# nh2/lz4-frame-conduit

Measured on AMD Instinct MI355X. Metric: GiB/s end-to-end (compress+decompress), 4 MiB blocks, 1/2/4/8 GPUs vs liblz4, higher is better.
Workload: dtype u8

## Files before the change

lz4_frame_conduit_amd/csrc/common.cuh:

```cuda
#pragma once
#include <hip/hip_runtime.h>
#include <stdint.h>

#include "records.hpp"

#define WAVE 64

namespace lz4f {

typedef const __attribute__((address_space(1))) void* gptr_t;
typedef __attribute__((address_space(3))) void* lptr_t;
typedef __attribute__((address_space(3))) uint32_t lds_u32;
typedef __attribute__((address_space(3))) uint8_t lds_u8;
typedef uint32_t u32_ua __attribute__((aligned(1)));
struct __attribute__((packed, aligned(1))) b16_ua { uint32_t a, b, c, d; };
struct __attribute__((aligned(4))) w3_a4 { uint32_t a, b, c; };

__device__ __forceinline__ uint32_t lane_id() { return threadIdx.x & (WAVE - 1); }
__device__ __forceinline__ uint32_t uni(uint32_t v) { return __builtin_amdgcn_readfirstlane(v); }
__device__ __forceinline__ uint64_t uni64(uint64_t v)
{
    uint32_t lo = __builtin_amdgcn_readfirstlane((uint32_t)v), hi = __builtin_amdgcn_readfirstlane((uint32_t)(v >> 32));
    return ((uint64_t)hi << 32) | lo;
}
// ... 41 lines not shown
        const bool body = lane < nfull, last = lane == nfull && tail;
        if (body || last) *(b16_ua*)(dst + (body ? lane * 16 : len - 16)) = b16_ua{p.a, p.b, p.c, p.d};
    }
}

struct v4u_ua { uint32_t a, b, c, d; } __attribute__((packed, aligned(1)));
struct CopyJob { const uint8_t* s; uint8_t* d; uint32_t n; };
__device__ __forceinline__ void job_load(Piece& p, const CopyJob& j, const uint8_t* safe)
{
    const uint32_t lane = lane_id(), nfull = j.n >> 4, tail = j.n & 15;
    const uint8_t* a = safe;
    if (lane < nfull) a = j.s + lane * 16; else if (lane == nfull && tail) a = j.s + j.n - 16;
    const v4u_ua t = *(const v4u_ua*)a;
    p.a = t.a; p.b = t.b; p.c = t.c; p.d = t.d;
}
__device__ __forceinline__ void job_store(const CopyJob& j, const Piece& p)
{
    const uint32_t lane = lane_id(), nfull = j.n >> 4, tail = j.n & 15;
    if (lane < nfull || (lane == nfull && tail)) {
        uint8_t* a = (lane < nfull) ? j.d + lane * 16 : j.d + j.n - 16;
        *(v4u_ua*)a = v4u_ua{p.a, p.b, p.c, p.d};
    }
}

__device__ __forceinline__ void wave_copy_match(uint8_t* dst, uint32_t offset, uint32_t len)
{
    const uint32_t lane = lane_id();
    const uint8_t* src = dst - offset;
    if (offset >= len) {
        wave_copy_disjoint(dst, src, len);
        return;
    }
    uint32_t done = 0;
    if (offset < 64) {
        uint32_t idx = lane % offset;
        const uint32_t inc = WAVE % offset;
        const uint32_t k = (1024 + offset - 1) / offset;
        const uint32_t need = (k - 1) * offset;
        while (done < len && done < need) {
            if (done + lane < len) dst[done + lane] = src[idx];
            idx += inc; if (idx >= offset) idx -= offset;
            done += WAVE;
        }
        if (done >= len) return;
        offset *= k;
        src = dst - offset;
    }
    const uint32_t R = (offset >= 1024) ? 1024u : (offset & ~15u);
    const uint32_t lanes_r = R >> 4;
    while (done < len) {
        const uint32_t left = len - done;
        if (left >= R) {
            if (lane < lanes_r) *(b16_ua*)(dst + done + lane * 16) = *(const b16_ua*)(src + done + lane * 16);
            done += R;
        } else {
            wave_copy_disjoint(dst + done, src + done, left);
            done = len;
        }
    }
}

__device__ __forceinline__ uint32_t dpp_incl_scan_add(uint32_t v)
{
    v += (uint32_t)__builtin_amdgcn_update_dpp(0, (int)v, 0x111 , 0xf, 0xf, true);
    v += (uint32_t)__builtin_amdgcn_update_dpp(0, (int)v, 0x112 , 0xf, 0xf, true);
    v += (uint32_t)__builtin_amdgcn_update_dpp(0, (int)v, 0x114 , 0xf, 0xf, true);
    v += (uint32_t)__builtin_amdgcn_update_dpp(0, (int)v, 0x118 , 0xf, 0xf, true);
    v += (uint32_t)__builtin_amdgcn_update_dpp(0, (int)v, 0x142 , 0xa, 0xf, false);
    v += (uint32_t)__builtin_amdgcn_update_dpp(0, (int)v, 0x143 , 0xc, 0xf, false);
    return v;
}
__device__ __forceinline__ uint32_t dpp_incl_scan_max(uint32_t v)
{
    uint32_t t;
    t = (uint32_t)__builtin_amdgcn_update_dpp(0, (int)v, 0x111, 0xf, 0xf, true); v = t > v ? t : v;
    t = (uint32_t)__builtin_amdgcn_update_dpp(0, (int)v, 0x112, 0xf, 0xf, true); v = t > v ? t : v;
    t = (uint32_t)__builtin_amdgcn_update_dpp(0, (int)v, 0x114, 0xf, 0xf, true); v = t > v ? t : v;
    t = (uint32_t)__builtin_amdgcn_update_dpp(0, (int)v, 0x118, 0xf, 0xf, true); v = t > v ? t : v;
    t = (uint32_t)__builtin_amdgcn_update_dpp(0, (int)v, 0x142, 0xa, 0xf, false); v = t > v ? t : v;
    t = (uint32_t)__builtin_amdgcn_update_dpp(0, (int)v, 0x143, 0xc, 0xf, false); v = t > v ? t : v;
    return v;
}

__device__ __forceinline__ uint32_t dpp_excl_scan_max(uint32_t v)
{
    const uint32_t incl = dpp_incl_scan_max(v);
    return (uint32_t)__builtin_amdgcn_update_dpp(0, (int)incl, 0x138 , 0xf, 0xf, true);
}

}
```

lz4_frame_conduit_amd/csrc/decode_indexed.cuh:

```cuda
#pragma once
#include "common.cuh"
#include "decode.cuh"
#include "decode_fused.cuh"
#include "decode_linked.cuh"
#include "encode.cuh"

namespace lz4f {

__device__ __forceinline__ uint64_t pt_load8(const uint8_t* __restrict__ in, uint32_t pos, uint64_t readable)
{
    if ((uint64_t)pos + 8 <= readable) { typedef uint64_t u64u __attribute__((aligned(1))); return *(const u64u*)(in + pos); }
    uint64_t v = 0;
    for (uint32_t i = 0; i < 8; i++) if ((uint64_t)pos + i < readable) v |= (uint64_t)in[pos + i] << (8 * i);
    return v;
}

__device__ __forceinline__ void pt_load16(const uint8_t* __restrict__ in, uint32_t pos, uint64_t readable, uint64_t& lo, uint64_t& hi)
{
    if ((uint64_t)pos + 16 <= readable) { typedef uint64_t u64u __attribute__((aligned(1))); lo = *(const u64u*)(in + pos); hi = *(const u64u*)(in + pos + 8); return; }
    lo = pt_load8(in, pos, readable); hi = pt_load8(in, pos + 8, readable);
}

__global__ void k_check_index(const void* __restrict__ ix, uint64_t ix_size, uint32_t n_max, uint32_t chunks_per_block, uint32_t chunk_size,
                              uint64_t seq_cap, uint32_t* __restrict__ flags, const ResultRec* __restrict__ res = nullptr)
{
    if (threadIdx.x != 0 || blockIdx.x != 0) return;
    const uint32_t n_blocks = res ? res->n_blocks : n_max;
    const IxHeader hd = *(const IxHeader*)ix;
    const bool ok = (!res || res->status == ST_OK) && n_blocks != 0 && n_blocks <= n_max && hd.magic == IX_MAGIC && hd.n_blocks == n_blocks && hd.chunks_per_block == chunks_per_block && hd.stride == IX_STRIDE &&
                    hd.total_entries <= (uint64_t)n_blocks * chunks_per_block * ix_max_entries_per_chunk(chunk_size) &&
                    hd.total_seqs <= (uint64_t)hd.total_entries * (IX_STRIDE + 1) && hd.total_seqs <= seq_cap &&
                    ix_entries_at(n_blocks, chunks_per_block) + (uint64_t)hd.total_entries * sizeof(IxEntry) <= ix_size;
    flags[7] = n_blocks;
    flags[8] = ok ? hd.total_entries : 0u;
    flags[9] = ok ? hd.total_seqs : 0u;
    if (!ok) atomicOr(flags, 1u);
}

__global__ __launch_bounds__(256) void k_check_blocks(const void* __restrict__ ix, const BlockOut* __restrict__ table, const ResultRec* __restrict__ res,
                                                      uint32_t n_max, uint32_t* __restrict__ flags)
{
    if (res->status != ST_OK || *flags) return;
    const uint32_t n = res->n_blocks < n_max ? res->n_blocks : n_max;
    const uint32_t b = blockIdx.x * blockDim.x + threadIdx.x;
    if (b >= n) return;
    const uint64_t n_seqs = flags[9], n_entries = flags[8];
    const IxBlock* blocks = ix_blocks(ix);
    const IxBlock bk = blocks[b];
    const bool stored = (table[b].word >> 31) != 0;
    bool wrong = stored ? (bk.nseq != 0 || bk.nentries != 0) : (bk.nseq == 0 || bk.nentries == 0);
    const uint64_t seq_end = (uint64_t)bk.seq_base + bk.nseq, ent_end = (uint64_t)bk.entry_base + bk.nentries;
    wrong |= seq_end > n_seqs || ent_end > n_entries;
    if (b == 0) wrong |= bk.seq_base != 0 || bk.entry_base != 0;
    if (b + 1 < n) { const IxBlock nb = blocks[b + 1]; wrong |= nb.seq_base != seq_end || nb.entry_base != ent_end; }
    else wrong |= seq_end != n_seqs || ent_end != n_entries;
    if (wrong) atomicOr(flags, 1u);
}

__device__ __forceinline__ bool parse_run(const uint8_t* __restrict__ in, uint32_t csize, uint64_t readable, uint32_t& pos, uint32_t op, uint32_t my_nseq,
                                          bool is_tail, SeqDesc* __restrict__ out, uint32_t linked, uint64_t out_front,
                                          uint32_t* opr = nullptr, uint32_t seq0 = 0, uint32_t omask = 0, uint32_t* op_end = nullptr)
{
    bool bad = false;
    uint32_t r0o = 0, r0n = 0, r0p = 0, r1o = 0, r1n = 0, r1p = 0, r2o = 0, r2n = 0, r2p = 0, r3o = 0, r3n = 0, r3p = 0;
    auto remember = [&](uint32_t o, uint32_t n, uint32_t pp) { r3o = r2o; r3n = r2n; r3p = r2p; r2o = r1o; r2n = r1n; r2p = r1p; r1o = r0o; r1n = r0n; r1p = r0p; r0o = o; r0n = n; r0p = pp; };
    uint64_t w, w_hi;
    SeqDesc pend{0u, 0u, 0u, 0u};
    pt_load16(in, pos, readable, w, w_hi);
    for (uint32_t i = 0; i < my_nseq && !bad; i++) {
        if (pos >= csize) { bad = true; break; }
        const uint32_t token = (uint32_t)w & 0xFF;
        uint32_t lit = token >> 4, p = pos + 1;
        if (lit == 15) {
            const uint64_t x = w >> 8;
            const uint32_t f = (uint32_t)__builtin_ctzll(~x), k = f >> 3;
            if (k < 7) { lit += 255u * k + (uint32_t)((x >> (f & 56u)) & 0xFF); p += k + 1; }
            else { for (;;) { if (p >= csize || lit > (1u << 24)) { bad = true; break; } const uint32_t v = in[p++]; lit += v; if (v != 255) break; } if (bad) break; }
        }
        if (p > csize || lit >= (1u << 24)) { bad = true; break; }
        const uint32_t in_left = csize - p;
        uint32_t mlen = 0, off = 0;
        if (lit + 8 > in_left) {
            if (lit != in_left || !is_tail || i + 1 != my_nseq) { bad = true; break; }
            pos = csize;
        } else {
            const uint32_t q = p + lit;
            uint64_t w2, w2_hi;
            pt_load16(in, q, readable, w2, w2_hi);
            __builtin_amdgcn_sched_barrier(0);
            if (i) out[i - 1] = pend;
            __builtin_amdgcn_sched_barrier(0);
            off = (uint32_t)w2 & 0xFFFF;
            if (off == 0) { bad = true; break; }
            mlen = token & 15; uint32_t pn = q + 2;
            bool reload = false;
            if (mlen == 15) {
                const uint64_t x = w2 >> 16;
                const uint32_t f = (uint32_t)__builtin_ctzll(~x), k = f >> 3;
                if (k < 6) { mlen += 255u * k + (uint32_t)((x >> (f & 56u)) & 0xFF); pn += k + 1; }
                else { reload = true; for (;;) { if (pn >= csize || mlen > (1u << 24)) { bad = true; break; } const uint32_t v = in[pn++]; mlen += v; if (v != 255) break; } if (bad) break; }
                if (pn + 4 >= csize) { bad = true; break; }
            }
            mlen += 4;
            pos = pn;
            if (reload) pt_load16(in, pos, readable, w, w_hi);
            else {
                const uint32_t sh = (pn - q) * 8u;
                w = sh >= 64 ? w2_hi : ((w2 >> sh) | (w2_hi << (64u - sh)));
            }
        }
        uint32_t f24 = off, mw = mlen;
        if (lit) remember(op, lit, p);
        if (mlen) {
            const uint32_t dm = op + lit;
            if (off > dm && (!linked || (uint64_t)(off - dm) > out_front)) { bad = true; break; }
            const uint32_t s0 = dm - off;
            uint32_t msrc = 0xFFFFFFFFu;
            if (mlen <= off && off <= dm) {
                if (s0 >= r0o && s0 + mlen <= r0o + r0n) msrc = r0p + (s0 - r0o);
// ... 1107 lines not shown
```

lz4_frame_conduit_amd/csrc/encode.cuh:

```cuda
#pragma once
#include <type_traits>
#include "common.cuh"

namespace lz4f {

constexpr uint32_t MFLIMIT = 12, LASTLIT = 5, MINMATCH = 4;
constexpr uint32_t ENC_POOL_SHORT = 0x200u;

struct ChunkInfo {
    uint32_t nrec;
    uint32_t first_lit;
    uint32_t tail_lit;
    uint32_t body_size;
    uint32_t carry_in;
    uint32_t flags;
    uint64_t out_off;
};

struct EncGeom {
    uint64_t src_size;
    uint64_t first_off;
    uint32_t write_endmark;
    uint32_t block_size;
    uint32_t chunk_size;
// ... 649 lines not shown
                        if (stop) { const uint32_t f = (uint32_t)__builtin_ctzll(stop); fw += f * 8 + (uint32_t)__builtin_amdgcn_readlane(g0, f); break; }
                        fw += WAVE * 8;
                    }
#endif
                    mp -= nb;
                    const uint32_t mlen = nb + fw;
                    myrec[nrec] = pack_rec(mp - anchor, mlen, d);
                    nrec++;
                    anchor = ip = mp + mlen;
                    step = (E1_STEP_HIT > 1 && mode == 1) ? (uint32_t)E1_STEP_HIT : 1u; two = 1;
                    atomicMax(lane == 0 ? &sh.cov : &sh.idle[lane], ip);
                    if (E1_OPENER == 2) *((lane == 0 && ip == end_lim) ? &sh.tail_d[par] : &sh.idle[lane]) = d;
                    E1DBG(a_hit += clock64() - z2;)
                    if (E1_IP2 && ip >= low + 2 && ip + 2 <= te) { const uint32_t q2 = ip - 2, hv2 = e1_mix(e1_ld32(sh.ring, q2)); *(lane == 0 ? &sh.table[e1_slot(hv2)] : (uint16_t*)&sh.idle[lane]) = (uint16_t)q2; *(lane == 0 ? &sh.tags[e1_slot(hv2)] : (uint8_t*)&sh.idle[lane]) = (uint8_t)e1_tag(hv2); }
                }
            }
            const bool mine_s = lane < grab && si + lane < nslice;
            *(mine_s ? &sh.s_end[par][si + lane] : &sh.idle[lane]) = (lane == 0 && nrec) ? anchor : 0u;
            *(mine_s ? &sh.s_n[par][si + lane] : (uint8_t*)&sh.idle[lane]) = (uint8_t)(lane == 0 ? nrec : 0u);
            if (mode == 0) atomicAdd(lane == 0 ? &sh.hits : &sh.idle[lane], nrec);
            if (opener) *(lane == 0 ? &sh.first : &sh.idle[lane]) = 1u;
        }
        E1DBG(const unsigned long long q2 = clock64();)
        __builtin_amdgcn_s_waitcnt(0);
        __syncthreads();
        mode_tile = uni(__hip_atomic_load(&sh.mode, __ATOMIC_RELAXED, __HIP_MEMORY_SCOPE_WORKGROUP));
        E1DBG(const unsigned long long q3 = clock64();)
        pend = true; p_c = c; p_par = par; p_ts = ts; p_te = te; p_bend = bend; p_ns = nslice;

        if (tid == 0) { sh.tail_d[par ^ 1u] = 0; sh.cov = nts; sh.hits = 0; sh.first = 0; sh.next = E1_ALIGN ? 0 : 1; sh.pieces[par ^ 1u] = 0; }
        if (tid < 16) sh.cur[tid] = 0;
        if (nlen) {
            if (nlen_full) {
                const uint32_t had = sh.pieces[par];
                for (uint32_t pc = had + wave; pc < E1_NPIECE; pc += E1_WAVES) e1_dma_piece(sh, src, org, nts, pc);
                if ((nts & E1_RMASK) == 0 && tid >= 64 && tid < 68) ((uint32_t*)(sh.ring + E1_RING))[tid - 64] = *(const u32_ua*)(src + (org + nts + (tid - 64) * 4u));
            } else e1_fill(sh, src, org, nts, nts + nlen, tid);
        }
        E1DBG(const unsigned long long q4 = clock64();)
        asm volatile("s_waitcnt vmcnt(0)" ::: "memory");
        E1DBG(const unsigned long long q5 = clock64();)
        __syncthreads();
        {
            const uint32_t td = uni(__hip_atomic_load(&sh.tail_d[par], __ATOMIC_RELAXED, __HIP_MEMORY_SCOPE_WORKGROUP));
            hold = (g.e1_solo & 1u) || (td != 0 && nlen >= 4 && uni(e1_ld32(sh.ring, nts)) == uni(e1_ld32(sh.ring, nts - td))) ? 1u : 0u;
        }
        E1DBG(if (blockIdx.x == 0 && lane == 0) { unsigned long long* d = (unsigned long long*)&scratch[E1_DBG_AT + 16 + wave * 8]; d[0] += q1 - q0; d[1] += q2 - q1; d[2] += q3 - q2; d[3] += q4 - q3; d[4] += q5 - q4; d[5] += clock64() - q5; d[6] += 1; unsigned long long* f = (unsigned long long*)&scratch[E1_DBG_AT + 160 + wave * 6]; f[0] += a_deq; f[1] += a_probe; f[2] += a_hit; f[3] += n_deq; f[4] += n_step; f[5] += n_hit; })
    }
    if (pend && wave == E1_WAVES - 1) merge(p_c, p_par, p_ts, p_te, p_bend, p_ns);
}


__device__ __forceinline__ uint32_t layout_block_chunks(ChunkInfo* __restrict__ ci, const uint32_t nch, const uint32_t blen)
{
    const uint32_t lane = lane_id();
    uint32_t carry_run = 0, total = 0;
    for (uint32_t c0 = 0; c0 < nch; c0 += WAVE) {
        const uint32_t c = c0 + lane;
        const bool act = c < nch;
        const uint4 x = act ? *(const uint4*)&ci[c] : uint4{0u, 0u, 0u, 0u};
        const bool has = act && x.x != 0;
        const uint64_t m = __ballot(has);
        uint32_t sum_tail, sum_size;
        const uint32_t pt = wave_excl_scan(act ? x.z : 0u, sum_tail);
        const uint64_t below = m & ((1ull << lane) - 1ull);
        const uint32_t p = below ? 63u - (uint32_t)__builtin_clzll(below) : 0u;
        const uint32_t pt_p = __shfl(pt, (int)p);
        const uint32_t carry = below ? pt - pt_p : carry_run + pt;
        const uint32_t size = has ? x.w + carry + len_ext_bytes(x.y + carry) - len_ext_bytes(x.y) : 0u;
        const uint32_t off = wave_excl_scan(size, sum_size);
        if (act) {
            *(uint2*)&ci[c].carry_in = uint2{carry, (c + 1 == nch) ? 2u : 0u};
            ci[c].out_off = total + off;
        }
        if (m) { const uint32_t last = 63u - (uint32_t)__builtin_clzll(m); carry_run = sum_tail - (uint32_t)__shfl(pt, (int)last); }
        else carry_run += sum_tail;
        total += sum_size;
    }
    total += 1 + len_ext_bytes(carry_run) + carry_run;
    const bool raw = total >= blen;
    if (raw) for (uint32_t c = lane; c < nch; c += WAVE) ci[c].flags = ((c + 1 == nch) ? 2u : 0u) | 1u;
    return raw ? (blen | 0x80000000u) : total;
}
__device__ __forceinline__ void layout_block(const EncGeom& g, ChunkInfo* __restrict__ info, BlockOut* __restrict__ table, uint32_t* __restrict__ blk_bytes, uint32_t b)
{
    const uint64_t bstart = g.first_off + (uint64_t)b * g.block_size;
    const uint32_t blen = (uint32_t)((bstart + g.block_size < g.src_size) ? g.block_size : g.src_size - bstart);
    const uint32_t word = layout_block_chunks(info + (uint64_t)b * g.chunks_per_block, (blen + g.chunk_size - 1) / g.chunk_size, blen);
    if (lane_id() == 0) {
        table[b].word = word;
        table[b].dst_off = bstart - g.first_off;
        table[b].dst_size = blen;
        blk_bytes[b] = 4 + (word & 0x7FFFFFFFu) + 4 * g.block_checksum;
    }
}
template <int WAVES_PER_WG>
__global__ __launch_bounds__(64 * WAVES_PER_WG) void k_layout_blocks(EncGeom g, ChunkInfo* __restrict__ info, BlockOut* __restrict__ table,
                                                                     uint32_t* __restrict__ blk_bytes)
{
    const uint32_t b = uni(blockIdx.x * WAVES_PER_WG + (threadIdx.x >> 6));
    if (b >= g.n_blocks) return;
    layout_block(g, info, table, blk_bytes, b);
}

__device__ __forceinline__ void layout_scan(const EncGeom& g, BlockOut* __restrict__ table, const uint32_t* __restrict__ blk_bytes,
                                            uint8_t* __restrict__ dst, uint64_t dst_cap, ResultRec* __restrict__ res, const uint64_t* __restrict__ recs,
                                            uint64_t* s_part, uint64_t& s_carry)
{
    const uint32_t t = threadIdx.x;
    if (t == 0) s_carry = g.header_size;
    __syncthreads();
    for (uint32_t base = 0; base < g.n_blocks; base += 1024) {
        const uint32_t b = base + t;
        const uint64_t v = (b < g.n_blocks) ? blk_bytes[b] : 0;
        s_part[t] = v;
        __syncthreads();
        for (uint32_t off = 1; off < 1024; off <<= 1) {
            uint64_t add = (t >= off) ? s_part[t - off] : 0;
            __syncthreads();
            s_part[t] += add;
            __syncthreads();
        }
        if (b < g.n_blocks) table[b].src_off = s_carry + s_part[t] - v + 4;
        __syncthreads();
        if (t == 1023) s_carry += s_part[1023];
        __syncthreads();
    }
    const uint64_t frame_size = s_carry + (g.write_endmark == 2 ? 8 : g.write_endmark ? 4 : 0);
    const bool fits = frame_size <= dst_cap;
    if (fits) {
        if (t < g.header_size) dst[t] = g.header[t];
        if (t < 4 && g.write_endmark) dst[s_carry + t] = 0;
    }
    if (t == 0 && res) {
        res->size = fits ? frame_size : 0; res->consumed = g.src_size - g.first_off;
        res->status = fits ? ST_OK : ST_DSTSMALL; res->n_blocks = g.n_blocks; res->first_bad_block = 0xFFFFFFFFu; res->flags = g.header[4] | ((g.n_chunks && rec_ctl(recs)[1]) ? ENC_POOL_SHORT : 0u);
    }
    if (t == 0 && g.n_chunks) { rec_ctl(recs)[0] = 0ull; rec_ctl(recs)[1] = 0ull; }
}
__global__ __launch_bounds__(1024) void k_layout_scan(EncGeom g, BlockOut* __restrict__ table, const uint32_t* __restrict__ blk_bytes,
                                                      uint8_t* __restrict__ dst, uint64_t dst_cap, ResultRec* __restrict__ res, const uint64_t* __restrict__ recs)
{
    __shared__ uint64_t s_part[1024];
    __shared__ uint64_t s_carry;
    layout_scan(g, table, blk_bytes, dst, dst_cap, res, recs, s_part, s_carry);
}

__device__ __forceinline__ void layout_chunk(const EncGeom& g, ChunkInfo* __restrict__ info, const BlockOut* __restrict__ table,
                                             uint8_t* __restrict__ dst, const ResultRec* res, uint32_t chunk)
{
    if (res->status != ST_OK) { info[chunk].flags |= 4u; return; }
    const uint32_t b = chunk / g.chunks_per_block, c = chunk % g.chunks_per_block;
    const BlockOut e = table[b];
    const uint32_t nch = (e.dst_size + g.chunk_size - 1) / g.chunk_size;
    if (c == 0) { const uint32_t w = e.word; uint8_t* q = dst + e.src_off - 4; q[0] = (uint8_t)w; q[1] = (uint8_t)(w >> 8); q[2] = (uint8_t)(w >> 16); q[3] = (uint8_t)(w >> 24); }
    if (c >= nch) return;
    info[chunk].out_off = (e.word >> 31) ? e.src_off + (uint64_t)c * g.chunk_size : e.src_off + info[chunk].out_off;
}
__global__ __launch_bounds__(256) void k_layout_chunks(EncGeom g, ChunkInfo* __restrict__ info, const BlockOut* __restrict__ table,
                                                       uint8_t* __restrict__ dst, const ResultRec* __restrict__ res)
{
    const uint32_t chunk = blockIdx.x * 256 + threadIdx.x;
    if (chunk >= g.n_chunks) return;
    layout_chunk(g, info, table, dst, res, chunk);
}
constexpr uint32_t LAYOUT_SMALL_BLOCKS = 64, LAYOUT_SMALL_CHUNKS = 4096;
__global__ __launch_bounds__(1024) void k_layout_small(EncGeom g, ChunkInfo* info, BlockOut* table, uint32_t* blk_bytes, uint8_t* __restrict__ dst, uint64_t dst_cap,
                                                       ResultRec* res, const uint64_t* __restrict__ recs)
{
    __shared__ uint64_t s_part[1024];
    __shared__ uint64_t s_carry;
    for (uint32_t b = uni(threadIdx.x >> 6); b < g.n_blocks; b += 16) layout_block(g, info, table, blk_bytes, b);
    __threadfence_block(); __syncthreads();
    layout_scan(g, table, blk_bytes, dst, dst_cap, res, recs, s_part, s_carry);
    __threadfence_block(); __syncthreads();
    for (uint32_t chunk = threadIdx.x; chunk < g.n_chunks; chunk += 1024) layout_chunk(g, info, table, dst, res, chunk);
}

constexpr uint32_t IX_MAGIC = 0x3258494Cu;
constexpr uint32_t IX_SRC_BIAS = 1u << 22;
constexpr uint32_t IX_STRIDE = 16;
struct IxHeader { uint32_t magic, n_blocks, chunks_per_block, total_seqs, total_entries, stride, pad0, pad1; };
struct IxBlock  { uint32_t seq_base, nseq, entry_base, nentries; };
struct IxChunk  { uint32_t ent_off, seq_off; };
struct IxEntry  { uint32_t in_off, out_pos, seq_off, nseq_blk; };
__host__ __device__ inline uint32_t ix_max_entries_per_chunk(uint32_t chunk_size) { return (chunk_size / 4 + 1 + IX_STRIDE - 1) / IX_STRIDE + 1; }
__host__ __device__ inline size_t ix_typical_entries(uint64_t src_size, uint32_t n_chunks) { return (size_t)(src_size / (64u * IX_STRIDE)) + n_chunks + 64; }
__host__ __device__ inline size_t ix_entries_at(uint32_t n_blocks, uint32_t chunks_per_block)
{
    return sizeof(IxHeader) + (size_t)n_blocks * sizeof(IxBlock) + (size_t)n_blocks * chunks_per_block * sizeof(IxChunk);
}
__device__ __forceinline__ IxBlock* ix_blocks(void* ix) { return (IxBlock*)((uint8_t*)ix + sizeof(IxHeader)); }
__device__ __forceinline__ const IxBlock* ix_blocks(const void* ix) { return (const IxBlock*)((const uint8_t*)ix + sizeof(IxHeader)); }
__device__ __forceinline__ IxChunk* ix_chunks(void* ix, uint32_t n_blocks) { return (IxChunk*)((uint8_t*)ix + sizeof(IxHeader) + (size_t)n_blocks * sizeof(IxBlock)); }
__device__ __forceinline__ IxEntry* ix_entries_w(void* ix, uint32_t n_blocks, uint32_t chunks_per_block) { return (IxEntry*)((uint8_t*)ix + ix_entries_at(n_blocks, chunks_per_block)); }
__device__ __forceinline__ const IxEntry* ix_entries(const void* ix, uint32_t n_blocks)
{
    return (const IxEntry*)((const uint8_t*)ix + ix_entries_at(n_blocks, ((const IxHeader*)ix)->chunks_per_block));
}

template <int WAVES_PER_WG>
__global__ __launch_bounds__(64 * WAVES_PER_WG) void k_index_blocks(EncGeom g, const ChunkInfo* __restrict__ info, const BlockOut* __restrict__ table,
                                                                    const ResultRec* __restrict__ res, void* __restrict__ ix, uint64_t ix_capacity)
{
    const uint32_t lane = lane_id();
    const uint32_t b = uni(blockIdx.x * WAVES_PER_WG + (threadIdx.x >> 6));
    if (b >= g.n_blocks || ix_capacity < ix_entries_at(g.n_blocks, g.chunks_per_block)) return;
    IxBlock* blocks = ix_blocks(ix);
    IxChunk* ck = ix_chunks(ix, g.n_blocks) + (uint64_t)b * g.chunks_per_block;
    const bool usable = res->status == ST_OK;
    const BlockOut e = table[b];
    const ChunkInfo* ci = info + (uint64_t)b * g.chunks_per_block;
    const uint32_t nch = (e.dst_size + g.chunk_size - 1) / g.chunk_size;
    uint32_t nseq = 0, nent = 0, last = 0xFFFFFFFFu;
    for (uint32_t c0 = 0; c0 < g.chunks_per_block; c0 += WAVE) {
        const uint32_t c = c0 + lane;
        const uint32_t nr = (c < nch && usable && !(e.word >> 31)) ? ci[c].nrec : 0u;
        uint32_t ts, te;
        const uint32_t ps = wave_excl_scan(nr, ts), pe = wave_excl_scan((nr + IX_STRIDE - 1) / IX_STRIDE, te);
        if (c < g.chunks_per_block) ck[c] = IxChunk{nent + pe, nseq + ps};
        const uint64_t m = __ballot(nr != 0);
        if (m) last = c0 + 63u - (uint32_t)__builtin_clzll(m);
        nseq += ts; nent += te;
    }
    if (lane == 0) {
        if (last != 0xFFFFFFFFu) { ck[last].ent_off |= 0x80000000u; nseq += 1; }
        blocks[b].nseq = nseq; blocks[b].nentries = nent;
    }
}

__global__ __launch_bounds__(1024) void k_build_index(EncGeom g, const ChunkInfo* __restrict__ info, const BlockOut* __restrict__ table,
                                                      const ResultRec* __restrict__ res, void* __restrict__ ix, uint64_t ix_capacity,
                                                      uint32_t blocks_done = 0)
{
    __shared__ uint32_t s_a[1024], s_b[1024];
    __shared__ uint32_t s_carry_a, s_carry_b;
    const uint32_t t = threadIdx.x;
    IxHeader* hd = (IxHeader*)ix;
    IxBlock* blocks = ix_blocks(ix);
    IxChunk* chunks = ix_chunks(ix, g.n_blocks);
    const size_t fixed = ix_entries_at(g.n_blocks, g.chunks_per_block);
    if (ix_capacity < fixed) { if (t == 0 && ix_capacity >= sizeof(IxHeader)) hd->magic = 0; return; }
    const bool usable = res->status == ST_OK;
    for (uint32_t b = t; b < g.n_blocks && !blocks_done; b += 1024) {
        const BlockOut e = table[b];
        const ChunkInfo* ci = info + (uint64_t)b * g.chunks_per_block;
        IxChunk* ck = chunks + (uint64_t)b * g.chunks_per_block;
        const uint32_t nch = (e.dst_size + g.chunk_size - 1) / g.chunk_size;
        uint32_t nseq = 0, nent = 0, last = 0xFFFFFFFFu;
        for (uint32_t c0 = 0; c0 < g.chunks_per_block; c0 += 8) {
            uint32_t nr[8];
#pragma unroll
            for (uint32_t k = 0; k < 8; k++) nr[k] = (c0 + k < nch) ? ci[c0 + k].nrec : 0;
#pragma unroll
            for (uint32_t k = 0; k < 8; k++) {
                const uint32_t c = c0 + k;
                if (c >= g.chunks_per_block) break;
                ck[c] = IxChunk{nent, nseq};
                if (usable && !(e.word >> 31) && nr[k]) { nseq += nr[k]; nent += (nr[k] + IX_STRIDE - 1) / IX_STRIDE; last = c; }
            }
        }
        if (last != 0xFFFFFFFFu) { ck[last].ent_off |= 0x80000000u; nseq += 1; }
        blocks[b].nseq = nseq; blocks[b].nentries = nent;
    }
    __syncthreads();
    if (t == 0) { s_carry_a = 0; s_carry_b = 0; }
    __syncthreads();
    for (uint32_t base = 0; base < g.n_blocks; base += 1024) {
        const uint32_t b = base + t;
        const uint32_t va = (b < g.n_blocks) ? blocks[b].nseq : 0, vb = (b < g.n_blocks) ? blocks[b].nentries : 0;
        s_a[t] = va; s_b[t] = vb;
        __syncthreads();
        for (uint32_t off = 1; off < 1024; off <<= 1) {
            const uint32_t aa = (t >= off) ? s_a[t - off] : 0, ab = (t >= off) ? s_b[t - off] : 0;
            __syncthreads();
            s_a[t] += aa; s_b[t] += ab;
            __syncthreads();
        }
        if (b < g.n_blocks) { blocks[b].seq_base = s_carry_a + s_a[t] - va; blocks[b].entry_base = s_carry_b + s_b[t] - vb; }
        __syncthreads();
        if (t == 1023) { s_carry_a += s_a[1023]; s_carry_b += s_b[1023]; }
        __syncthreads();
    }
    if (t == 0) {
        const bool fits = (uint64_t)s_carry_b * sizeof(IxEntry) <= ix_capacity - fixed;
        *hd = IxHeader{usable && fits ? IX_MAGIC : 0u, g.n_blocks, g.chunks_per_block, s_carry_a, s_carry_b, IX_STRIDE, g.linked ? 1u : 0u, 0u};
    }
}

__device__ __forceinline__ void emit_len_ext(uint8_t* p, uint32_t v )
{
    const uint32_t n255 = v / 255, lane = lane_id();
    for (uint32_t i = lane; i < n255; i += WAVE) p[i] = 255;
    if (lane == 0) p[n255] = (uint8_t)(v - n255 * 255);
}

#ifndef E2_V2
#define E2_V2 1
#endif
template <bool split>
__device__ __forceinline__ void emit_chunk(const uint8_t* __restrict__ src, const EncPlace& pl, const ChunkInfo& ci, const uint64_t* __restrict__ rec,
                                           uint8_t* __restrict__ dst, IxEntry* ent, const uint32_t ent_seq0, const uint32_t ent_last, const uint64_t pay0,
                                           const uint32_t blk, uint4* T0, uint4* T1, const uint32_t sub, const uint32_t nsub)
{
    const uint32_t lane = lane_id();
    const uint64_t bstart = pl.bstart, cs_abs = pl.cs_abs, ce_abs = pl.ce_abs;
    if (ci.flags & 4u) return;
    if (ci.flags & 1u) {
        uint8_t* o = dst + ci.out_off;
        const uint64_t n = ce_abs - cs_abs;
        if (sub) return;
        for (uint64_t off = 0; off < n; off += 1u << 20) {
            const uint32_t m = (uint32_t)((n - off < (1u << 20)) ? n - off : (1u << 20));
            wave_copy_disjoint(o + off, src + cs_abs + off, m);
        }
        return;
    }
    uint64_t lp_off = cs_abs - ci.carry_in;
    uint64_t o_off = ci.out_off;
    auto scan = [&](uint32_t v, uint32_t& total) -> uint32_t {
        uint32_t incl = v;
#pragma unroll
        for (int sft = 1; sft < 64; sft <<= 1) { const uint32_t t = __shfl_up(incl, sft); if ((int)lane >= sft) incl += t; }
        total = __builtin_amdgcn_readlane(incl, 63);
        return incl - v;
    };
    auto find = [&](uint32_t u) -> uint32_t {
        uint32_t j = 0;
#pragma unroll
        for (uint32_t step = 32; step; step >>= 1) { const uint32_t c = j + step; if (T0[c].x <= u) j = c; }
        return j;
    };
    auto put_ext = [&](uint8_t* q, uint32_t v ) {
        const uint32_t n255 = v / 255;
        for (uint32_t i = 0; i < n255; i++) q[i] = 255;
        q[n255] = (uint8_t)(v - n255 * 255);
    };
    if ((uint64_t)ci.nrec * 192 <= ce_abs - cs_abs) {
        uint8_t* o = dst + o_off;
        const uint8_t* lp = src + lp_off;
#if E2_V2
        for (uint32_t r0 = 0; r0 < ci.nrec; r0 += WAVE) {
            const uint32_t rl = r0 + lane;
            const uint64_t xr = rl < ci.nrec ? rec[rl] : 0ull;
            uint32_t vlit = (uint32_t)(xr & 0xFFFFFFu);
            const uint32_t vmlen = (uint32_t)((xr >> 24) & 0xFFFFFFu), voff = (uint32_t)(xr >> 48);
            if (rl == 0) vlit += ci.carry_in;
            const uint32_t vmcode = rl < ci.nrec ? vmlen - MINMATCH : 0u;
            const uint32_t vhb = 1 + len_ext_bytes(vlit), vtb = 2 + len_ext_bytes(vmcode);
            const uint32_t vtoken = ((vlit < 15 ? vlit : 15) << 4) | (vmcode < 15 ? vmcode : 15);
            const uint32_t vlrest = vlit >= 15 ? (vlit - 15) % 255 : 0u, vmrest = vmcode >= 15 ? (vmcode - 15) % 255 : 0u;
            const bool vbig = vhb > WAVE || vtb > WAVE;
            const uint32_t vp1 = (vbig ? 0u : vhb | (vtb << 8)) | (vtoken << 16) | (vlrest << 24), vp2 = voff | (vmrest << 16), vadv = vlit + vmlen;
            const uint32_t nb = ci.nrec - r0 < WAVE ? ci.nrec - r0 : WAVE;
            if constexpr (split) {
                const bool vact = rl < ci.nrec;
                uint32_t tot_sz, tot_adv;
                const uint32_t vso = scan(vact ? vhb + vlit + vtb : 0u, tot_sz), vsa = scan(vact ? vadv : 0u, tot_adv);
                for (uint32_t k = sub; k < nb; k += nsub) {
                    const uint32_t r = r0 + k;
                    const uint32_t lit = (uint32_t)__builtin_amdgcn_readlane((int)vlit, (int)k), so = (uint32_t)__builtin_amdgcn_readlane((int)vso, (int)k);
                    const uint32_t sa = (uint32_t)__builtin_amdgcn_readlane((int)vsa, (int)k);
                    const uint32_t p1 = (uint32_t)__builtin_amdgcn_readlane((int)vp1, (int)k), p2 = (uint32_t)__builtin_amdgcn_readlane((int)vp2, (int)k);
                    const uint32_t hb = p1 & 0xFFu, tb = (p1 >> 8) & 0xFFu, token = (p1 >> 16) & 0xFFu, off = p2 & 0xFFFFu;
                    uint8_t* q = o + so;
                    const uint8_t* ls = lp + sa;
                    if (ent && (r % IX_STRIDE) == 0 && lane == 0) {
                        uint32_t ns = ci.nrec - r < IX_STRIDE ? ci.nrec - r : IX_STRIDE;
                        if (ent_last && r + IX_STRIDE >= ci.nrec) ns += 1;
                        ent[r / IX_STRIDE] = IxEntry{(uint32_t)((uint64_t)(q - dst) - pay0), (uint32_t)((uint64_t)(ls - src) - bstart), ent_seq0 + r, ns | (blk << 8)};
// ... 228 lines not shown
```

lz4_frame_conduit_amd/csrc/engine.hip:

```cpp
#include <hip/hip_runtime.h>
#include <stdarg.h>
#include <stdio.h>
#include <stdlib.h>
#include <string.h>

#include <algorithm>
#include <mutex>
#include <vector>

#include "engine.hpp"
#include "frame_dev.cuh"
#include "decode_batch.cuh"
#include "encode_batch.cuh"
#include "measure_batch.cuh"

using namespace lz4f;

static_assert(sizeof(ChunkInfo) == 32, "chunk info layout");
static_assert(sizeof(BatchFrame) == 80 && sizeof(BatchBlk) == 40, "batch workspace layout");
static_assert(sizeof(BatchCore) == 64 && sizeof(MeasBlk) == 24, "batch measure workspace layout");
static_assert(sizeof(BcFrame) == 72 && sizeof(BcBlk) == 32 && sizeof(BcChunk) == 64, "batch encode workspace layout");

namespace lz4f {

// ... 62 lines not shown
    dense_mode = (unsigned)num("LZ4F_MI355X_DENSE_MODE", 0, 2, 0);
    group_kib = (unsigned)num("LZ4F_MI355X_GROUP_KIB", 64, 4096, 0);
    if (group_kib & (group_kib - 1)) group_kib = 0;
    feed_round = (unsigned)num("LZ4F_MI355X_FEED_ROUND", 17, 4096, 0);
    chain_gate = num("LZ4F_MI355X_CHAIN_GATE", 1, (1 << 20) - 1, 0);
    decode_mode = 0; if (const char* v = getenv("LZ4F_MI355X_DECODE")) decode_mode = v[0];
    e1_run = (unsigned)num("LZ4F_MI355X_E1_RUN", 1, 4096, 0);
    e1_solo = 0; if (const char* v = getenv("LZ4F_MI355X_E1_SOLO")) e1_solo = (unsigned)atoi(v);
    if (on("LZ4F_MI355X_DETERMINISTIC")) e1_solo |= 1u;
    wait_ticks = 0; if (const char* v = getenv("LZ4F_MI355X_WAIT_TICKS")) { unsigned long long a = 0; if (sscanf(v, "%llu", &a) == 1) wait_ticks = a; }
    dblk_lds = (unsigned)num("LZ4F_MI355X_DBLK_LDS", 1, 150, 0) << 10;
    recs_per_tile = (unsigned)num("LZ4F_MI355X_RECS_PER_TILE", 1, 16385, 0);
    hc_attempts = (unsigned)num("LZ4F_MI355X_HC_ATTEMPTS", 1, 65536, 0);
    hc_lazy = (unsigned)num("LZ4F_MI355X_HC_LAZY", 1, 2, 0);
    seed = 2; if (const char* v = getenv("LZ4F_MI355X_SEED")) { unsigned a = 0; if (sscanf(v, "%u", &a) == 1 && a >= 1 && a <= 64) seed = a; }
}
namespace lz4f {
size_t new_engine(lz4f_mi355x_engine** out, int device, void* stream, bool borrow)
{
    int n = 0;
    hipError_t e = hipGetDeviceCount(&n);
    if (e != hipSuccess || n <= 0) {
        set_last_error("no usable HIP device (hipGetDeviceCount: %s, count %d): liblz4f_mi355x has no CPU fallback", hipGetErrorString(e), n);
        return make_err(LZ4F_ERROR_GENERIC);
    }
    if (device < 0 || device >= n) { set_last_error("device %d out of range (%d devices)", device, n); return make_err(LZ4F_ERROR_GENERIC); }
    HIP_TRY(hipSetDevice(device));
    lz4f_mi355x_engine* en = new lz4f_mi355x_engine();
    en->device = device;
    en->sw.read();
    if (borrow) { en->stream = stream; en->own_stream = false; }
    else {
        hipStream_t s;
        hipError_t e2 = hipStreamCreateWithFlags(&s, hipStreamNonBlocking);
        if (e2 != hipSuccess) { delete en; set_last_error("hipStreamCreate failed: %s", hipGetErrorString(e2)); return make_err(LZ4F_ERROR_GENERIC); }
        en->stream = s; en->own_stream = true;
    }
    *out = en;
    return 0;
}

namespace {
struct EnginePool {
    std::mutex mu;
    std::vector<lz4f_mi355x_engine*> idle;
    ~EnginePool() { drain(); }
    void drain()
    {
        std::vector<lz4f_mi355x_engine*> v;
        { std::lock_guard<std::mutex> g(mu); v.swap(idle); }
        for (auto* e : v) delete e;
    }
};
EnginePool& pool() { static EnginePool p; return p; }
}

size_t acquire_engine(lz4f_mi355x_engine** out, int device)
{
    if (device < 0) device = selected_device();
    {
        EnginePool& p = pool();
        std::lock_guard<std::mutex> g(p.mu);
        for (size_t i = 0; i < p.idle.size(); i++)
            if (p.idle[i]->device == device) { *out = p.idle[i]; p.idle.erase(p.idle.begin() + i); return 0; }
    }
    return new_engine(out, device, nullptr, false);
}
void release_engine(lz4f_mi355x_engine* e)
{
    if (!e) return;
    EnginePool& p = pool();
    std::lock_guard<std::mutex> g(p.mu);
    p.idle.push_back(e);
}
void release_idle_engines() { pool().drain(); }

}

lz4f_mi355x_engine::~lz4f_mi355x_engine()
{
    (void)hipSetDevice(device);
    (void)hipStreamSynchronize((hipStream_t)stream);
    desc.release(); seqcnt.release(); spx.release(); selfix.release(); selfcnt.release(); postab.release(); pdbuf.release(); tight.release();
    info.release(); recs.release(); e1_scratch.release(); walkbuf.release(); density.release(); ixtmp.release(); table.release(); blk_bytes.release(); res.release(); bad.release();
    d_in.release(); d_out.release(); bframes.release(); btable.release(); mframes.release(); mtable.release(); cframes.release(); cblocks.release(); cchunks.release();
    h_in.release(); h_out.release(); h_small.release();
    for (int i = 0; i < 24; i++) if (ev[i]) (void)hipEventDestroy((hipEvent_t)ev[i]);
    if (aux_stream) { (void)hipStreamSynchronize((hipStream_t)aux_stream); (void)hipStreamDestroy((hipStream_t)aux_stream); }
    if (ev_fork) (void)hipEventDestroy((hipEvent_t)ev_fork);
    if (ev_join) (void)hipEventDestroy((hipEvent_t)ev_join);
    if (own_stream && stream) (void)hipStreamDestroy((hipStream_t)stream);
}

void lz4f_mi355x_engine::tick(int slot, bool end, void* on_stream)
{
    if (!timing) return;
    const int i = slot * 2 + (end ? 1 : 0);
    if (!ev[i]) { hipEvent_t e; if (hipEventCreate(&e) != hipSuccess) return; ev[i] = e; }
    (void)hipEventRecord((hipEvent_t)ev[i], (hipStream_t)(on_stream ? on_stream : stream));
    if (end) ev_used[slot] = true;
}
bool lz4f_mi355x_engine::aux_ready()
{
    if (aux_stream && ev_fork && ev_join) return true;
    hipStream_t s; hipEvent_t a, b;
    if (!aux_stream) { if (hipStreamCreateWithFlags(&s, hipStreamNonBlocking) != hipSuccess) { (void)hipGetLastError(); return false; } aux_stream = s; }
    if (!ev_fork) { if (hipEventCreateWithFlags(&a, hipEventDisableTiming) != hipSuccess) { (void)hipGetLastError(); return false; } ev_fork = a; }
    if (!ev_join) { if (hipEventCreateWithFlags(&b, hipEventDisableTiming) != hipSuccess) { (void)hipGetLastError(); return false; } ev_join = b; }
    return true;
}

size_t lz4f_mi355x_engine::sync()
{
    HIP_TRY(hipSetDevice(device));
    HIP_TRY(hipStreamSynchronize((hipStream_t)stream));
    if (aux_pending && aux_stream) { HIP_TRY(hipStreamSynchronize((hipStream_t)aux_stream)); aux_pending = false; }
    return 0;
}

static unsigned long long* g_prof = nullptr;
static unsigned long long* prof_buf()
{
    if (!g_prof) { if (hipMalloc(&g_prof, 1024) != hipSuccess) return nullptr; (void)hipMemset(g_prof, 0, 1024); (void)hipMemset(g_prof + 70, 0xFF, 8); (void)hipMemset(g_prof + 75, 0xFF, 8); }
    return g_prof;
}
extern "C" __attribute__((visibility("default"))) int lz4f_mi355x_debug_prof(unsigned long long* out128)
{
    if (!prof_buf()) return 1;
    (void)hipDeviceSynchronize();
    const int rc = hipMemcpy(out128, g_prof, 1024, hipMemcpyDeviceToHost) == hipSuccess ? 0 : 2;
#ifdef DB_PROF
    { unsigned long long z[32] = {0}; (void)hipMemcpyFromSymbol(out128 + 96, HIP_SYMBOL(lz4f::g_dbprof), sizeof(z)); (void)hipMemcpyToSymbol(HIP_SYMBOL(lz4f::g_dbprof), z, sizeof(z)); }
#endif
    (void)hipMemset(g_prof, 0, 1024); (void)hipMemset(g_prof + 70, 0xFF, 8); (void)hipMemset(g_prof + 75, 0xFF, 8);
    return rc;
}

static uint32_t device_cus(int device)
{
    static int cus[64];
    const unsigned d = (unsigned)device % 64;
    if (!cus[d]) { int v = 0; if (hipDeviceGetAttribute(&v, hipDeviceAttributeMultiprocessorCount, device) != hipSuccess || v < 1) v = 256; cus[d] = v; }
    return (uint32_t)cus[d];
}


struct EncShape { uint32_t chunk, chunks_per_block; uint64_t n_blocks; };
static EncShape enc_shape(uint64_t payload, uint32_t block_size)
{
    const uint32_t chunk = pick_chunk_size(block_size);
    return EncShape{chunk, block_size / chunk, (payload + block_size - 1) / block_size};
}
static size_t index_capacity(uint64_t payload, const EncShape& s)
{
    return ix_entries_at((uint32_t)s.n_blocks, s.chunks_per_block) + ix_typical_entries(payload, (uint32_t)(s.n_blocks * s.chunks_per_block)) * sizeof(IxEntry);
}

static uint64_t rec_pool_records(uint32_t n_chunks, uint32_t max_rec_per_chunk, unsigned per_tile)
{
    const uint64_t worst = (uint64_t)(n_chunks + 1) * max_rec_per_chunk;
    uint64_t want = (uint64_t)(n_chunks + 1) * (per_tile ? per_tile : 12288u);
    if (want < 64ull * max_rec_per_chunk) want = 64ull * max_rec_per_chunk;
    if (want > worst) want = worst;
    if (want > 0xFFFFFFF0ull) want = 0xFFFFFFF0ull;
    return want;
}

struct lz4f_mi355x_engine::EncodePlan {
    bool too_large;
    EncGeom g;
    enum Finder { E1_SHARED, E1_SOLO, HASH_CHAIN } finder;
    uint32_t e1_wgs;
    bool layout_small, e2_split;
    bool xxh_lane4;
    bool inband;
    size_t index_cap;
    size_t info_bytes, recs_bytes, blk_bytes, table_bytes, res_bytes, e1_scratch_bytes, ixtmp_bytes;
};

lz4f_mi355x_engine::EncodePlan lz4f_mi355x_engine::encode_plan(const CompressJob& j, const Switches& sw, uint32_t cus, bool inband, size_t index_cap)
{
    EncodePlan p; memset(&p, 0, sizeof(p));
    EncGeom& g = p.g;
    const uint64_t payload = j.src_size - j.first_off;
    const EncShape s = enc_shape(payload, j.block_size);
    if (s.n_blocks > 0x7FFFFFFFull / s.chunks_per_block) { p.too_large = true; return p; }
    g.src_size = j.src_size; g.first_off = j.first_off; g.write_endmark = j.endmark ? (j.content_checksum ? 2 : 1) : 0;
    g.block_size = j.block_size; g.chunk_size = s.chunk; g.chunks_per_block = s.chunks_per_block;
    g.n_blocks = (uint32_t)s.n_blocks; g.n_chunks = g.n_blocks * g.chunks_per_block;
    g.linked = j.linked; g.block_checksum = j.block_checksum;
    g.header_size = j.header_size; memcpy(g.header, j.header, j.header_size);
    g.max_rec_per_chunk = g.chunk_size / 4 + 1;
    g.seed_stride = sw.seed;
    const bool hc = j.level >= 3;
    p.finder = hc ? EncodePlan::HASH_CHAIN : ((sw.e1_solo & 1u) && !(sw.e1_solo & 4u)) ? EncodePlan::E1_SOLO : EncodePlan::E1_SHARED;
    if (hc) {
        const HcLevel hl = hc_level(j.level);
        g.hc_attempts = sw.hc_attempts ? sw.hc_attempts : hl.attempts;
        g.hc_lazy = sw.hc_lazy ? sw.hc_lazy : hl.lazy;
    }
    g.rec_pool = rec_pool_records(g.n_chunks, g.max_rec_per_chunk, ((sw.e1_solo & 1u) || hc) ? 16385u : sw.recs_per_tile);
    if (g.n_chunks) {
        uint32_t run = g.n_chunks / cus; run = run < 1 ? 1 : run > 64 ? 64 : run;
        if ((g.n_chunks + run - 1) / run > 1024) run = (g.n_chunks + 1023) / 1024;
        if (sw.e1_run) run = sw.e1_run;
        g.tiles_per_wg = run;
        g.e1_solo = sw.e1_solo;
        p.e1_wgs = (g.n_chunks + run - 1) / run;
        p.e1_scratch_bytes = (size_t)p.e1_wgs * 2 * E1_NSLICE * E1_REC_PER_SLICE * 8 + 2048;
    }
    p.layout_small = g.n_blocks <= LAYOUT_SMALL_BLOCKS && g.n_chunks <= LAYOUT_SMALL_CHUNKS; p.e2_split = g.n_chunks <= 512;
    p.xxh_lane4 = g.n_blocks < XXH_LANE4_BELOW;
    p.inband = inband;
    p.index_cap = inband ? index_capacity(payload, s) + 64 : index_cap;
    p.ixtmp_bytes = inband ? p.index_cap + 64 : 0;
    p.info_bytes = (size_t)(g.n_chunks + 1) * sizeof(ChunkInfo); p.recs_bytes = (size_t)(rec_pool_at(g.n_chunks) + g.rec_pool) * 8;
    p.blk_bytes = (size_t)(g.n_blocks + 1) * 4; p.table_bytes = (size_t)(g.n_blocks + 1) * sizeof(BlockOut);
    p.res_bytes = sizeof(ResultRec) + sizeof(TrailerPlan) + 64;
    return p;
}

#ifdef E1_DEBUG
static void e1_debug_dump(hipStream_t st, const uint8_t* counters)
{
    unsigned long long d[256]; if (hipStreamSynchronize(st) == hipSuccess && hipMemcpy(d, counters, 2048, hipMemcpyDeviceToHost) == hipSuccess) {
                for (int w = 0; w < 16; w += 5) { unsigned long long* x = d + 16 + w * 8; if (x[6]) fprintf(stderr, "E1 wave %d: per tile cycles: merge %llu parse %llu waitB1 %llu dma-issue %llu dma-wait %llu waitB2 %llu (%llu tiles)\n", w, x[0]/x[6], x[1]/x[6], x[2]/x[6], x[3]/x[6], x[4]/x[6], x[5]/x[6], x[6]); unsigned long long* f = d + 160 + w * 6; fprintf(stderr, "   parse: dequeue %llu cycles x %llu, probe step %llu cycles x %llu, hit %llu cycles x %llu (per tile)\n", f[3] ? f[0]/f[3] : 0, f[3]/x[6], f[4] ? f[1]/f[4] : 0, f[4]/x[6], f[5] ? f[2]/f[5] : 0, f[5]/x[6]); }
                fprintf(stderr, "E1 dense passes (workgroup 0): %llu, matches taken %llu, positions advanced %llu; one-match steps because: hit in B %llu, mode not dense %llu, step != 1 %llu, first match long %llu\n", d[13], d[14], d[15], d[4], d[5], d[6], d[7]);
                fprintf(stderr, "E1 debug: bounds hit: dequeue %llu, probe %llu, backward %llu, forward %llu; probe ip/last %llx step/slice %llx; back room/nb %llx; fwd mp/fw %llx end_lim/d %llx\n", d[0], d[1], d[2], d[3], d[8], d[9], d[10], d[11], d[12]); }
}
#endif

size_t lz4f_mi355x_engine::enc_workspaces(const EncodePlan& p, bool own_table)
{
    if (ixtmp.ensure(p.ixtmp_bytes) || res.ensure(p.res_bytes) || info.ensure(p.info_bytes) || recs.ensure(p.recs_bytes) || blk_bytes.ensure(p.blk_bytes) ||
        (own_table && table.ensure(p.table_bytes)) || e1_scratch.ensure(p.e1_scratch_bytes))
        return make_err(LZ4F_ERROR_allocation_failed);
    return 0;
}

size_t lz4f_mi355x_engine::enc_find(const CompressJob& j, const EncodePlan& p)
{
    hipStream_t st = (hipStream_t)stream; const EncGeom& g = p.g;
#ifdef E1_DEBUG
    uint8_t* const counters = (uint8_t*)e1_scratch.p + p.e1_scratch_bytes - 2048;
    (void)hipMemsetAsync(counters, 0, 2048, st);
#endif
    if (recs_ctl_clean != recs.p) { HIP_TRY(hipMemsetAsync(recs.p, 0, 64, st)); }
    recs_ctl_clean = nullptr;
    if (p.finder == EncodePlan::HASH_CHAIN)
        hipLaunchKernelGGL(k_find_matches_hc, dim3(g.n_chunks), dim3(64 * HC_WAVES), 0, st, j.d_src, g, (ChunkInfo*)info.p, (uint64_t*)recs.p);
    else if (p.finder == EncodePlan::E1_SOLO)
        hipLaunchKernelGGL((k_find_matches_solo<1>), dim3(g.n_chunks), dim3(64), 0, st, j.d_src, g, (ChunkInfo*)info.p, (uint64_t*)recs.p);
    else
        hipLaunchKernelGGL(k_find_matches, dim3(p.e1_wgs), dim3(64 * E1_WAVES), 0, st, j.d_src, g, (ChunkInfo*)info.p, (uint64_t*)recs.p, (uint64_t*)e1_scratch.p);
    if (sw.e1_sync) (void)hipStreamSynchronize(st);
#ifdef E1_DEBUG
    e1_debug_dump(st, counters);
#endif
    return 0;
}

void lz4f_mi355x_engine::enc_layout(const EncodePlan& p, uint8_t* d_dst, uint64_t dst_cap, ResultRec* rec, BlockOut* tbl, void* d_index)
{
    constexpr int W = 4;
    hipStream_t st = (hipStream_t)stream; const EncGeom& g = p.g;
    if (p.layout_small)
        hipLaunchKernelGGL(k_layout_small, dim3(1), dim3(1024), 0, st, g, (ChunkInfo*)info.p, tbl, (uint32_t*)blk_bytes.p, d_dst, dst_cap, rec, (const uint64_t*)recs.p);
    else {
        if (g.n_blocks) hipLaunchKernelGGL((k_layout_blocks<W>), dim3((g.n_blocks + W - 1) / W), dim3(64 * W), 0, st, g, (ChunkInfo*)info.p, tbl, (uint32_t*)blk_bytes.p);
        hipLaunchKernelGGL(k_layout_scan, dim3(1), dim3(1024), 0, st, g, tbl, (const uint32_t*)blk_bytes.p, d_dst, dst_cap, rec, (const uint64_t*)recs.p);
        if (g.n_chunks) hipLaunchKernelGGL(k_layout_chunks, dim3((g.n_chunks + 255) / 256), dim3(256), 0, st, g, (ChunkInfo*)info.p, (const BlockOut*)tbl, d_dst, (const ResultRec*)rec);
    }
    if (g.n_chunks) recs_ctl_clean = recs.p;
    if (d_index) {
        if (g.n_blocks) hipLaunchKernelGGL((k_index_blocks<W>), dim3((g.n_blocks + W - 1) / W), dim3(64 * W), 0, st, g, (const ChunkInfo*)info.p, (const BlockOut*)tbl, (const ResultRec*)rec, d_index, (uint64_t)p.index_cap);
        hipLaunchKernelGGL(k_build_index, dim3(1), dim3(1024), 0, st, g, (const ChunkInfo*)info.p, (const BlockOut*)tbl, (const ResultRec*)rec, d_index, (uint64_t)p.index_cap, 1u);
    }
}

void lz4f_mi355x_engine::enc_emit(const CompressJob& j, const EncodePlan& p, uint8_t* d_dst, const ResultRec* rec, BlockOut* tbl, void* d_index)
{
    constexpr int W = 4;
    hipStream_t st = (hipStream_t)stream; const EncGeom& g = p.g;
    tick(2, false);
    if (p.e2_split)
        hipLaunchKernelGGL((k_emit_gather<W, true>), dim3(g.n_chunks), dim3(64 * W), 0, st, j.d_src, g, (const ChunkInfo*)info.p,
                           (const uint64_t*)recs.p, d_dst, (const BlockOut*)tbl, d_index);
    else
        hipLaunchKernelGGL((k_emit_gather<W, false>), dim3((g.n_chunks + W - 1) / W), dim3(64 * W), 0, st, j.d_src, g, (const ChunkInfo*)info.p,
                           (const uint64_t*)recs.p, d_dst, (const BlockOut*)tbl, d_index);
    tick(2, true);
    if (!j.block_checksum) return;
    tick(3, false);
    if (p.xxh_lane4)
        hipLaunchKernelGGL((k_xxh32_blocks4<1>), dim3(g.n_blocks), dim3(64), XXH_SPREAD_LDS, st, d_dst, tbl, rec, g.n_blocks, 0u, (uint32_t*)nullptr);
    else
        hipLaunchKernelGGL((k_xxh32_blocks<W>), dim3((g.n_blocks + W - 1) / W), dim3(64 * W), 0, st, d_dst, tbl, rec, g.n_blocks, 0u, (uint32_t*)nullptr);
    tick(3, true);
}

void lz4f_mi355x_engine::enc_tail(const CompressJob& j, const EncodePlan& p, uint8_t* d_dst, uint64_t dst_cap, ResultRec* rec, const BlockOut* tbl, const void* d_index)
{
    hipStream_t st = (hipStream_t)stream; const EncGeom& g = p.g;
    if (j.endmark && j.content_checksum)
        hipLaunchKernelGGL(k_xxh32_content, dim3(1), dim3(64), 0, st, j.d_src + j.first_off, (uint64_t)(j.src_size - j.first_off), d_dst, rec, 0u);
    if (p.inband && g.n_blocks) {
        TrailerPlan* plan = (TrailerPlan*)((uint8_t*)res.p + sizeof(ResultRec) + 32);
        hipLaunchKernelGGL(k_trailer_plan, dim3(1), dim3(64), 0, st, d_dst, dst_cap, rec, g.n_blocks, d_index,
                           (uint64_t)ix_entries_at(g.n_blocks, g.chunks_per_block), plan);
        hipLaunchKernelGGL(k_trailer_copy, dim3(256), dim3(256), 0, st, d_dst, (const TrailerPlan*)plan, tbl, g.n_blocks, d_index);
    }
}

lz4f_mi355x_engine::CompressJob lz4f_mi355x_engine::make_compress_job(const uint8_t* d_src, uint64_t src_size, uint64_t first_off, uint32_t block_size,
                                                                      bool linked, bool block_checksum, int level, const LZ4F_preferences_t* frame)
{
    CompressJob j; memset(&j, 0, sizeof(j));
    j.d_src = d_src; j.src_size = src_size; j.first_off = first_off; j.block_size = block_size;
    j.linked = linked; j.block_checksum = block_checksum; j.level = level;
    if (frame) { j.endmark = true; j.content_checksum = frame->frameInfo.contentChecksumFlag != 0; j.header_size = (uint32_t)write_frame_header(j.header, *frame); }
    return j;
}

size_t lz4f_mi355x_engine::launch_compress(const CompressJob& j, uint8_t* d_dst, uint64_t dst_cap,
                                           lz4f_mi355x_result* d_res, lz4f_mi355x_block* d_table, void* d_index, size_t index_cap)
{
    const bool inband = d_index == nullptr && index_cap == LZ4F_MI355X_INBAND;
    HIP_TRY(hipSetDevice(device));
    const EncodePlan p = encode_plan(j, sw, device_cus(device), inband, index_cap);
    if (inband && ((uintptr_t)d_dst & 15) != 0) { set_last_error("in-band index: the frame buffer must be 16-byte aligned"); return make_err(LZ4F_ERROR_GENERIC); }
    if (p.too_large) { set_last_error("input too large for one call"); return make_err(LZ4F_ERROR_srcSize_tooLarge); }
    if (size_t e = enc_workspaces(p, !d_table)) return e;
    if (inband) d_index = ixtmp.p;
    BlockOut* tbl = (BlockOut*)(d_table ? d_table : table.p);
    ResultRec* r = (ResultRec*)(d_res ? d_res : res.p);
    for (int i = 0; i < 4; i++) ev_used[i] = false;
    ev_used[10] = false;
    tick(10, false);
    if (p.g.n_chunks) {
        tick(0, false);
        if (size_t e = enc_find(j, p)) return e;
        tick(0, true);
    }
    tick(1, false);
    enc_layout(p, d_dst, dst_cap, r, tbl, d_index);
    tick(1, true);
    if (p.g.n_chunks) enc_emit(j, p, d_dst, r, tbl, d_index);
    enc_tail(j, p, d_dst, dst_cap, r, tbl, d_index);
    tick(10, true);
    HIP_TRY(hipGetLastError());
    return 0;
}

lz4f_mi355x_engine::DecodePlan lz4f_mi355x_engine::decode_plan(const DecompressJob& j, const Switches& sw, uint32_t cus)
{
    DecodePlan p;
    p.given = j.d_table || j.table_in_place || j.table_direct;
    p.n_max = p.given ? j.n_blocks : j.max_blocks;
    p.begin_small = p.given && p.n_max <= 256;
    const bool hinted = j.hint_list && j.hint_n <= p.n_max;
    if (p.given) p.walk = DecodePlan::WALK_NONE;
    else if (hinted) p.walk = DecodePlan::WALK_TRAILER;
    else if (j.block_size <= (256u << 10) && j.frame_cap >= (1u << 20) && !sw.serial_walk) p.walk = DecodePlan::WALK_PARALLEL;
    else if (j.block_size > (256u << 10) && j.frame_cap >= (size_t)192 * j.block_size && !sw.serial_walk) p.walk = DecodePlan::WALK_SEEDED;
    else p.walk = DecodePlan::WALK_SERIAL;
    p.mode = sw.decode_mode ? sw.decode_mode : (j.linked || j.block_size >= (256u << 10)) ? 'f' : '1';
    p.ix_by_trailer = j.d_index && j.ix_seqs && hinted;
    p.self_index = !sw.no_selfindex && (j.linked ? j.hist0 <= 65536 && p.n_max >= 2 : j.block_size >= (256u << 10) && j.block_size <= (4u << 20) && !sw.no_spx);
    p.n_ix = hinted ? j.hint_n : p.n_max;
    p.windowed = j.linked && j.dst_cap < 0xFFF00000ull && !sw.no_window && !(p.n_max == 1 && p.given);
    p.small = !j.linked && j.block_size <= (1u << 20);
    p.relay = j.block_size > 65536u && sw.dense_mode != 2 && (sw.dense_mode == 1 || p.n_max <= 3u * cus);
    const uint32_t group_bytes = sw.group_kib ? sw.group_kib << 10 : ((uint64_t)p.n_ix * j.block_size <= (2ull << 30) ? (512u << 10) : (1u << 20));
    p.group = (j.linked && j.block_size < group_bytes && !sw.no_groups) ? group_bytes / j.block_size : 1u;
    p.wait_ticks = sw.wait_ticks ? sw.wait_ticks : 50000000ull + 20ull * p.n_ix * j.block_size;
    return p;
}
lz4f_mi355x_engine::IxRoute lz4f_mi355x_engine::ix_route(const DecompressJob& j, const Switches& sw, uint32_t n_ix, uint32_t ix_seqs)
{
    IxRoute r;
    const uint64_t span = (uint64_t)n_ix * j.block_size;
    r.doubling = ((uint64_t)ix_seqs * 48 > span || sw.trace_always) && span <= IXP_MAX_SPAN && !sw.no_doubling;
    r.selffed = !j.linked && !sw.no_selffeed && !sw.no_resolve && !sw.trace_always && !r.doubling;
    const bool trace_can = !sw.no_trace && !sw.no_resolve && (j.block_size & 63u) == 0;
    r.gate = !trace_can ? 0u : sw.trace_always ? 2u : (j.linked || r.doubling) ? 1u : 0u;
    return r;
}
static bool prof_read(hipStream_t st, void* to, const void* from, size_t n) { return hipStreamSynchronize(st) == hipSuccess && hipMemcpy(to, from, n, hipMemcpyDeviceToHost) == hipSuccess; }

size_t lz4f_mi355x_engine::dec_table(const DecompressJob& j, const DecodePlan& p, ResultRec* res, BlockOut** tbl_out, uint32_t* path)
{
    hipStream_t st = (hipStream_t)stream; const uint32_t n_max = p.n_max;
    BlockOut* tbl = (BlockOut*)j.table_direct;
    if (!tbl) { if (table.ensure((size_t)(n_max + 1) * sizeof(BlockOut))) return make_err(LZ4F_ERROR_allocation_failed); tbl = (BlockOut*)table.p; }
    if (p.given) {
        if (!j.table_in_place && !j.table_direct)
            HIP_TRY(hipMemcpyAsync(tbl, j.d_table, (size_t)n_max * sizeof(BlockOut), hipMemcpyDeviceToDevice, st));
        if (p.begin_small)
            hipLaunchKernelGGL(k_begin_table_small, dim3(1), dim3(256), 0, st, (const BlockOut*)tbl, n_max, (uint64_t)j.frame_cap, (uint64_t)j.dst_cap,
                               j.block_size, j.block_checksum ? 1u : 0u, j.linked ? 1u : 0u, res, (uint32_t*)bad.p);
        else {
            hipLaunchKernelGGL(k_init_result, dim3(1), dim3(64), 0, st, res, n_max, 0u);
            if (n_max) hipLaunchKernelGGL(k_check_table, dim3(std::min<uint32_t>((n_max + 255) / 256, 1024u)), dim3(256), 0, st, (const BlockOut*)tbl, n_max, (uint64_t)j.frame_cap, (uint64_t)j.dst_cap,
                                          j.block_size, j.block_checksum ? 1u : 0u, j.linked ? 1u : 0u, res);
        }
        *path |= LZ4F_MI355X_PATH_TABLE_GIVEN;
    } else {
        tick(4, false);
        const size_t list_cap = (size_t)n_max + 1024;
        uint32_t lgrid = std::min<uint32_t>((uint32_t)((list_cap + 255) / 256), 4096u);
        WalkState* ws = nullptr; const uint64_t* list = nullptr;
        if (p.walk == DecodePlan::WALK_TRAILER) {
            if (walkbuf.ensure(256)) return make_err(LZ4F_ERROR_allocation_failed);
            ws = (WalkState*)walkbuf.p;
            hipLaunchKernelGGL(k_walk_head, dim3(1), dim3(64), 0, st, j.d_frame, j.frame_cap, ws, j.hint_n);
            list = j.hint_list;
            lgrid = std::min<uint32_t>((j.hint_n + 255) / 256, 4096u);
            *path |= LZ4F_MI355X_PATH_TRAILER;
        } else if (p.walk == DecodePlan::WALK_PARALLEL) {
            const uint32_t n_chunks = (uint32_t)((j.frame_cap + WK_CHUNK - 1) / WK_CHUNK);
            const size_t at_chunks = 256, at_list = at_chunks + (size_t)n_chunks * sizeof(WalkChunk), at_list2 = at_list + list_cap * 8, at_mark = at_list2 + list_cap * 8;
            if (walkbuf.ensure(at_mark + list_cap * 4)) return make_err(LZ4F_ERROR_allocation_failed);
            ws = (WalkState*)walkbuf.p;
            WalkChunk* ch = (WalkChunk*)((uint8_t*)walkbuf.p + at_chunks);
            uint64_t* list1 = (uint64_t*)((uint8_t*)walkbuf.p + at_list);
            uint64_t* list2 = (uint64_t*)((uint8_t*)walkbuf.p + at_list2);
            uint32_t* mark = (uint32_t*)((uint8_t*)walkbuf.p + at_mark);
            HIP_TRY(hipMemsetAsync(mark, 0, list_cap * 4, st));
            hipLaunchKernelGGL(k_walk_head, dim3(1), dim3(64), 0, st, j.d_frame, j.frame_cap, ws);
            hipLaunchKernelGGL(k_walk_cand, dim3(n_chunks), dim3(256), 0, st, j.d_frame, j.frame_cap, (const WalkState*)ws, ch);
            hipLaunchKernelGGL(k_walk_order, dim3(1), dim3(1024), 0, st, ch, n_chunks, ws, list1, (uint32_t)list_cap);
            hipLaunchKernelGGL(k_walk_mark, dim3(lgrid), dim3(256), 0, st, j.d_frame, j.frame_cap, (const WalkState*)ws, (const uint64_t*)list1, mark);
            hipLaunchKernelGGL(k_walk_filter, dim3(1), dim3(1024), 0, st, ws, (const uint64_t*)list1, (const uint32_t*)mark, list2);
            list = list2;
            *path |= LZ4F_MI355X_PATH_PARALLEL_WALK;
        } else if (p.walk == DecodePlan::WALK_SEEDED) {
            const size_t at_seeds = 256, at_list = at_seeds + (WK_SEEDS + 1) * 8;
            if (walkbuf.ensure(at_list + list_cap * 8)) return make_err(LZ4F_ERROR_allocation_failed);
            ws = (WalkState*)walkbuf.p;
            unsigned long long* seeds = (unsigned long long*)((uint8_t*)walkbuf.p + at_seeds);
            HIP_TRY(hipMemsetAsync(seeds, 0xFF, (WK_SEEDS + 1) * 8, st));
            uint64_t* list1 = (uint64_t*)((uint8_t*)walkbuf.p + at_list);
            hipLaunchKernelGGL(k_walk_head, dim3(1), dim3(64), 0, st, j.d_frame, j.frame_cap, ws);
            hipLaunchKernelGGL(k_walk_seeds, dim3(WK_SEEDS * wk_seed_pieces(j.block_size)), dim3(256), 0, st, j.d_frame, j.frame_cap, (const WalkState*)ws, seeds);
            hipLaunchKernelGGL(k_walk_chains, dim3(1), dim3(WK_SEEDS), 0, st, j.d_frame, j.frame_cap, ws, (const unsigned long long*)seeds, list1, (uint32_t)std::min<size_t>(list_cap, 0xFFFFFFFFu));
            list = list1;
            *path |= LZ4F_MI355X_PATH_PARALLEL_WALK;
        }
        if (list) {
            hipLaunchKernelGGL(k_walk_link, dim3(lgrid), dim3(256), 0, st, j.d_frame, j.frame_cap, j.dst_cap, ws, list, tbl, n_max);
            hipLaunchKernelGGL(k_walk_verdict, dim3(1), dim3(64), 0, st, j.d_frame, j.frame_cap, j.dst_cap, ws, list, n_max, res);
            WalkState h;
            if (sw.prof && p.walk == DecodePlan::WALK_PARALLEL && prof_read(st, &h, ws, sizeof(h))) fprintf(stderr, "parallel walk: done %u overflow %u candidates %u first_end %u first_break %u (header ok %u, hsize %u, block %u)\n", h.done, h.overflow, h.total, h.first_end, h.first_break, h.head_ok, h.hsize, h.bs);
            if (sw.prof && p.walk == DecodePlan::WALK_SEEDED && prof_read(st, &h, ws, sizeof(h))) fprintf(stderr, "seeded walk: done %u overflow %u entries %u first_end %u first_break %u\n", h.done, h.overflow, h.total, h.first_end, h.first_break);
        }
        hipLaunchKernelGGL(k_walk_frame, dim3(1), dim3(64), 0, st, j.d_frame, j.frame_cap, j.dst_cap, tbl, n_max, res, list ? (const uint32_t*)&ws->done : nullptr);
        tick(4, true);
    }
    if (!p.begin_small) {
        HIP_TRY(hipMemsetAsync(bad.p, 0xFF, 8, st));
        HIP_TRY(hipMemsetAsync((uint8_t*)bad.p + 8, 0, 24, st));
    }
    *tbl_out = tbl;
    return 0;
}

size_t lz4f_mi355x_engine::dec_checksums(const DecompressJob& j, const DecodePlan& p, ResultRec* res, BlockOut* tbl)
{
    constexpr int W = 4;
    hipStream_t st = (hipStream_t)stream; const uint32_t n_max = p.n_max;
    const bool beside = !sw.no_overlap && aux_ready();
    hipStream_t xs = beside ? (hipStream_t)aux_stream : st;
    if (beside) { HIP_TRY(hipEventRecord((hipEvent_t)ev_fork, st)); HIP_TRY(hipStreamWaitEvent(xs, (hipEvent_t)ev_fork, 0)); }
    tick(5, false, xs);
    if (n_max < XXH_LANE4_BELOW)
        hipLaunchKernelGGL((k_xxh32_blocks4<1>), dim3(n_max), dim3(64), beside ? (12u << 10) : XXH_SPREAD_LDS, xs, (uint8_t*)j.d_frame, tbl, res, n_max, 1u, (uint32_t*)bad.p);
    else
        hipLaunchKernelGGL((k_xxh32_blocks<W>), dim3((n_max + W - 1) / W), dim3(64 * W), 0, xs, (uint8_t*)j.d_frame, tbl, res, n_max, 1u, (uint32_t*)bad.p);
    tick(5, true, xs);
    if (beside) { HIP_TRY(hipEventRecord((hipEvent_t)ev_join, xs)); aux_pending = true; }
    return 0;
}

size_t lz4f_mi355x_engine::dec_index(const DecompressJob& j, const DecodePlan& p, ResultRec* res, BlockOut* tbl, IndexSrc* ix, uint32_t* path)
{
    if (p.mode != 'f' || sw.no_index) return 0;
    hipStream_t st = (hipStream_t)stream;
    IndexSrc x{p.ix_by_trailer ? IndexSrc::TRAILER : IndexSrc::GIVEN, j.d_index, j.index_size, j.ix_seqs, j.ix_entries};
    if (j.d_index && j.index_size >= sizeof(IxHeader) && !p.ix_by_trailer && (j.linked || !j.ix_seqs)) {
        IxHeader hd; memset(&hd, 0, sizeof(hd));
        HIP_TRY(hipMemcpyAsync(&hd, j.d_index, sizeof(hd), hipMemcpyDeviceToHost, st));
        HIP_TRY(hipStreamSynchronize(st));
        if (hd.magic == IX_MAGIC && hd.stride == IX_STRIDE) { x.seqs = hd.total_seqs; x.entries = hd.total_entries; x.from = IndexSrc::HEADER; }
        else if (j.linked) x = IndexSrc();
    }
    if (!x.d && p.self_index)
        if (size_t e = dec_self_index(j, p, res, tbl, !j.linked, &x)) return e;
    const bool self = x.from == IndexSrc::SELF_LINKED || x.from == IndexSrc::SPX;
    if (self) *path |= LZ4F_MI355X_PATH_SELF_INDEX;
    if (!x.d || x.size < sizeof(IxHeader) || (j.linked && !self && !((p.given || p.ix_by_trailer) && j.hist0 <= 65536))) return 0;
    if ((uint64_t)x.seqs > (uint64_t)x.entries * (IX_STRIDE + 1) || x.entries > (x.size - sizeof(IxHeader)) / sizeof(IxEntry)) x.seqs = 0;
    *ix = x;
    return 0;
}

size_t lz4f_mi355x_engine::dec_self_index(const DecompressJob& j, const DecodePlan& p, ResultRec* res, BlockOut* tbl, bool spx_walk, IndexSrc* ix)
{
    hipStream_t st = (hipStream_t)stream; const uint32_t n_max = p.n_max, cpb = j.block_size / pick_chunk_size(j.block_size);
    const size_t fixed = ix_entries_at(n_max, cpb), spx_at = (size_t)n_max * (SPX_MAXPT + 1) * sizeof(SpxPoint);
    if (selfcnt.ensure((size_t)n_max * 8 + 64) || seqcnt.ensure(256 + (size_t)n_max * (8 + 8 * IXL_PUB)) || selfix.ensure(fixed + 64) || density.ensure(64) ||
        (spx_walk && spx.ensure((size_t)n_max * ((SPX_MAXPT + 1) * sizeof(SpxPoint) + 4) + 64)))
        return make_err(LZ4F_ERROR_allocation_failed);
    uint32_t* cnt = (uint32_t*)selfcnt.p; uint32_t* osz = cnt + n_max;
    HIP_TRY(hipMemsetAsync(seqcnt.p, 0, spx_walk ? 256 : 64, st));
    hipLaunchKernelGGL(k_density_probe, dim3(1), dim3(64), 0, st, j.d_frame, (uint64_t)j.frame_cap, (const BlockOut*)tbl, res, n_max, (uint32_t*)density.p);
    if (spx_walk)
        hipLaunchKernelGGL(k_spx_index, dim3(n_max), dim3(SPX_MAXSEG), 0, st, j.d_frame, (uint64_t)j.frame_cap, (const BlockOut*)tbl, res, n_max, cnt, osz,
                           (SpxPoint*)spx.p, (uint32_t*)((uint8_t*)spx.p + spx_at), (uint32_t*)seqcnt.p, sw.no_density_probe ? (const uint32_t*)nullptr : (const uint32_t*)density.p + 1);
    else {
        hipLaunchKernelGGL((k_selfindex_walk_wave<0, 4>), dim3((n_max + 3) / 4), dim3(256), 0, st, j.d_frame, (uint64_t)j.frame_cap, (const BlockOut*)tbl,
                           res, n_max, cnt, osz, (void*)nullptr, (uint32_t*)seqcnt.p, (const uint32_t*)density.p);
        hipLaunchKernelGGL(k_selfindex_walk<0>, dim3((n_max + 255) / 256), dim3(256), 0, st, j.d_frame, (uint64_t)j.frame_cap, (const BlockOut*)tbl,
                           res, n_max, cnt, osz, (void*)nullptr, (uint32_t*)seqcnt.p, (const uint32_t*)density.p + 1);
    }
    uint32_t tot[10];
    for (int pass = 0; pass < 2; pass++) {
        hipLaunchKernelGGL(k_selfindex_scan, dim3(1), dim3(1024), 0, st, tbl, res, n_max, (const uint32_t*)cnt, (const uint32_t*)osz,
                           selfix.p, cpb, (uint64_t)j.dst_cap, j.block_size, (uint32_t*)seqcnt.p, spx_walk ? 1u : 0u);
        if (pass == 1) break;
        HIP_TRY(hipMemcpyAsync(tot, seqcnt.p, sizeof(tot), hipMemcpyDeviceToHost, st));
        HIP_TRY(hipStreamSynchronize(st));
        if (spx_walk && sw.prof) fprintf(stderr, "spx: flags %u, %u sequences in %u blocks, %u stretches walked by the stitching thread\n", tot[0], tot[9], n_max, tot[2]);
#ifdef SPX_PROF
        if (spx_walk) { uint32_t y[8]; if (hipMemcpy(y, (uint32_t*)seqcnt.p + 48, 32, hipMemcpyDeviceToHost) == hipSuccess) fprintf(stderr, "spx lanes: hit the hop cap %u, without a start %u, started at their segment's first byte %u, ran into something %u; most sequences in one lane %u\n", y[0], y[1], y[2], y[3], y[4]); }
        if (spx_walk) { uint32_t z[8]; if (hipMemcpy(z, (uint32_t*)seqcnt.p + 40, 32, hipMemcpyDeviceToHost) == hipSuccess) fprintf(stderr, "spx cycles: guess max %u avg %u, walk max %u avg %u, stitch max %u avg %u, workgroup max %u (waves %u)\n", z[0], (unsigned)(((unsigned long long)z[4] << 8) / (2 * n_max)), z[1], (unsigned)(((unsigned long long)z[5] << 8) / (2 * n_max)), z[2], (unsigned)(((unsigned long long)z[6] << 8) / n_max), z[3], 2 * n_max); }
#endif
        if (tot[0] != 0 || tot[9] == 0) break;
        const void* before = selfix.p;
        if (selfix.ensure(fixed + (size_t)tot[8] * sizeof(IxEntry) + 64)) return make_err(LZ4F_ERROR_allocation_failed);
        if (selfix.p == before) break;
    }
    if (tot[0] != 0 || tot[9] == 0) return 0;
    if (!spx_walk) {
        hipLaunchKernelGGL((k_selfindex_walk_wave<1, 4>), dim3((n_max + 3) / 4), dim3(256), 0, st, j.d_frame, (uint64_t)j.frame_cap, (const BlockOut*)tbl,
                           res, n_max, cnt, osz, selfix.p, (uint32_t*)seqcnt.p, (const uint32_t*)density.p);
        hipLaunchKernelGGL(k_selfindex_walk<1>, dim3((n_max + 255) / 256), dim3(256), 0, st, j.d_frame, (uint64_t)j.frame_cap, (const BlockOut*)tbl,
                           res, n_max, cnt, osz, selfix.p, (uint32_t*)seqcnt.p, (const uint32_t*)density.p + 1);
    }
    *ix = IndexSrc{spx_walk ? IndexSrc::SPX : IndexSrc::SELF_LINKED, selfix.p, fixed + (size_t)tot[8] * sizeof(IxEntry), tot[9], tot[8]};
    return 0;
}

size_t lz4f_mi355x_engine::dec_indexed(const DecompressJob& j, const DecodePlan& p, ResultRec* res, BlockOut* tbl, const IndexSrc& ix, const uint32_t** ix_flags, uint32_t* path)
{
    if (!ix.d) return 0;
    hipStream_t st = (hipStream_t)stream; void* d_index = ix.d;
    const uint32_t chunk = pick_chunk_size(j.block_size), cpb = j.block_size / chunk, n_ix = p.n_ix;
    if ((size_t)ix.seqs + 4096 > ix_seq_cap) ix_seq_cap = (size_t)ix.seqs + ix.seqs / 4 + 4096;
    if (!ix.seqs) return 0;
    const size_t dsrc_at = (ix_seq_cap + 64) * sizeof(SeqDesc);
    if (desc.ensure(dsrc_at + (ix_seq_cap + 64) * 4) || seqcnt.ensure(256 + (size_t)p.n_max * (8 + 8 * IXL_PUB))) return make_err(LZ4F_ERROR_allocation_failed);
    HIP_TRY(hipMemsetAsync(seqcnt.p, 0, 256 + (j.linked ? (size_t)p.n_max * 8 : 0), st));
    unsigned long long* iprof = (unsigned long long*)(sw.prof ? prof_buf() : nullptr);
    tick(8, false);
    hipLaunchKernelGGL(k_check_index, dim3(1), dim3(64), 0, st, (const void*)d_index, (uint64_t)ix.size, n_ix, cpb, chunk,
                       (uint64_t)ix_seq_cap, (uint32_t*)seqcnt.p, (const ResultRec*)res);
    hipLaunchKernelGGL(k_check_blocks, dim3((n_ix + 255) / 256), dim3(256), 0, st, (const void*)d_index, (const BlockOut*)tbl, (const ResultRec*)res, n_ix,
                       (uint32_t*)seqcnt.p);
    const IxRoute r = ix_route(j, sw, n_ix, ix.seqs);
    *ix_flags = (const uint32_t*)seqcnt.p;
    *path |= LZ4F_MI355X_PATH_INDEXED;
    if (r.selffed) {
        tick(8, true); tick(9, false);
        auto selffed = [&](auto src) {
            using S = decltype(src);
            if (j.block_size <= (1u << 20))
                hipLaunchKernelGGL((k_copy_selffed<FzCfgS4, S>), dim3(n_ix), dim3(64 * 4), 0, st, j.d_frame, (uint64_t)j.frame_cap, j.d_dst, tbl, (const ResultRec*)res, n_ix,
                                   (const void*)d_index, (SeqDesc*)desc.p, (uint32_t*)seqcnt.p, iprof, src, sw.feed_round, j.block_size);
            else
                hipLaunchKernelGGL((k_copy_selffed<FzCfgS8, S>), dim3(n_ix), dim3(64 * 8), 0, st, j.d_frame, (uint64_t)j.frame_cap, j.d_dst, tbl, (const ResultRec*)res, n_ix,
                                   (const void*)d_index, (SeqDesc*)desc.p, (uint32_t*)seqcnt.p, iprof, src, sw.feed_round, j.block_size);
        };
        if (ix.from == IndexSrc::SPX) selffed(FzSrcSpx{(const SpxPoint*)spx.p, (const uint32_t*)((const uint8_t*)spx.p + (size_t)p.n_max * (SPX_MAXPT + 1) * sizeof(SpxPoint))});
        else selffed(FzSrcIx{(const void*)d_index, n_ix});
        tick(9, true);
        return 0;
    }
    uint32_t* done = (uint32_t*)seqcnt.p + 64;
    const uint32_t lk = j.linked ? 1u | (uint32_t)sw.chain_gate << 1 : 0u;
    const uint32_t n_lanes = ix.entries > n_ix ? ix.entries : n_ix;
    if (ix.from == IndexSrc::SPX)
        hipLaunchKernelGGL(k_spx_parse, dim3(n_ix), dim3(128), 0, st, j.d_frame, (uint64_t)j.frame_cap, (const BlockOut*)tbl, (const ResultRec*)res, n_ix,
                           d_index, (const SpxPoint*)spx.p, (const uint32_t*)((const uint8_t*)spx.p + (size_t)p.n_max * (SPX_MAXPT + 1) * sizeof(SpxPoint)),
                           (SeqDesc*)desc.p, (uint32_t*)seqcnt.p);
    else
        hipLaunchKernelGGL(k_parse_indexed, dim3((n_lanes + 255) / 256), dim3(256), 0, st, j.d_frame, (uint64_t)j.frame_cap,
                           (const BlockOut*)tbl, d_index, n_ix, (SeqDesc*)desc.p, (uint32_t*)seqcnt.p, lk, (uint64_t)j.hist0);
    const uint64_t trace_span = (uint64_t)n_ix * j.block_size;
    const uint32_t res_gy = j.block_size >= (1u << 19) ? j.block_size >> 18 : 1u;
    uint32_t gate = r.gate;
    if (gate && postab.ensure((size_t)(trace_span >> 6) * 4 + 512 + ((size_t)(trace_span >> IXT_REGION_LOG) + 4) * 4)) gate = 0;
    if (gate && r.doubling)
        hipLaunchKernelGGL(k_dense_gate, dim3(1), dim3(64), 0, st, (uint32_t*)seqcnt.p, gate, (const BlockOut*)tbl, (const ResultRec*)res, n_ix, 1u, 1u);
    uint32_t* dsrc = sw.no_resolve ? nullptr : (uint32_t*)((uint8_t*)desc.p + dsrc_at);
    if (dsrc)
        hipLaunchKernelGGL(k_resolve_direct, dim3(n_ix, res_gy), dim3(256), 0, st, d_index, (const BlockOut*)tbl, (const ResultRec*)res, n_ix, (const SeqDesc*)desc.p,
                           dsrc, (uint32_t*)seqcnt.p, (iprof ? 1u : 0u) | (gate ? 2u : 0u), lk);
    if (iprof) {
        uint32_t c[8]; if (prof_read(st, c, seqcnt.p, 32)) fprintf(stderr, "indexed: flags %u, matches direct after parse %u, resolved %u, left to the chain %u\n", c[0], c[4], c[5], c[6]);
        uint32_t x[6] = {0, 0, 0, 0, 0, 0}; if (hipMemcpy(x, (uint32_t*)seqcnt.p + 10, 24, hipMemcpyDeviceToHost) == hipSuccess) fprintf(stderr, "indexed (linked): %u matches stay on the chain, %u of them reach into the block in front (%u blocks); not resolved because: beyond one block %u, source straddles two runs %u, run-length source %u, hop limit %u\n", x[0], x[1], n_ix, x[2], x[3], x[4], x[5]);
    }
    hipLaunchKernelGGL(k_dense_gate, dim3(1), dim3(64), 0, st, (uint32_t*)seqcnt.p, gate, (const BlockOut*)tbl, (const ResultRec*)res, n_ix, 0u, res_gy);
    if (gate) {
        hipLaunchKernelGGL(k_build_postab, dim3(n_ix, res_gy), dim3(256), 0, st, d_index, (const BlockOut*)tbl, (const ResultRec*)res, n_ix,
                           (const SeqDesc*)desc.p, (uint32_t*)postab.p, (uint32_t*)seqcnt.p);
        const uint64_t n_thr = (trace_span + IXT_TB - 1) / IXT_TB;
        const uint32_t pd_grid = (uint32_t)((trace_span / 4 + 255) / 256), pd_ngrp = pd_grid * 4u;
        const size_t pd_grp_at = (((size_t)trace_span * 4 + 255) & ~(size_t)255) + (((IXP_ROUNDS + 1) * IXP_STRIPES * 4 + 255) & ~(size_t)255);
        if (r.doubling && !pdbuf.ensure(pd_grp_at + 2 * (size_t)pd_ngrp + 256)) {
            *path |= LZ4F_MI355X_PATH_DOUBLING;
            uint32_t* remaining = (uint32_t*)((uint8_t*)pdbuf.p + (((size_t)trace_span * 4 + 255) & ~(size_t)255));
            if (hipMemsetAsync(remaining, 0, (IXP_ROUNDS + 1) * IXP_STRIPES * 4, st) != hipSuccess) return make_err(LZ4F_ERROR_GENERIC);
            hipLaunchKernelGGL(k_pd_init, dim3((uint32_t)((n_thr + 255) / 256)), dim3(256), 0, st, j.d_frame, (uint64_t)j.frame_cap, j.d_dst, (const BlockOut*)tbl,
                               (const ResultRec*)res, n_ix, d_index, (const SeqDesc*)desc.p, (const uint32_t*)dsrc, (const uint32_t*)postab.p, (uint32_t*)seqcnt.p,
                               lk & 1u, (uint32_t)j.block_size, (uint64_t)j.hist0, (uint32_t*)pdbuf.p, remaining);
            for (uint32_t rd = 1; rd <= IXP_ROUNDS; rd++)
                hipLaunchKernelGGL(k_pd_round, dim3(pd_grid), dim3(256), 0, st, j.d_dst, (uint32_t*)pdbuf.p, (const BlockOut*)tbl,
                                   (const ResultRec*)res, n_ix, rd, remaining, (uint32_t*)seqcnt.p, (uint8_t*)pdbuf.p + pd_grp_at, pd_ngrp);
            hipLaunchKernelGGL(k_pd_verdict, dim3(1), dim3(64), 0, st, (uint32_t*)seqcnt.p, (const uint32_t*)remaining);
            if (iprof) { static uint32_t t[(IXP_ROUNDS + 1) * IXP_STRIPES]; if (prof_read(st, t, remaining, sizeof(t))) { fprintf(stderr, "doubling: bytes open after each round:"); for (uint32_t rd = 0; rd <= IXP_ROUNDS; rd++) { uint64_t sum = 0; for (uint32_t q = 0; q < IXP_STRIPES; q++) sum += t[rd * IXP_STRIPES + q]; fprintf(stderr, " %llu", (unsigned long long)sum); } fprintf(stderr, "\n"); } }
        } else {
            *path |= LZ4F_MI355X_PATH_TRACE_HOPS;
            uint32_t* region_cnt = (uint32_t*)((uint8_t*)postab.p + (((size_t)(trace_span >> 6) * 4 + 255) & ~(size_t)255));
            if (hipMemsetAsync(region_cnt, 0, ((size_t)(trace_span >> IXT_REGION_LOG) + 2) * 4, st) != hipSuccess) return make_err(LZ4F_ERROR_GENERIC);
            const uint32_t tc_wg = (uint32_t)((n_thr + 255) / 256);
            hipLaunchKernelGGL(k_trace_copy, dim3(std::min<uint32_t>(tc_wg, 8192u)), dim3(256), 0, st, j.d_frame, (uint64_t)j.frame_cap, j.d_dst, (const BlockOut*)tbl,
                               (const ResultRec*)res, n_ix, d_index, (const SeqDesc*)desc.p, (const uint32_t*)dsrc, (const uint32_t*)postab.p, (uint32_t*)seqcnt.p,
                               lk & 1u, (uint32_t)j.block_size, (uint64_t)j.hist0, region_cnt, iprof ? 1u : 0u, tc_wg);
            uint32_t t[8] = {0, 0, 0, 0, 0, 0, 0, 0};
            if (iprof && prof_read(st, t, (uint32_t*)seqcnt.p + 24, 32) && t[0]) fprintf(stderr, "traced: %llu turns for %u pieces (%u read from the output), deepest thread %u turns\n", (unsigned long long)t[2] | ((unsigned long long)t[3] << 32), t[4], t[5], t[6]);
        }
    }
    tick(8, true); tick(9, false);
    auto copy = [&](auto cfg) {
        using C = decltype(cfg);
        hipLaunchKernelGGL(k_copy_indexed<C>, dim3((n_ix + p.group - 1) / p.group), dim3(64 * C::WAVES), 0, st, j.d_frame, j.d_dst, tbl, (const ResultRec*)res, n_ix,
                           d_index, (const SeqDesc*)desc.p, (const uint32_t*)dsrc, (uint32_t*)seqcnt.p, iprof, lk, done, p.group, (uint64_t)j.hist0, p.wait_ticks);
    };
    if (j.block_size <= (1u << 20)) copy(FzCfg<4>()); else copy(FzCfg<8>());
    tick(9, true);
    uint32_t y[4] = {0, 0, 0, 0};
    if (iprof && j.linked && prof_read(st, y, (uint32_t*)seqcnt.p + 20, 16)) fprintf(stderr, "indexed (linked): blocks that found the block in front at state 3: %u (of those, had to wait for all of it: %u); blocks with set-aside matches %u (block in front already done: %u)\n", y[0], y[1], y[2], y[3]);
    hipLaunchKernelGGL(k_check_tails, dim3((n_ix + 255) / 256), dim3(256), 0, st, tbl, (const ResultRec*)res, n_ix, d_index,
                       (const SeqDesc*)desc.p, (uint64_t)ix_seq_cap, j.block_size, (const uint32_t*)seqcnt.p);
    return 0;
}

size_t lz4f_mi355x_engine::dec_generic(const DecompressJob& j, const DecodePlan& p, ResultRec* res, BlockOut* tbl, const uint32_t* only_if, uint32_t* path)
{
    constexpr int W = 4;
    hipStream_t st = (hipStream_t)stream; const uint32_t n_max = p.n_max;
    if (p.mode == 'f') {
        unsigned long long* prof = (unsigned long long*)(sw.prof ? prof_buf() : nullptr);
        const bool indexed = only_if != nullptr;
        if (p.windowed) {
            *path |= LZ4F_MI355X_PATH_WINDOW;
            if (!indexed && seqcnt.ensure(256)) return make_err(LZ4F_ERROR_allocation_failed);
            uint32_t* fb = (uint32_t*)seqcnt.p + (indexed ? 16 : 0);
            hipLaunchKernelGGL(k_decode_linked, dim3(1), dim3(64 * LK_WAVES), 0, st, j.d_frame, j.d_dst, j.dst_cap, tbl,
                               (const ResultRec*)res, n_max, j.block_size, j.hist0, fb, only_if);
            only_if = fb;
            uint32_t dbg[3] = {0, 0, 0};
            if (sw.prof && prof_read(st, dbg, fb, 12)) fprintf(stderr, "k_decode_linked: fallback %u why %u block %u\n", dbg[0], dbg[1], dbg[2]);
        }
        *path |= LZ4F_MI355X_PATH_FUSED;
        if (!indexed && !j.linked && !sw.no_density_probe) {
            if (density.ensure(64)) return make_err(LZ4F_ERROR_allocation_failed);
            hipLaunchKernelGGL(k_density_probe, dim3(1), dim3(64), 0, st, j.d_frame, (uint64_t)j.frame_cap, (const BlockOut*)tbl, (const ResultRec*)res, n_max, (uint32_t*)density.p);
            if (p.relay) {
                *path |= LZ4F_MI355X_PATH_WORKGROUP_PER_BLOCK;
                hipLaunchKernelGGL((k_decode_blocks_relay<RELAY_W, RELAY_S>), dim3(n_max), dim3(64 * (RELAY_W + RELAY_S + 3)), 0, st, j.d_frame, j.d_dst, tbl, (const ResultRec*)res, n_max, (uint64_t)j.frame_cap,
                                   (const uint32_t*)density.p);
            } else
                hipLaunchKernelGGL((k_decode_blocks<W>), dim3((n_max + W - 1) / W), dim3(64 * W), 0, st, j.d_frame, j.d_dst, j.dst_cap, tbl, (const ResultRec*)res,
                                   n_max, 0u, j.block_size, j.hist0, (uint64_t)j.frame_cap, (const uint32_t*)density.p);
            only_if = (const uint32_t*)density.p + 1;
            *path |= LZ4F_MI355X_PATH_WAVE_PER_BLOCK;
        }
        auto fused = [&](auto cfg) {
            using C = decltype(cfg);
            hipLaunchKernelGGL(k_decode_blocks_fused<C>, dim3(j.linked ? 1u : n_max), dim3(64 * C::WAVES), 0, st, j.d_frame, j.d_dst, j.dst_cap, tbl,
                               (const ResultRec*)res, n_max, j.linked ? 1u : 0u, j.block_size, j.hist0, prof, only_if);
        };
        if (p.small) fused(FzCfg<4>()); else fused(FzCfg<8>());
    } else {
        *path |= LZ4F_MI355X_PATH_WAVE_PER_BLOCK;
        hipLaunchKernelGGL((k_decode_blocks<W>), dim3(j.linked ? 1u : (n_max + W - 1) / W), dim3(64 * W), sw.dblk_lds, st, j.d_frame, j.d_dst, j.dst_cap, tbl, (const ResultRec*)res,
                           n_max, j.linked ? 1u : 0u, j.block_size, j.hist0, (uint64_t)j.frame_cap);
    }
    return 0;
}

size_t lz4f_mi355x_engine::dec_finish(const DecompressJob& j, const DecodePlan& p, ResultRec* res, BlockOut* tbl, const uint32_t* ix_flags, uint32_t path)
{
    hipStream_t st = (hipStream_t)stream; const uint32_t n_max = p.n_max;
    tick(7, false);
    if (n_max && !p.given && j.block_size && j.dst_cap % j.block_size != 0) {
        if (tight.ensure((size_t)65536 + j.block_size + 64)) return make_err(LZ4F_ERROR_allocation_failed);
        hipLaunchKernelGGL(k_redo_tight_block, dim3(1), dim3(64), 0, st, j.d_frame, (uint64_t)j.frame_cap, j.d_dst, (uint64_t)j.dst_cap, tbl,
                           (const ResultRec*)res, n_max, j.linked ? 1u : 0u, j.block_size, (uint64_t)j.hist0, (uint8_t*)tight.p);
    }
    const bool check_here = n_max <= 64;
    if (n_max && !check_here) hipLaunchKernelGGL(k_finish_check, dim3((n_max + 255) / 256), dim3(256), 0, st, (const BlockOut*)tbl, (const ResultRec*)res, n_max, j.linked ? 1u : 0u, j.block_size, (uint32_t*)bad.p);
    hipLaunchKernelGGL(k_finish_decode, dim3(1), dim3(64), 0, st, j.d_dst, tbl, res, n_max, j.linked ? 1u : 0u, j.block_size,
                       (const uint32_t*)bad.p, j.block_checksum ? 1u : 0u, path, ix_flags, check_here ? 1u : 0u, (uint64_t)j.dst_cap);
    if (j.content_checksum && !p.given && !sw.no_content_check)
        hipLaunchKernelGGL(k_xxh32_content, dim3(1), dim3(64), 0, st, (const uint8_t*)j.d_dst, 0ull, (uint8_t*)j.d_frame, res, 1u);
    tick(7, true);
    return 0;
}

size_t lz4f_mi355x_engine::launch_decompress(const DecompressJob& j, lz4f_mi355x_result* d_res)
{
    HIP_TRY(hipSetDevice(device));
    hipStream_t st = (hipStream_t)stream;
    if (!d_res) { if (res.ensure(sizeof(ResultRec))) return make_err(LZ4F_ERROR_allocation_failed); d_res = (lz4f_mi355x_result*)res.p; }
    if (bad.ensure(64)) return make_err(LZ4F_ERROR_allocation_failed);
    ResultRec* r = (ResultRec*)d_res;
    const DecodePlan p = decode_plan(j, sw, device_cus(device));
    uint32_t path = 0;
    for (int i = 4; i < 10; i++) ev_used[i] = false;
    ev_used[11] = false;
    if (aux_pending) { HIP_TRY(hipStreamWaitEvent(st, (hipEvent_t)ev_join, 0)); aux_pending = false; }
    struct AuxJoin {
        lz4f_mi355x_engine* e; hipStream_t st;
        ~AuxJoin() { if (e->aux_pending && hipStreamWaitEvent(st, (hipEvent_t)e->ev_join, 0) == hipSuccess) e->aux_pending = false; }
    } aux_join{this, st};
    tick(11, false);
    BlockOut* tbl;
    if (size_t e = dec_table(j, p, r, &tbl, &path)) return e;
    const uint32_t* ix_flags = nullptr;
    if (p.n_max) {
        if (j.block_checksum) { if (size_t e = dec_checksums(j, p, r, tbl)) return e; }
        tick(6, false);
        IndexSrc ix;
        if (size_t e = dec_index(j, p, r, tbl, &ix, &path)) return e;
        if (size_t e = dec_indexed(j, p, r, tbl, ix, &ix_flags, &path)) return e;
        if (size_t e = dec_generic(j, p, r, tbl, ix_flags, &path)) return e;
        tick(6, true);
    }
    if (aux_pending) { HIP_TRY(hipStreamWaitEvent(st, (hipEvent_t)ev_join, 0)); aux_pending = false; }
    if (size_t e = dec_finish(j, p, r, tbl, ix_flags, path)) return e;
    tick(11, true);
    HIP_TRY(hipGetLastError());
    return 0;
}


constexpr uint32_t BATCH_GRID = 8192;

static size_t batch_begin(lz4f_mi355x_engine* e, const char* call, bool pointers_ok)
{
    if (!pointers_ok) { set_last_error("%s: null pointer", call); return make_err(LZ4F_ERROR_GENERIC); }
    if (hipSetDevice(e->device) != hipSuccess) { set_last_error("hipSetDevice failed"); return make_err(LZ4F_ERROR_GENERIC); }
    if (e->aux_pending) { HIP_TRY(hipStreamWaitEvent((hipStream_t)e->stream, (hipEvent_t)e->ev_join, 0)); e->aux_pending = false; }
    return 0;
}
static size_t batch_end(const char* call)
{
    if (hipGetLastError() != hipSuccess) { set_last_error("%s: launch failed", call); return make_err(LZ4F_ERROR_GENERIC); }
    return 0;
}
static uint64_t batch_table_cap(uint32_t n_frames, uint64_t shared)
{
    return std::min<uint64_t>((uint64_t)n_frames + shared + 1, 0xFFFFFFF0ull);
}
static dim3 batch_grid(uint64_t items, uint32_t per_wg, uint32_t most = BATCH_GRID)
{
    return dim3((uint32_t)std::min<uint64_t>((items + per_wg - 1) / per_wg, most));
}
struct Carve {
    DevBuf& buf;
    size_t end = 0;
    size_t take(size_t bytes, size_t align = 1) { const size_t at = (end + align - 1) & ~(align - 1); end = at + bytes; return at; }
    int ensure() { return buf.ensure(end); }
    template <typename T> T* at(size_t off) const { return (T*)((uint8_t*)buf.p + off); }
};

extern "C" {

const char* lz4f_mi355x_last_error(void) { return lz4f::last_error(); }

int lz4f_mi355x_device_count(void)
{
    int n = 0;
    if (hipGetDeviceCount(&n) != hipSuccess) return 0;
    return n;
}

size_t lz4f_mi355x_set_device(int device)
{
    int n = lz4f_mi355x_device_count();
    if (device < 0 || device >= n) { set_last_error("device %d out of range (%d devices)", device, n); return make_err(LZ4F_ERROR_GENERIC); }
    lz4f::t_device = device;
    return 0;
}

size_t lz4f_mi355x_engine_create(lz4f_mi355x_engine** out, int device, void* hipStream, int borrowStream)
{
    if (!out) return make_err(LZ4F_ERROR_GENERIC);
    return new_engine(out, device, hipStream, borrowStream != 0);
}
size_t lz4f_mi355x_engine_free(lz4f_mi355x_engine* e) { delete e; return 0; }
void lz4f_mi355x_release_engines(void) { lz4f::release_idle_engines(); }
void* lz4f_mi355x_host_alloc(size_t size)
{
    void* p = nullptr;
    if (hipSetDevice(lz4f::selected_device()) != hipSuccess || hipHostMalloc(&p, size ? size : 1, hipHostMallocPortable) != hipSuccess) { (void)hipGetLastError(); set_last_error("hipHostMalloc(%zu) failed", size); return nullptr; }
    return p;
}
void lz4f_mi355x_host_free(void* p) { if (p) (void)hipHostFree(p); }
void* lz4f_mi355x_engine_stream(lz4f_mi355x_engine* e) { return e ? e->stream : nullptr; }

size_t lz4f_mi355x_engine_set_deterministic(lz4f_mi355x_engine* e, int enable)
{
    if (!e) return make_err(LZ4F_ERROR_GENERIC);
    if (enable) e->sw.e1_solo |= 1u; else e->sw.e1_solo &= ~1u;
    return 0;
}
size_t lz4f_mi355x_engine_set_timing(lz4f_mi355x_engine* e, int enable)
// ... 272 lines not shown
```

lz4_frame_conduit_amd/csrc/engine.hpp:

```cpp
#pragma once
#include <stddef.h>
#include <stdint.h>
#include <functional>
#include <string>
#include <vector>

#include "../../include/lz4f_mi355x.h"
#include "records.hpp"

namespace lz4f {

inline size_t make_err(int code) { return (size_t)-(ptrdiff_t)code; }
inline bool   is_err(size_t v) { return v > make_err(LZ4F_ERROR_maxCode); }
const char*   err_name(size_t v);
void          set_last_error(const char* fmt, ...);
const char*   last_error();

struct Xxh32State {
    uint32_t total_len, large, v[4], memsize;
    uint8_t  mem[16];
    void reset(uint32_t seed = 0);
    void update(const void* data, size_t len);
    uint32_t digest() const;
};
uint32_t xxh32_host(const void* data, size_t len, uint32_t seed = 0);

size_t block_size_of(unsigned blockSizeID);
size_t write_frame_header(uint8_t* dst, const LZ4F_preferences_t& p);
size_t compress_bound_internal(size_t srcSize, const LZ4F_preferences_t* prefs, size_t alreadyBuffered);
struct ParsedHeader { LZ4F_frameInfo_t info; size_t header_size; size_t max_block; };
size_t parse_frame_header(const uint8_t* src, size_t n, ParsedHeader* out);

struct DevBuf {
    void* p = nullptr; size_t cap = 0;
    int ensure(size_t n);
    void release();
};
struct PinBuf {
    void* p = nullptr; size_t cap = 0;
    int ensure(size_t n);
    void release();
};

#define HIP_TRY(expr)                                                                                   \
    do {                                                                                                \
        hipError_t e_ = (expr);                                                                         \
        if (e_ != hipSuccess) {                                                                         \
            lz4f::set_last_error("%s failed: %s (%s:%d)", #expr, hipGetErrorString(e_), __FILE__, __LINE__);  \
            return lz4f::make_err(LZ4F_ERROR_GENERIC);                                                  \
        }                                                                                               \
    } while (0)

}

struct lz4f_mi355x_engine {
    int   device = 0;
    void* stream = nullptr;
    bool  own_stream = false;
    lz4f::DevBuf info, recs, table, blk_bytes, res, bad;
    lz4f::DevBuf ixtmp;
    lz4f::DevBuf walkbuf;
    lz4f::DevBuf density;
    lz4f::DevBuf e1_scratch;
    lz4f::DevBuf spx;
    lz4f::DevBuf selfix, selfcnt;
    lz4f::DevBuf pdbuf;
    lz4f::DevBuf tight;
    lz4f::DevBuf postab;
    lz4f::DevBuf desc, seqcnt;
    lz4f::DevBuf d_in, d_out;
    lz4f::DevBuf bframes, btable;
    lz4f::DevBuf mframes, mtable;
    lz4f::DevBuf cframes, cblocks, cchunks;
    lz4f::PinBuf h_in, h_out, h_small;
    struct Switches {
        bool no_index, no_selfindex, no_resolve, no_trace, no_doubling, trace_always, no_groups, no_window, serial_walk, no_trailer, no_content_check, no_density_probe, no_spx, no_overlap, prof, e1_sync, no_selffeed;
        unsigned dense_mode;
        unsigned group_kib;
        unsigned feed_round;
        int chain_gate; char decode_mode; unsigned e1_run, e1_solo, seed, dblk_lds, recs_per_tile, hc_attempts, hc_lazy; unsigned long long wait_ticks;
        void read();
    } sw;
    void*  recs_ctl_clean = nullptr;
    size_t ix_seq_cap = 0;
    bool  timing = false;
    void* ev[24] = {nullptr};
    bool  ev_used[12] = {false};
    void  tick(int slot, bool end, void* on_stream = nullptr);
    void* aux_stream = nullptr; void* ev_fork = nullptr; void* ev_join = nullptr;
    bool  aux_ready();
    bool  aux_pending = false;

    struct CompressJob {
        const uint8_t* d_src; uint64_t src_size; uint64_t first_off;
        uint32_t block_size; bool linked; bool block_checksum; bool endmark;
        bool content_checksum;
        uint8_t header[20]; uint32_t header_size;
        int level;
    };
    static CompressJob make_compress_job(const uint8_t* d_src, uint64_t src_size, uint64_t first_off, uint32_t block_size, bool linked, bool block_checksum,
                                         int level, const LZ4F_preferences_t* frame = nullptr);
    size_t launch_compress(const CompressJob& j, uint8_t* d_dst, uint64_t dst_cap, lz4f_mi355x_result* d_res, lz4f_mi355x_block* d_table,
                           void* d_index = nullptr, size_t index_cap = 0);
    struct DecompressJob {
        const uint8_t* d_frame; uint64_t frame_cap; uint8_t* d_dst; uint64_t dst_cap; uint64_t hist0;
        void* d_index; size_t index_size;
        uint32_t block_size; bool linked; bool block_checksum;
        bool content_checksum;
        const lz4f_mi355x_block* d_table; uint32_t n_blocks;
        bool table_in_place;
        lz4f_mi355x_block* table_direct;
        uint32_t max_blocks;
        const uint64_t* hint_list; uint32_t hint_n;
        uint32_t ix_seqs, ix_entries;
    };
    size_t launch_decompress(const DecompressJob& j, lz4f_mi355x_result* d_res);
    size_t sync();

    size_t compress_blocks_host(const uint8_t* src, size_t n, const uint8_t* hist, size_t hist_len,
                                uint32_t block_size, bool linked, bool block_checksum, uint8_t* dst, size_t dst_cap, size_t* written, int level = 0);
    size_t slab_compress(const uint8_t* src, size_t n, const uint8_t* hist, size_t hist_len, uint32_t block_size, bool linked, bool block_checksum,
                         bool src_pinned, size_t* size, int level = 0);
    size_t slab_fetch(uint8_t* dst, size_t size, size_t d_off, bool dst_pinned);
    size_t compress_block_pinned(const uint8_t* pin_src, size_t hist_len, size_t n, uint32_t block_size, bool linked, bool block_checksum,
                                 uint8_t* pin_dst, size_t dst_cap, size_t* size, int level = 0);
    size_t slab_decode(const uint8_t* frame_part, size_t part_len, const std::vector<lz4f_mi355x_block>& entries, const lz4f::ParsedHeader& ph,
                       const uint8_t* hist, size_t hist_len, bool src_pinned, size_t* got, uint8_t* fetch_to = nullptr, size_t fetch_room = 0);
    size_t decompress_block_host(const uint8_t* payload, uint32_t csize, bool bck, const uint8_t* hist, size_t hist_len,
                                 uint8_t* dst, uint32_t dst_cap, bool linked, uint32_t block_size, uint32_t* decoded);

    ~lz4f_mi355x_engine();

private:
    struct EncodePlan;
    static EncodePlan encode_plan(const CompressJob& j, const Switches& sw, uint32_t cus, bool inband, size_t index_cap);
    size_t enc_workspaces(const EncodePlan& p, bool own_table);
    size_t enc_find(const CompressJob& j, const EncodePlan& p);
    void   enc_layout(const EncodePlan& p, uint8_t* d_dst, uint64_t dst_cap, lz4f::ResultRec* rec, lz4f::BlockOut* tbl, void* d_index);
    void   enc_emit(const CompressJob& j, const EncodePlan& p, uint8_t* d_dst, const lz4f::ResultRec* rec, lz4f::BlockOut* tbl, void* d_index);
    void   enc_tail(const CompressJob& j, const EncodePlan& p, uint8_t* d_dst, uint64_t dst_cap, lz4f::ResultRec* rec, const lz4f::BlockOut* tbl, const void* d_index);

    struct DecodePlan {
        bool given, begin_small;
        uint32_t n_max, n_ix;
        enum Walk { WALK_NONE, WALK_TRAILER, WALK_PARALLEL, WALK_SEEDED, WALK_SERIAL } walk;
        char mode;
        bool ix_by_trailer;
        bool self_index;
        bool windowed, small, relay;
        uint32_t group;
        uint64_t wait_ticks;
    };
    struct IndexSrc {
        enum From { GIVEN, TRAILER, HEADER, SELF_LINKED, SPX } from = GIVEN;
        void* d = nullptr; size_t size = 0;
        uint32_t seqs = 0, entries = 0;
    };
    struct IxRoute { bool selffed, doubling; uint32_t gate; };
    static DecodePlan decode_plan(const DecompressJob& j, const Switches& sw, uint32_t cus);
    static IxRoute ix_route(const DecompressJob& j, const Switches& sw, uint32_t n_ix, uint32_t ix_seqs);
    size_t dec_table(const DecompressJob& j, const DecodePlan& p, lz4f::ResultRec* res, lz4f::BlockOut** tbl, uint32_t* path);
    size_t dec_checksums(const DecompressJob& j, const DecodePlan& p, lz4f::ResultRec* res, lz4f::BlockOut* tbl);
    size_t dec_index(const DecompressJob& j, const DecodePlan& p, lz4f::ResultRec* res, lz4f::BlockOut* tbl, IndexSrc* ix, uint32_t* path);
    size_t dec_self_index(const DecompressJob& j, const DecodePlan& p, lz4f::ResultRec* res, lz4f::BlockOut* tbl, bool spx_walk, IndexSrc* ix);
    size_t dec_indexed(const DecompressJob& j, const DecodePlan& p, lz4f::ResultRec* res, lz4f::BlockOut* tbl, const IndexSrc& ix, const uint32_t** ix_flags, uint32_t* path);
    size_t dec_generic(const DecompressJob& j, const DecodePlan& p, lz4f::ResultRec* res, lz4f::BlockOut* tbl, const uint32_t* only_if, uint32_t* path);
    size_t dec_finish(const DecompressJob& j, const DecodePlan& p, lz4f::ResultRec* res, lz4f::BlockOut* tbl, const uint32_t* ix_flags, uint32_t path);
};

namespace lz4f {
size_t acquire_engine(lz4f_mi355x_engine** out, int device = -1);
void   release_engine(lz4f_mi355x_engine* e);
void   release_idle_engines();
struct EngineLease {
    lz4f_mi355x_engine* e = nullptr;
    size_t get(int device = -1) { return acquire_engine(&e, device); }
    ~EngineLease() { release_engine(e); }
    lz4f_mi355x_engine* operator->() const { return e; }
};
size_t new_engine(lz4f_mi355x_engine** out, int device, void* stream, bool borrow);
int    selected_device();
bool   is_pinned_host(const void* p);
int    bulk_devices();
void   set_bulk_devices(int n);
int    logical_devices();
size_t pipe_compress_blocks(const uint8_t* src, size_t n, uint32_t block_size, bool linked, bool bck, uint8_t* dst, size_t cap, size_t* written,
                            size_t hist_before = 0, int level = 0);
struct FrameCarry { Xxh32State cck; uint64_t out_total = 0; std::vector<uint8_t> hist; FrameCarry() { cck.reset(0); } };
size_t pipe_decompress_frame(const uint8_t* frame, size_t n, const ParsedHeader& ph, uint8_t* flat, size_t flat_cap,
                             const std::function<void(const uint8_t*, size_t)>* sink, size_t* decoded, size_t* consumed, FrameCarry* carry = nullptr);
uint32_t pick_chunk_size(uint32_t block_size);
struct BlockList {
    std::vector<uint64_t> at;
    bool add_blocks(const uint8_t* blocks, size_t n, uint64_t frame_off, bool block_checksum);
};
size_t host_trailer_size(uint64_t frame_size, uint64_t n_blocks);
void   host_write_trailer(uint8_t* dst, uint64_t frame_size, const uint64_t* at, uint32_t n_blocks);
}
```

lz4_frame_conduit_amd/csrc/frame_dev.cuh:

```cuda
#pragma once
#include "common.cuh"
#include "decode.cuh"
#include "decode_relay.cuh"
#include "decode_fused.cuh"
#include "decode_linked.cuh"
#include "encode.cuh"
#include "encode_solo.cuh"
#include "encode_hc.cuh"
#include "decode_indexed.cuh"
#include "decode_spx.cuh"

namespace lz4f {

__device__ __forceinline__ uint32_t xxh32_finish(uint32_t h, const uint8_t* p, uint32_t rem)
{
    while (rem >= 4) { h = rotl32(h + ld32(p) * XP3, 17) * XP4; p += 4; rem -= 4; }
    while (rem > 0) { h = rotl32(h + (*p) * XP5, 11) * XP1; p++; rem--; }
    h ^= h >> 15; h *= XP2; h ^= h >> 13; h *= XP3; h ^= h >> 16;
    return h;
}

__device__ __forceinline__ uint32_t wave_xxh32(const uint8_t* __restrict__ p, uint32_t len)
{
    const uint32_t lane = lane_id();
// ... 70 lines not shown
    const uint32_t lane = lane_id();
    const uint64_t nstripes = len >> 4;
    uint32_t h = XP5;
    if (len >= 16) {
        const uint32_t c = lane & 3u;
        uint32_t v = c == 0 ? XP1 + XP2 : c == 1 ? XP2 : c == 2 ? 0u : 0u - XP1;
        auto fetch = [&](uint64_t s0) -> b16_ua {
            const uint64_t s = s0 + lane < nstripes ? s0 + lane : nstripes - 1;
            return *(const b16_ua*)(p + s * 16);
        };
        auto store = [&](const b16_ua& w, uint32_t half) {
            *(uint4*)((uint8_t*)park + half * 1024u + lane * 16u) = uint4{w.a * XP2, w.b * XP2, w.c * XP2, w.d * XP2};
        };
        b16_ua r0 = fetch(0);            asm volatile("" ::: "memory");
        b16_ua r1 = fetch(WAVE);         asm volatile("" ::: "memory");
        b16_ua r2 = fetch(2 * WAVE);     asm volatile("" ::: "memory");
        b16_ua r3 = fetch(3 * WAVE);     asm volatile("" ::: "memory");
        uint32_t half = 0;
        auto step = [&](const b16_ua& r, uint64_t s0) {
            store(r, half);
            const uint32_t n = (nstripes - s0 < WAVE) ? (uint32_t)(nstripes - s0) : WAVE;
            const uint32_t* q = (const uint32_t*)((const uint8_t*)park + half * 1024u) + c;
            if (n == WAVE) {
#pragma unroll
                for (int i = 0; i < WAVE; i++) { v = rotl32(v + q[i * 4], 13) * XP1; asm("" : "+v"(v)); }
            } else {
                for (uint32_t i = 0; i < n; i++) { v = rotl32(v + q[i * 4], 13) * XP1; asm("" : "+v"(v)); }
            }
            half ^= 1u;
        };
        for (uint64_t s0 = 0; s0 < nstripes; s0 += 4 * WAVE) {
            step(r0, s0); r0 = fetch(s0 + 4 * WAVE);
            if (s0 + WAVE < nstripes) step(r1, s0 + WAVE);
            r1 = fetch(s0 + 5 * WAVE);
            if (s0 + 2 * WAVE < nstripes) step(r2, s0 + 2 * WAVE);
            r2 = fetch(s0 + 6 * WAVE);
            if (s0 + 3 * WAVE < nstripes) step(r3, s0 + 3 * WAVE);
            r3 = fetch(s0 + 7 * WAVE);
        }
        h = rotl32((uint32_t)__builtin_amdgcn_readlane(v, 0), 1) + rotl32((uint32_t)__builtin_amdgcn_readlane(v, 1), 7) +
            rotl32((uint32_t)__builtin_amdgcn_readlane(v, 2), 12) + rotl32((uint32_t)__builtin_amdgcn_readlane(v, 3), 18);
    }
    h += (uint32_t)len;
    const uint64_t done = nstripes << 4;
    return xxh32_finish(h, p + done, (uint32_t)(len - done));
}

constexpr uint32_t XXH_SPREAD_LDS = 36u << 10;
constexpr uint32_t XXH_LANE4_BELOW = 16384;
template <int WAVES_PER_WG>
__global__ __launch_bounds__(64 * WAVES_PER_WG) void k_xxh32_blocks4(uint8_t* frame, BlockOut* __restrict__ table, const ResultRec* __restrict__ res,
                                                                     uint32_t n_max, uint32_t mode, uint32_t* __restrict__ bad)
{
    __shared__ __attribute__((aligned(16))) uint32_t park[WAVES_PER_WG][XXH_PARK / 4];
    const uint32_t wv = uni(threadIdx.x >> 6);
    const uint32_t b = uni(blockIdx.x * WAVES_PER_WG + wv);
    const uint32_t n = res ? res->n_blocks : n_max;
    if (b >= n || b >= n_max) return;
    if (res && res->status != ST_OK) return;
    const uint64_t off = table[b].src_off;
    const uint32_t len = table[b].word & 0x7FFFFFFFu;
    const uint32_t h = lane4_xxh32(frame + off, len, park[wv]);
    if (lane_id() == 0) {
        uint8_t* c = frame + off + len;
        if (mode == 0) st32le(c, h);
        else if (rd32le(c) != h) atomicMin(bad, b);
    }
}

__global__ __launch_bounds__(64) void k_xxh32_content(const uint8_t* __restrict__ data, uint64_t data_len, uint8_t* frame, ResultRec* __restrict__ res, uint32_t mode)
{
    __shared__ __attribute__((aligned(16))) uint32_t park[XXH_PARK / 4];
    if (res->status != ST_OK) return;
    if (mode == 1 && !flg_cck(res->flags)) return;
    const uint64_t len = mode == 0 ? data_len : res->size;
    const uint32_t h = lane4_xxh32(data, len, park);
    if (threadIdx.x == 0) {
        uint8_t* c = frame + (mode == 0 ? res->size : res->consumed) - 4;
        if (mode == 0) st32le(c, h);
        else if (rd32le(c) != h) res->status = ST_CONTENTCK;
    }
}

__global__ __launch_bounds__(64) void k_walk_frame(const uint8_t* __restrict__ frame, uint64_t frame_cap, uint64_t dst_cap,
                             BlockOut* __restrict__ table, uint32_t table_cap, ResultRec* __restrict__ res, const uint32_t* __restrict__ walked = nullptr)
{
    if (threadIdx.x >= WAVE || blockIdx.x != 0) return;
    if (walked && *walked) return;
    const uint32_t lane = lane_id();
    ResultRec r; r.size = 0; r.consumed = 0; r.status = ST_OK; r.n_blocks = 0; r.first_bad_block = 0xFFFFFFFFu; r.flags = 0;
    __shared__ uint32_t ra_sink[WAVE];
    const uint32_t sink0 = uni((uint32_t)(uintptr_t)(lptr_t)ra_sink);
    auto fail = [&](uint32_t st) { asm volatile("s_waitcnt vmcnt(0)" ::: "memory"); r.status = st; *res = r; };
    if (frame_cap < 7) return fail(ST_INCOMPLETE);
    if (is_skippable(rd32le(frame))) {
        if (const uint32_t st = skippable_span(frame, frame_cap, r.consumed)) { r.consumed = 0; return fail(st); }
        r.flags = FLAG_SKIPPABLE; *res = r; return;
    }
    FrameHead h;
    if (const uint32_t st = frame_head_parse(frame, frame_cap, h)) return fail(st);
    const uint32_t flg = h.flg, bs = h.bs, bck = h.bck;
    r.flags = flg;
    uint64_t pos = h.hsize, out = 0;
    uint32_t n = 0;
    if (!frame_word_fits(frame_cap - pos)) return fail(ST_INCOMPLETE);
    uint32_t w = *(const u32_ua*)(frame + pos);
    for (;;) {
        pos += 4;
        if (is_endmark(w)) break;
        uint32_t csz; uint64_t step;
        if (const uint32_t st = frame_block_word(w, bs, bck, frame_cap - pos, csz, step)) return fail(st);
        if (n >= table_cap) return fail(ST_DSTSMALL);
        if (out >= dst_cap) return fail(ST_DSTSMALL);
        table[n].src_off = pos; table[n].dst_off = out; table[n].word = w;
        table[n].dst_size = (uint32_t)((dst_cap - out < bs) ? dst_cap - out : bs);
        out += bs;
        pos += step;
        n++;
        if (!frame_word_fits(frame_cap - pos)) return fail(ST_INCOMPLETE);
        const uint64_t guess = pos + 4 + step + (uint64_t)lane * 128u;
        const bool inside = guess >= 4096u + 4u && guess - 4096u + 4u <= frame_cap;
        const uint8_t* pw = frame + pos;
        const uint8_t* pa = inside ? frame + ((guess - 4096u) & ~(uint64_t)3) : pw;
        uint32_t keep;
        asm volatile("global_load_dword %0, %2, off\n\ts_mov_b32 %1, m0\n\ts_mov_b32 m0, %4\n\ts_nop 0\n\tglobal_load_lds_dword %3, off\n\ts_mov_b32 m0, %1\n\ts_waitcnt vmcnt(1)"
                     : "=&v"(w), "=&s"(keep) : "v"(pw), "v"(pa), "s"(sink0) : "memory");
    }
    asm volatile("s_waitcnt vmcnt(0)" ::: "memory");
    uint32_t tail;
    if (const uint32_t st = frame_end(flg, frame_cap - pos, tail)) return fail(st);
    pos += tail;
    r.n_blocks = n; r.consumed = pos; r.size = h.content;
    *res = r;
}

constexpr uint32_t WK_CHUNK = 65536, WK_SLOTS = 30, WK_HOPS = 3;
struct WalkState {
    uint32_t done;
    uint32_t overflow;
    uint32_t total;
    uint32_t first_end;
    uint32_t first_break;
    uint32_t hsize, bs, bck, flg;
    uint32_t head_ok;
    uint64_t content;
};
struct WalkChunk { uint32_t n; uint32_t off[WK_SLOTS]; uint32_t pad; };

__global__ void k_walk_head(const uint8_t* __restrict__ frame, uint64_t frame_cap, WalkState* __restrict__ ws, uint32_t preset_total = 0)
{
    if (threadIdx.x != 0 || blockIdx.x != 0) return;
    FrameHead h = {};
    const uint32_t st = frame_head_parse(frame, frame_cap, h);
    ws->done = 0; ws->overflow = 0; ws->total = preset_total; ws->first_end = 0xFFFFFFFFu; ws->first_break = 0xFFFFFFFFu;
    ws->hsize = h.hsize; ws->bs = h.bs; ws->bck = h.bck; ws->flg = h.flg; ws->content = h.content;
    ws->head_ok = st == ST_OK ? 1u : 0u;
}

__device__ __forceinline__ bool walk_step(const uint8_t* __restrict__ frame, uint64_t frame_cap, uint32_t bs, uint32_t bck, uint64_t pos, uint64_t& next, bool& end)
{
    if (pos > frame_cap || !frame_word_fits(frame_cap - pos)) return false;
    const uint32_t w = *(const u32_ua*)(frame + pos);
    end = is_endmark(w);
    uint32_t csz; uint64_t step;
    if (frame_block_word(w, bs, bck, frame_cap - pos - 4, csz, step)) return false;
    next = pos + 4 + step;
    return end || frame_word_fits(frame_cap - next);
}

__global__ __launch_bounds__(256) void k_walk_cand(const uint8_t* __restrict__ frame, uint64_t frame_cap, const WalkState* __restrict__ ws,
                                                   WalkChunk* __restrict__ chunks)
{
    __shared__ uint32_t s_n;
    __shared__ uint32_t s_off[WK_SLOTS];
    if (!ws->head_ok) return;
    const uint32_t bs = ws->bs, bck = ws->bck, hsize = ws->hsize;
    const uint64_t c0 = (uint64_t)blockIdx.x * WK_CHUNK;
    if (threadIdx.x == 0) s_n = 0;
    __syncthreads();
    const uint32_t hi_mask = ~((bs << 1) - 1u) & 0x7FFFFFFFu;
    auto load20 = [&](uint64_t p0, uint32_t (&w)[5]) {
        w[0] = w[1] = w[2] = w[3] = w[4] = 0;
        if (p0 + 4 > frame_cap) return;
        if (p0 + 20 <= frame_cap) { const b16_ua t = *(const b16_ua*)(frame + p0); w[0] = t.a; w[1] = t.b; w[2] = t.c; w[3] = t.d; w[4] = *(const u32_ua*)(frame + p0 + 16); }
        else { for (uint32_t k = 0; k < 20 && p0 + k < frame_cap; k++) w[k >> 2] |= (uint32_t)frame[p0 + k] << (8 * (k & 3)); }
    };
    auto scan16 = [&](uint32_t o, const uint32_t (&w)[5]) {
        const uint64_t p0 = c0 + o;
        if (p0 + 4 > frame_cap) return;
        auto zb = [](uint32_t x) { const uint32_t y = x & 0x7F7F7F7Fu; return (y - 0x01010101u) & 0x80808080u; };
        if (((zb(w[0]) & 0x80000000u) | zb(w[1]) | zb(w[2]) | zb(w[3]) | (zb(w[4]) & 0x00808080u)) == 0u) return;
        uint32_t plausible = 0;
#pragma unroll
        for (uint32_t i = 0; i < 16; i++) {
            const uint32_t sh = (i & 3) * 8;
            const uint32_t v = sh ? (w[i >> 2] >> sh) | (w[(i >> 2) + 1] << (32 - sh)) : w[i >> 2];
            plausible |= ((v & hi_mask) == 0 && v != 0) ? 1u << i : 0u;
        }
#pragma unroll 1
        while (plausible) {
            const uint32_t i = (uint32_t)__builtin_ctz(plausible);
            plausible &= plausible - 1;
            const uint64_t p = p0 + i;
            if (p < hsize || p + 4 > frame_cap) continue;
            uint64_t q = p, nx = 0; bool end = false, good = true;
#pragma unroll 1
            for (uint32_t h = 0; h < WK_HOPS && good && !end; h++) { good = walk_step(frame, frame_cap, bs, bck, q, nx, end); if (h == 0 && end) good = false; q = nx; }
            if (!good) continue;
            const uint32_t at = atomicAdd(&s_n, 1u);
            if (at < WK_SLOTS) s_off[at] = o + i;
        }
    };
    constexpr uint32_t STRIDE = 256 * 16;
    for (uint32_t o = threadIdx.x * 16; o < WK_CHUNK; o += 4 * STRIDE) {
        uint32_t wa[5], wb[5], wc[5], wd[5];
        load20(c0 + o, wa); load20(c0 + o + STRIDE, wb); load20(c0 + o + 2 * STRIDE, wc); load20(c0 + o + 3 * STRIDE, wd);
        scan16(o, wa); scan16(o + STRIDE, wb); scan16(o + 2 * STRIDE, wc); scan16(o + 3 * STRIDE, wd);
// ... 94 lines not shown
    const uint32_t n = s_n < WK_SEED_LIST ? s_n : WK_SEED_LIST;
    for (uint32_t j = t; j < n; j += 256) {
        const uint32_t o = s_list[j];
        uint64_t c = pp + o, nx = 0; bool end = false, good = true;
#pragma unroll 1
        for (uint32_t h = 0; h < WK_SEED_HOPS && good && !end; h++) { good = walk_step(frame, frame_cap, bs, bck, c, nx, end); if (h == 0 && end) good = false; c = nx; }
        if (good) atomicMin(&s_best, o);
    }
    __syncthreads();
    if (t == 0 && s_best != 0xFFFFFFFFu) atomicMin(&seeds[s], (unsigned long long)(pp + s_best));
}
__global__ __launch_bounds__(WK_SEEDS) void k_walk_chains(const uint8_t* __restrict__ frame, uint64_t frame_cap, WalkState* __restrict__ ws,
                                                          const unsigned long long* __restrict__ seeds, uint64_t* __restrict__ list, uint32_t list_cap)
{
    __shared__ uint64_t s_seed[WK_SEEDS + 1];
    __shared__ uint32_t s_cnt[WK_SEEDS];
    __shared__ uint64_t s_pos[WK_LANE_CAP][WK_SEEDS];
    if (!ws->head_ok) return;
    const uint32_t bs = ws->bs, bck = ws->bck, t = threadIdx.x;
    s_seed[t] = seeds[t];
    if (t == 0) s_seed[WK_SEEDS] = WK_NOSEED;
    __syncthreads();
    uint64_t start = s_seed[t];
    for (uint32_t k = 0; k < t; k++) if (s_seed[k] != WK_NOSEED && s_seed[k] >= start) start = WK_NOSEED;
    uint64_t stop = WK_NOSEED;
    for (uint32_t k = t + 1; k < WK_SEEDS; k++) if (s_seed[k] != WK_NOSEED && s_seed[k] > start) { stop = s_seed[k]; break; }
    uint64_t p = start; uint32_t c = 0; bool over = false;
    while (p != WK_NOSEED && p < stop) {
        uint64_t nx = 0; bool end = false;
        if (!walk_step(frame, frame_cap, bs, bck, p, nx, end) || end) break;
        if (c >= WK_LANE_CAP) { over = true; break; }
        s_pos[c][t] = p;
        c++; p = nx;
    }
    s_cnt[t] = over ? 0xFFFFFFFFu : c;
    __syncthreads();
    uint32_t base = 0, tot = 0; bool any_over = false;
    for (uint32_t k = 0; k < WK_SEEDS; k++) { if (s_cnt[k] == 0xFFFFFFFFu) { any_over = true; break; } if (k == t) base = tot; tot += s_cnt[k]; }
    if (any_over || tot > list_cap) { if (t == 0) ws->overflow = 1; return; }
    for (uint32_t i = 0; i < c; i++) list[base + i] = s_pos[i][t];
    if (t == 0) ws->total = tot;
}

__global__ __launch_bounds__(256) void k_walk_mark(const uint8_t* __restrict__ frame, uint64_t frame_cap, const WalkState* __restrict__ ws,
                                                   const uint64_t* __restrict__ list, uint32_t* __restrict__ mark)
{
    if (!ws->head_ok || ws->overflow) return;
    const uint32_t total = ws->total, bs = ws->bs, bck = ws->bck;
    for (uint32_t i = blockIdx.x * 256 + threadIdx.x; i < total; i += gridDim.x * 256) {
        uint64_t nx = 0; bool end = false;
        if (!walk_step(frame, frame_cap, bs, bck, list[i], nx, end) || end) continue;
        uint32_t lo = i + 1, hi = total;
        while (lo < hi) { const uint32_t mid = (lo + hi) >> 1; if (list[mid] < nx) lo = mid + 1; else hi = mid; }
        if (lo < total && list[lo] == nx) mark[lo] = 1;
    }
}
__global__ __launch_bounds__(1024) void k_walk_filter(WalkState* __restrict__ ws, const uint64_t* __restrict__ list, const uint32_t* __restrict__ mark, uint64_t* __restrict__ list2)
{
    __shared__ uint32_t s_part[1024];
    __shared__ uint32_t s_carry;
    if (!ws->head_ok || ws->overflow) return;
    const uint32_t t = threadIdx.x, total = ws->total;
    if (t == 0) s_carry = 0;
    __syncthreads();
    for (uint32_t base = 0; base < total; base += 1024) {
        const uint32_t i = base + t;
        const uint32_t k = (i < total && (i == 0 || mark[i])) ? 1u : 0u;
        s_part[t] = k;
        __syncthreads();
        for (uint32_t off = 1; off < 1024; off <<= 1) {
            const uint32_t a = t >= off ? s_part[t - off] : 0u;
            __syncthreads();
            s_part[t] += a;
            __syncthreads();
        }
        if (k) list2[s_carry + s_part[t] - 1] = list[i];
        __syncthreads();
        if (t == 1023) s_carry += s_part[1023];
        __syncthreads();
    }
    if (t == 0) ws->total = s_carry;
}

__global__ __launch_bounds__(256) void k_walk_link(const uint8_t* __restrict__ frame, uint64_t frame_cap, uint64_t dst_cap, WalkState* __restrict__ ws,
                                                   const uint64_t* __restrict__ list, BlockOut* __restrict__ table, uint32_t table_cap)
{
    if (!ws->head_ok || ws->overflow) return;
    const uint32_t total = ws->total;
    const uint32_t bs = ws->bs, bck = ws->bck;
    for (uint32_t i = blockIdx.x * 256 + threadIdx.x; i < total; i += gridDim.x * 256) {
        const uint64_t p = list[i];
        uint64_t nx = 0; bool end = false;
        bool ok = walk_step(frame, frame_cap, bs, bck, p, nx, end) && !end;
        bool last = false;
        if (ok) {
            uint64_t n2 = 0; bool e2 = false;
            const bool ok2 = walk_step(frame, frame_cap, bs, bck, nx, n2, e2);
            last = ok2 && e2;
            ok = last || (i + 1 < total && list[i + 1] == nx);
        }
        if (!ok) atomicMin(&ws->first_break, i);
        else if (last) atomicMin(&ws->first_end, i);
        if (ok && i < table_cap) {
            const uint64_t out = (uint64_t)i * bs;
            const uint32_t w = *(const u32_ua*)(frame + p);
            table[i].src_off = p + 4; table[i].dst_off = out; table[i].word = w;
            table[i].dst_size = out >= dst_cap ? 0u : (uint32_t)((dst_cap - out < bs) ? dst_cap - out : bs);
        }
    }
}

__global__ void k_walk_verdict(const uint8_t* __restrict__ frame, uint64_t frame_cap, uint64_t dst_cap, WalkState* __restrict__ ws,
                               const uint64_t* __restrict__ list, uint32_t table_cap, ResultRec* __restrict__ res)
{
    if (threadIdx.x != 0 || blockIdx.x != 0) return;
    if (!ws->head_ok || ws->overflow) return;
    const uint32_t hsize = ws->hsize, bs = ws->bs, bck = ws->bck, flg = ws->flg;
    uint32_t n = 0; uint64_t pos = hsize;
    if (ws->total == 0 || list[0] != hsize) {
        if (frame_cap - pos < 4 || *(const u32_ua*)(frame + pos) != 0) return;
        pos += 4;
    } else {
        const uint32_t e = ws->first_end;
        if (e == 0xFFFFFFFFu || ws->first_break <= e || e >= table_cap) return;
        if ((uint64_t)e * bs >= dst_cap) return;
        n = e + 1;
        const uint64_t p = list[e];
        pos = p + 4 + word_size(*(const u32_ua*)(frame + p)) + 4 * bck + 4;
    }
    uint32_t tail;
    if (frame_end(flg, frame_cap - pos, tail)) return;
    pos += tail;
    ResultRec r; r.size = ws->content; r.consumed = pos; r.status = ST_OK; r.n_blocks = n; r.first_bad_block = 0xFFFFFFFFu; r.flags = flg;
    *res = r;
    ws->done = 1;
}

struct TrailerPlan { uint64_t at, list_at, ix_at, ix_bytes, total; uint32_t n_list, ok; };

__global__ void k_trailer_plan(uint8_t* __restrict__ dst, uint64_t dst_cap, ResultRec* __restrict__ res, uint32_t n_blocks, const void* __restrict__ ix,
                               uint64_t ix_fixed, TrailerPlan* __restrict__ plan)
{
    if (threadIdx.x != 0 || blockIdx.x != 0) return;
    TrailerPlan p; memset(&p, 0, sizeof(p));
    if (res->status == ST_OK && n_blocks) {
        const uint64_t F = res->size;
        const IxHeader* hd = (const IxHeader*)ix;
        const bool with_ix = ix && hd->magic == IX_MAGIC;
        p.at = F;
        p.list_at = (F + 8 + 15) & ~(uint64_t)15;
        p.n_list = (n_blocks + 1) & ~1u;
        p.ix_at = p.list_at + (uint64_t)p.n_list * 8;
        p.ix_bytes = with_ix ? (ix_fixed + (uint64_t)hd->total_entries * sizeof(IxEntry) + 15) & ~(uint64_t)15 : 0;
        p.total = p.ix_at + p.ix_bytes + sizeof(TrailerFoot) - F;
        p.ok = (F + p.total <= dst_cap && p.total - 8 < 0xFFFFFFFFull) ? 1u : 0u;
        if (p.ok) {
            uint8_t* t = dst + F;
            const uint32_t sz = (uint32_t)(p.total - 8);
            st32le(t, TR_MAGIC); st32le(t + 4, sz);
            for (uint64_t q = F + 8; q < p.list_at; q++) dst[q] = 0;
            TrailerFoot f{with_ix ? hd->total_seqs : 0u, with_ix ? hd->total_entries : 0u, 0u, 0u, TR_FOOT, n_blocks, p.total};
            memcpy(dst + p.ix_at + p.ix_bytes, &f, sizeof(f));
            res->size = F + p.total;
        } else res->status = ST_DSTSMALL;
    }
    *plan = p;
}
__global__ __launch_bounds__(256) void k_trailer_copy(uint8_t* __restrict__ dst, const TrailerPlan* __restrict__ plan, const BlockOut* __restrict__ table,
                                                      uint32_t n_blocks, const void* __restrict__ ix)
{
    const TrailerPlan p = *plan;
    if (!p.ok) return;
    const uint64_t t = (uint64_t)blockIdx.x * 256 + threadIdx.x, step = (uint64_t)gridDim.x * 256;
    uint64_t* list = (uint64_t*)(dst + p.list_at);
    for (uint64_t i = t; i < p.n_list; i += step) list[i] = i < n_blocks ? table[i].src_off - 4 : 0;
    const uint4* s = (const uint4*)ix; uint4* d = (uint4*)(dst + p.ix_at);
    for (uint64_t i = t; i < p.ix_bytes / 16; i += step) d[i] = s[i];
}

__global__ void k_init_result(ResultRec* res, uint32_t n_blocks, uint32_t flags)
{
    if (threadIdx.x == 0 && blockIdx.x == 0) {
        res->size = 0; res->consumed = 0; res->status = ST_OK; res->n_blocks = n_blocks; res->first_bad_block = 0xFFFFFFFFu; res->flags = flags;
    }
}
__device__ __forceinline__ void check_table_entries(const BlockOut* __restrict__ table, uint32_t n, uint64_t frame_cap, uint64_t dst_cap, uint32_t block_size,
                                                    uint32_t bck, uint32_t linked, ResultRec* res)
{
    for (uint32_t i = blockIdx.x * 256 + threadIdx.x; i < n; i += gridDim.x * 256) {
        const BlockOut e = table[i];
        const uint64_t csz = e.word & 0x7FFFFFFFu;
        bool bad = csz > block_size || e.src_off > frame_cap || frame_cap - e.src_off < csz + 4ull * bck;
        bad = bad || e.dst_off > dst_cap || e.dst_size > block_size || (!linked && dst_cap - e.dst_off < e.dst_size);
        if (!bad && i + 1 < n) {
            const BlockOut x = table[i + 1];
            bad = x.src_off < e.src_off + csz + 4ull * bck + 4ull;
            if (!linked) bad = bad || x.dst_off < e.dst_off + e.dst_size;
        }
        if (bad) { atomicMin(&res->first_bad_block, i); atomicMax(&res->status, (uint32_t)ST_GENERIC); }
    }
}
__global__ __launch_bounds__(256) void k_check_table(const BlockOut* __restrict__ table, uint32_t n, uint64_t frame_cap, uint64_t dst_cap, uint32_t block_size,
                                                     uint32_t bck, uint32_t linked, ResultRec* __restrict__ res)
{
    check_table_entries(table, n, frame_cap, dst_cap, block_size, bck, linked, res);
}
__global__ __launch_bounds__(256) void k_begin_table_small(const BlockOut* __restrict__ table, uint32_t n, uint64_t frame_cap, uint64_t dst_cap, uint32_t block_size,
                                                           uint32_t bck, uint32_t linked, ResultRec* res, uint32_t* __restrict__ w)
{
    if (threadIdx.x == 0) { res->size = 0; res->consumed = 0; res->status = ST_OK; res->n_blocks = n; res->first_bad_block = 0xFFFFFFFFu; res->flags = 0u; }
    if (threadIdx.x < 8) w[threadIdx.x] = threadIdx.x < 2 ? 0xFFFFFFFFu : 0u;
    __threadfence_block(); __syncthreads();
    check_table_entries(table, n, frame_cap, dst_cap, block_size, bck, linked, res);
}
__global__ void k_set_block(BlockOut* t, BlockOut e) { if (threadIdx.x == 0 && blockIdx.x == 0) *t = e; }

__global__ __launch_bounds__(64) void k_density_probe(const uint8_t* __restrict__ frame, uint64_t frame_cap, const BlockOut* __restrict__ table,
                                                      const ResultRec* __restrict__ res, uint32_t n_max, uint32_t* __restrict__ flags)
{
    const uint32_t lane = lane_id();
    uint32_t seqs = 0, bytes = 0;
    const uint32_t n = res->n_blocks < n_max ? res->n_blocks : n_max;
    if (res->status == ST_OK && n) {
        const uint32_t b = (uint32_t)(((uint64_t)lane * n) >> 6);
        const BlockOut e = table[b];
        const uint32_t csz = e.word & 0x7FFFFFFFu;
        if (!(e.word >> 31) && csz >= 64 && e.src_off + csz <= frame_cap && (lane == 0 || b != (uint32_t)(((uint64_t)(lane - 1) * n) >> 6))) {
            const uint8_t* in = frame + e.src_off;
            const uint32_t want = n >= 64u ? 512u : n >= 4u ? 512u * (64u / n) : 8192u;
            const uint32_t lim = csz < want ? csz - 16u : want - 16u;
            uint32_t pos = 0, first_end = 0;
            while (pos < lim && seqs < 2048u) {
                const uint32_t t = in[pos++];
                uint32_t lit = t >> 4;
                if (lit == 15) { uint32_t x; do { x = pos < lim ? in[pos] : 0u; pos++; lit += x; } while (x == 255u && pos < lim); }
                pos += lit + 2;
                if ((t & 15u) == 15u) { uint32_t x; do { x = pos < lim ? in[pos] : 0u; pos++; } while (x == 255u && pos < lim); }
                seqs++;
                if (seqs == 1) first_end = pos;
            }
            if (seqs > 1) { seqs -= 1; bytes = (pos < want + 512u ? pos : want + 512u) - (first_end < pos ? first_end : pos); } else { seqs = 0; bytes = 0; }
        }
    }
    uint32_t st = seqs, bt = bytes;
#pragma unroll
    for (int sft = 1; sft < 64; sft <<= 1) { st += __shfl_xor(st, sft); bt += __shfl_xor(bt, sft); }
    if (lane == 0) { const bool dense = st != 0 && bt < 24u * st; flags[0] = dense ? 1u : 0u; flags[1] = dense ? 0u : 1u; flags[2] = st ? bt / st : 0u; }
}

template <int WAVES_PER_WG>
__global__ __launch_bounds__(64 * WAVES_PER_WG, 8) void k_decode_blocks(const uint8_t* __restrict__ frame, uint8_t* dst, uint64_t dst_cap,
                                                                     BlockOut* __restrict__ table, const ResultRec* __restrict__ res,
                                                                     uint32_t n_max, uint32_t linked, uint32_t block_size, uint64_t hist0,
                                                                     uint64_t frame_cap, const uint32_t* __restrict__ only_if = nullptr)
{
    __shared__ uint32_t expand[WAVES_PER_WG][64];
    const uint32_t w = uni(blockIdx.x * WAVES_PER_WG + (threadIdx.x >> 6));
    if (res->status != ST_OK) return;
    if (only_if && *only_if == 0) return;
    const uint32_t n = res->n_blocks < n_max ? res->n_blocks : n_max;
    const uint32_t lane = lane_id();
    if (!linked) {
        if (w >= n) return;
        const BlockOut e = table[w];
        const uint32_t csz = e.word & 0x7FFFFFFFu;
        int32_t got;
        if (e.word >> 31) {
            if (csz > e.dst_size) got = -2;
            else { wave_copy_disjoint(dst + e.dst_off, frame + e.src_off, csz); got = (int32_t)csz; }
        } else {
            got = wave_decode_block_win<true>(frame + e.src_off, csz, frame_cap - e.src_off, dst + e.dst_off, e.dst_size, expand[uni(threadIdx.x >> 6)]);
        }
        if (lane == 0) table[w].dst_size = (uint32_t)got;
        return;
    }
    if (w != 0) return;
    uint64_t out = 0;
    for (uint32_t b = 0; b < n; b++) {
        const BlockOut e = table[b];
        const uint32_t csz = e.word & 0x7FFFFFFFu;
        const uint32_t room = (uint32_t)((dst_cap - out < block_size) ? dst_cap - out : block_size);
        int32_t got;
        if (e.word >> 31) {
            if (csz > room) got = -2;
            else { wave_copy_disjoint(dst + out, frame + e.src_off, csz); got = (int32_t)csz; }
        } else {
            got = wave_decode_block(frame + e.src_off, csz, dst + out, room, out + hist0);
        }
        if (lane == 0) { table[b].dst_off = out; table[b].dst_size = (uint32_t)got; }
        if (got < 0) {
            for (uint32_t k = b + 1 + lane; k < n; k += WAVE) table[k].dst_size = 0;
            break;
        }
        out += (uint32_t)got;
    }
}

__global__ __launch_bounds__(64) void k_redo_tight_block(const uint8_t* __restrict__ frame, uint64_t frame_cap, uint8_t* dst, uint64_t dst_cap,
                                                         BlockOut* __restrict__ table, const ResultRec* __restrict__ res, uint32_t n_max,
                                                         uint32_t linked, uint32_t block_size, uint64_t hist0, uint8_t* __restrict__ scratch)
{
    if (res->status != ST_OK) return;
    const uint32_t n = res->n_blocks < n_max ? res->n_blocks : n_max;
    if (n == 0) return;
    const uint32_t b = n - 1, lane = lane_id();
    const BlockOut e = table[b];
    if ((int32_t)e.dst_size >= 0 || (e.word >> 31) || e.dst_off > dst_cap || dst_cap - e.dst_off >= block_size) return;
    if (linked && b > 0 && (int32_t)table[b - 1].dst_size < 0) return;
    const uint32_t csz = e.word & 0x7FFFFFFFu;
    if (csz == 0 || csz > block_size || e.src_off + csz > frame_cap) return;
    const uint32_t h = linked ? (uint32_t)(e.dst_off + hist0 < 65536u ? e.dst_off + hist0 : 65536u) : 0u;
    uint8_t* const out = scratch + 65536u;
    for (uint32_t i = lane; i < h; i += WAVE) out[(int64_t)i - h] = dst[(int64_t)e.dst_off + i - h];
    __threadfence(); __syncthreads();
    const int32_t got = wave_decode_block(frame + e.src_off, csz, out, block_size, h);
    __threadfence(); __syncthreads();
    const uint64_t room = dst_cap - e.dst_off;
    if (got >= 0 && (uint64_t)got <= room) wave_copy_disjoint(dst + e.dst_off, out, (uint32_t)got);
    if (lane == 0) table[b].dst_size = got < 0 ? (uint32_t)-3 : (uint64_t)got <= room ? (uint32_t)got : (uint32_t)-2;
}

__global__ __launch_bounds__(256) void k_finish_check(const BlockOut* __restrict__ table, const ResultRec* __restrict__ res, uint32_t n_max,
                                                      uint32_t linked, uint32_t block_size, uint32_t* __restrict__ w)
{
    if (res->status != ST_OK) return;
    const uint32_t n = res->n_blocks < n_max ? res->n_blocks : n_max;
    const uint32_t b = blockIdx.x * 256u + threadIdx.x, lane = lane_id();
    const bool in = b < n;
    const uint32_t sz = in ? table[b].dst_size : 0u;
    const uint64_t at = in ? table[b].dst_off : 0ull;
    const bool bad = in && (int32_t)sz < 0;
    if (bad) atomicMin(&w[1], b);
    const bool moves = in && !linked && (at != (uint64_t)b * block_size || (b + 1 < n && sz != block_size));
    const uint64_t mv = __ballot(moves);
    uint32_t sum = bad ? 0u : sz;
#pragma unroll
    for (int sft = 1; sft < 64; sft <<= 1) sum += __shfl_xor(sum, sft);
    if (lane == 0) {
        if (mv) atomicOr(&w[2], 1u);
        if (sum) atomicAdd((unsigned long long*)(w + 4), (unsigned long long)sum);
    }
}

__global__ __launch_bounds__(64) void k_finish_decode(uint8_t* dst, BlockOut* __restrict__ table, ResultRec* res, uint32_t n_max,
                                                      uint32_t linked, uint32_t block_size, const uint32_t* __restrict__ bad_ck, uint32_t with_ck,
                                                      uint32_t plan = 0, const uint32_t* __restrict__ ix_flags = nullptr, uint32_t check_here = 0,
                                                      uint64_t dst_cap = ~0ull)
{
    if (lane_id() == 0) res->flags = (res->flags & 0xFFFu) | (plan << 12) | ((ix_flags && *ix_flags) ? (LZ4F_MI355X_PATH_INDEX_DROPPED << 12) : 0u);
    if (res->status != ST_OK) return;
    const uint32_t n = res->n_blocks < n_max ? res->n_blocks : n_max;
    uint32_t n_scan = n;
    const uint32_t lane = lane_id();
    uint32_t w1 = 0xFFFFFFFFu, w2 = 0u; uint64_t w45 = 0;
    if (check_here) {
        const bool in = lane < n;
        const uint32_t sz = in ? table[lane].dst_size : 0u;
        const uint64_t at = in ? table[lane].dst_off : 0ull;
        const bool bad = in && (int32_t)sz < 0;
        const uint64_t bm = __ballot(bad);
        if (bm) w1 = (uint32_t)__builtin_ctzll(bm);
        w2 = __ballot(in && !linked && (at != (uint64_t)lane * block_size || (lane + 1 < n && sz != block_size))) ? 1u : 0u;
        uint64_t sum = bad ? 0u : sz;
#pragma unroll
        for (int sft = 1; sft < 64; sft <<= 1) sum += __shfl_xor(sum, sft);
        w45 = sum;
    } else { w1 = bad_ck[1]; w2 = bad_ck[2]; w45 = *(const uint64_t*)(bad_ck + 4); }
    const uint32_t first_bad = w1 < n ? w1 : 0xFFFFFFFFu;
    const uint32_t bad_kind = first_bad != 0xFFFFFFFFu ? table[first_bad].dst_size : 0u;
    const uint32_t ck = with_ck ? bad_ck[0] : 0xFFFFFFFFu;
    if (ck != 0xFFFFFFFFu && ck <= first_bad) {
        if (lane == 0) { res->status = ST_BLOCKCK; res->first_bad_block = ck; }
        return;
    }
    if (first_bad != 0xFFFFFFFFu) {
        if (lane == 0) { res->status = block_fail_status((int32_t)bad_kind, table[first_bad].dst_off, dst_cap, block_size); res->first_bad_block = first_bad; }
        return;
    }
    uint64_t out = w45;
    bool in_place = w2 == 0;
    if (!in_place) { out = 0; in_place = true; }
    else n_scan = 0;
    for (uint32_t b0 = 0; b0 < n_scan; b0 += WAVE) {
        const uint32_t b = b0 + lane;
        const uint32_t sz = b < n ? table[b].dst_size : 0u;
        const uint64_t at = b < n ? table[b].dst_off : 0ull;
        uint64_t incl = sz;
        for (uint32_t d = 1; d < WAVE; d <<= 1) { const uint64_t t = __shfl_up(incl, d); if (lane >= d) incl += t; }
        if (!linked && __ballot(b < n && at != out + incl - sz)) { in_place = false; break; }
        out += __shfl(incl, WAVE - 1);
    }
    if (!in_place) {
        out = 0;
        for (uint32_t b = 0; b < n; b++) {
            const uint64_t at = table[b].dst_off; const uint32_t sz = table[b].dst_size;
            if (at != out) {
                for (uint32_t o = 0; o < sz; o += 1024) {
                    const uint32_t m = (sz - o < 1024) ? sz - o : 1024;
                    uint8_t v = 0; b16_ua v16;
                    const uint32_t i = lane * 16;
                    const bool full = i + 16 <= m;
                    if (full) v16 = *(const b16_ua*)(dst + at + o + i);
                    if (full) *(b16_ua*)(dst + out + o + i) = v16;
                    for (uint32_t j = (m & ~15u) + lane; j < m; j += WAVE) { v = dst[at + o + j]; dst[out + o + j] = v; }
                }
                if (lane == 0) table[b].dst_off = out;
            }
            out += sz;
        }
    }
    if (lane == 0) {
        const uint64_t declared = res->size;
        res->size = out;
        if (const uint32_t st = frame_size_status(res->flags, declared, out)) res->status = st;
    }
}

}
```

Measured before the change: 749.8.

## Fuse layout, index, trailer and finish kernels using last-workgroup ticket

Merges the per-block layout and index kernels with their scans into one kernel. A last-arriving workgroup, chosen by an atomic ticket with agent-scope fences, performs the serial scan. The trailer plan and copy kernels become one, and finish_check is fused with finish_decode the same way. The 1024-wide LDS Hillis-Steele scans are replaced by wave-level scans plus a 16-entry reduction. This cuts kernel launches and barriers per frame, at the cost of ticket and fence synchronization and the risk of subtle memory-ordering bugs.

```diff
diff --git a/lz4_frame_conduit_amd/csrc/common.cuh b/lz4_frame_conduit_amd/csrc/common.cuh
--- a/lz4_frame_conduit_amd/csrc/common.cuh
+++ b/lz4_frame_conduit_amd/csrc/common.cuh
@@ -147,6 +147,27 @@
     return v;
 }
 
+__device__ __forceinline__ bool wg_arrives_last(uint32_t* ticket, uint32_t n_wgs, uint32_t* s_last)
+{
+    asm volatile("s_waitcnt vmcnt(0)" ::: "memory");
+    __syncthreads();
+    if (threadIdx.x == 0) {
+        __builtin_amdgcn_fence(__ATOMIC_RELEASE, "agent");
+        asm volatile("s_waitcnt vmcnt(0)" ::: "memory");
+        const uint32_t t = __hip_atomic_fetch_add(ticket, 1u, __ATOMIC_RELAXED, __HIP_MEMORY_SCOPE_AGENT);
+        const bool last = t + 1 == n_wgs;
+        if (last) {
+            __hip_atomic_store(ticket, 0u, __ATOMIC_RELAXED, __HIP_MEMORY_SCOPE_AGENT);
+            __builtin_amdgcn_fence(__ATOMIC_ACQUIRE, "agent");
+            asm volatile("s_waitcnt vmcnt(0)" ::: "memory");
+        }
+        *s_last = last ? 1u : 0u;
+    }
+    __syncthreads();
+    return *s_last != 0;
+}
+__device__ __forceinline__ uint32_t ld_agent(const uint32_t* p) { return __hip_atomic_load(p, __ATOMIC_RELAXED, __HIP_MEMORY_SCOPE_AGENT); }
+
 __device__ __forceinline__ uint32_t dpp_excl_scan_max(uint32_t v)
 {
     const uint32_t incl = dpp_incl_scan_max(v);
diff --git a/lz4_frame_conduit_amd/csrc/decode_indexed.cuh b/lz4_frame_conduit_amd/csrc/decode_indexed.cuh
--- a/lz4_frame_conduit_amd/csrc/decode_indexed.cuh
+++ b/lz4_frame_conduit_amd/csrc/decode_indexed.cuh
@@ -21,10 +21,9 @@
     lo = pt_load8(in, pos, readable); hi = pt_load8(in, pos + 8, readable);
 }
 
-__global__ void k_check_index(const void* __restrict__ ix, uint64_t ix_size, uint32_t n_max, uint32_t chunks_per_block, uint32_t chunk_size,
-                              uint64_t seq_cap, uint32_t* __restrict__ flags, const ResultRec* __restrict__ res = nullptr)
-{
-    if (threadIdx.x != 0 || blockIdx.x != 0) return;
+__device__ __forceinline__ void check_index(const void* __restrict__ ix, uint64_t ix_size, uint32_t n_max, uint32_t chunks_per_block, uint32_t chunk_size,
+                                            uint64_t seq_cap, uint32_t* __restrict__ flags, const ResultRec* __restrict__ res)
+{
     const uint32_t n_blocks = res ? res->n_blocks : n_max;
     const IxHeader hd = *(const IxHeader*)ix;
     const bool ok = (!res || res->status == ST_OK) && n_blocks != 0 && n_blocks <= n_max && hd.magic == IX_MAGIC && hd.n_blocks == n_blocks && hd.chunks_per_block == chunks_per_block && hd.stride == IX_STRIDE &&
@@ -35,6 +34,12 @@
     flags[8] = ok ? hd.total_entries : 0u;
     flags[9] = ok ? hd.total_seqs : 0u;
     if (!ok) atomicOr(flags, 1u);
+}
+__global__ void k_check_index(const void* __restrict__ ix, uint64_t ix_size, uint32_t n_max, uint32_t chunks_per_block, uint32_t chunk_size,
+                              uint64_t seq_cap, uint32_t* __restrict__ flags, const ResultRec* __restrict__ res = nullptr)
+{
+    if (threadIdx.x != 0 || blockIdx.x != 0) return;
+    check_index(ix, ix_size, n_max, chunks_per_block, chunk_size, seq_cap, flags, res);
 }
 
 __global__ __launch_bounds__(256) void k_check_blocks(const void* __restrict__ ix, const BlockOut* __restrict__ table, const ResultRec* __restrict__ res,
diff --git a/lz4_frame_conduit_amd/csrc/encode.cuh b/lz4_frame_conduit_amd/csrc/encode.cuh
--- a/lz4_frame_conduit_amd/csrc/encode.cuh
+++ b/lz4_frame_conduit_amd/csrc/encode.cuh
@@ -755,7 +755,7 @@
     if (raw) for (uint32_t c = lane; c < nch; c += WAVE) ci[c].flags = ((c + 1 == nch) ? 2u : 0u) | 1u;
     return raw ? (blen | 0x80000000u) : total;
 }
-__device__ __forceinline__ void layout_block(const EncGeom& g, ChunkInfo* __restrict__ info, BlockOut* __restrict__ table, uint32_t* __restrict__ blk_bytes, uint32_t b)
+__device__ __forceinline__ uint32_t layout_block(const EncGeom& g, ChunkInfo* __restrict__ info, BlockOut* __restrict__ table, uint32_t* __restrict__ blk_bytes, uint32_t b)
 {
     const uint64_t bstart = g.first_off + (uint64_t)b * g.block_size;
     const uint32_t blen = (uint32_t)((bstart + g.block_size < g.src_size) ? g.block_size : g.src_size - bstart);
@@ -766,37 +766,28 @@
         table[b].dst_size = blen;
         blk_bytes[b] = 4 + (word & 0x7FFFFFFFu) + 4 * g.block_checksum;
     }
-}
-template <int WAVES_PER_WG>
-__global__ __launch_bounds__(64 * WAVES_PER_WG) void k_layout_blocks(EncGeom g, ChunkInfo* __restrict__ info, BlockOut* __restrict__ table,
-                                                                     uint32_t* __restrict__ blk_bytes)
-{
-    const uint32_t b = uni(blockIdx.x * WAVES_PER_WG + (threadIdx.x >> 6));
-    if (b >= g.n_blocks) return;
-    layout_block(g, info, table, blk_bytes, b);
-}
-
-__device__ __forceinline__ void layout_scan(const EncGeom& g, BlockOut* __restrict__ table, const uint32_t* __restrict__ blk_bytes,
+    return word;
+}
+
+__device__ __forceinline__ bool layout_scan(const EncGeom& g, BlockOut* __restrict__ table, const uint32_t* __restrict__ blk_bytes,
                                             uint8_t* __restrict__ dst, uint64_t dst_cap, ResultRec* __restrict__ res, const uint64_t* __restrict__ recs,
                                             uint64_t* s_part, uint64_t& s_carry)
 {
     const uint32_t t = threadIdx.x;
     if (t == 0) s_carry = g.header_size;
     __syncthreads();
+    const uint32_t wave = t >> 6;
     for (uint32_t base = 0; base < g.n_blocks; base += 1024) {
         const uint32_t b = base + t;
-        const uint64_t v = (b < g.n_blocks) ? blk_bytes[b] : 0;
-        s_part[t] = v;
+        uint32_t wave_total;
+        const uint32_t pre = wave_excl_scan((b < g.n_blocks) ? blk_bytes[b] : 0u, wave_total);
+        if (lane_id() == 0) s_part[wave] = wave_total;
         __syncthreads();
-        for (uint32_t off = 1; off < 1024; off <<= 1) {
-            uint64_t add = (t >= off) ? s_part[t - off] : 0;
-            __syncthreads();
-            s_part[t] += add;
-            __syncthreads();
-        }
-        if (b < g.n_blocks) table[b].src_off = s_carry + s_part[t] - v + 4;
+        uint64_t before = 0, all = 0;
+        for (uint32_t k = 0; k < 16; k++) { const uint64_t x = s_part[k]; all += x; if (k < wave) before += x; }
+        if (b < g.n_blocks) table[b].src_off = s_carry + before + pre + 4;
         __syncthreads();
-        if (t == 1023) s_carry += s_part[1023];
+        if (t == 0) s_carry += all;
         __syncthreads();
     }
     const uint64_t frame_size = s_carry + (g.write_endmark == 2 ? 8 : g.write_endmark ? 4 : 0);
@@ -810,13 +801,7 @@
         res->status = fits ? ST_OK : ST_DSTSMALL; res->n_blocks = g.n_blocks; res->first_bad_block = 0xFFFFFFFFu; res->flags = g.header[4] | ((g.n_chunks && rec_ctl(recs)[1]) ? ENC_POOL_SHORT : 0u);
     }
     if (t == 0 && g.n_chunks) { rec_ctl(recs)[0] = 0ull; rec_ctl(recs)[1] = 0ull; }
-}
-__global__ __launch_bounds__(1024) void k_layout_scan(EncGeom g, BlockOut* __restrict__ table, const uint32_t* __restrict__ blk_bytes,
-                                                      uint8_t* __restrict__ dst, uint64_t dst_cap, ResultRec* __restrict__ res, const uint64_t* __restrict__ recs)
-{
-    __shared__ uint64_t s_part[1024];
-    __shared__ uint64_t s_carry;
-    layout_scan(g, table, blk_bytes, dst, dst_cap, res, recs, s_part, s_carry);
+    return fits;
 }
 
 __device__ __forceinline__ void layout_chunk(const EncGeom& g, ChunkInfo* __restrict__ info, const BlockOut* __restrict__ table,
@@ -841,7 +826,7 @@
 __global__ __launch_bounds__(1024) void k_layout_small(EncGeom g, ChunkInfo* info, BlockOut* table, uint32_t* blk_bytes, uint8_t* __restrict__ dst, uint64_t dst_cap,
                                                        ResultRec* res, const uint64_t* __restrict__ recs)
 {
-    __shared__ uint64_t s_part[1024];
+    __shared__ uint64_t s_part[16];
     __shared__ uint64_t s_carry;
     for (uint32_t b = uni(threadIdx.x >> 6); b < g.n_blocks; b += 16) layout_block(g, info, table, blk_bytes, b);
     __threadfence_block(); __syncthreads();
@@ -872,23 +857,15 @@
     return (const IxEntry*)((const uint8_t*)ix + ix_entries_at(n_blocks, ((const IxHeader*)ix)->chunks_per_block));
 }
 
-template <int WAVES_PER_WG>
-__global__ __launch_bounds__(64 * WAVES_PER_WG) void k_index_blocks(EncGeom g, const ChunkInfo* __restrict__ info, const BlockOut* __restrict__ table,
-                                                                    const ResultRec* __restrict__ res, void* __restrict__ ix, uint64_t ix_capacity)
+__device__ __forceinline__ void index_block(const EncGeom& g, const ChunkInfo* __restrict__ ci, void* __restrict__ ix, uint32_t b, uint32_t nch, bool counted)
 {
     const uint32_t lane = lane_id();
-    const uint32_t b = uni(blockIdx.x * WAVES_PER_WG + (threadIdx.x >> 6));
-    if (b >= g.n_blocks || ix_capacity < ix_entries_at(g.n_blocks, g.chunks_per_block)) return;
     IxBlock* blocks = ix_blocks(ix);
     IxChunk* ck = ix_chunks(ix, g.n_blocks) + (uint64_t)b * g.chunks_per_block;
-    const bool usable = res->status == ST_OK;
-    const BlockOut e = table[b];
-    const ChunkInfo* ci = info + (uint64_t)b * g.chunks_per_block;
-    const uint32_t nch = (e.dst_size + g.chunk_size - 1) / g.chunk_size;
     uint32_t nseq = 0, nent = 0, last = 0xFFFFFFFFu;
     for (uint32_t c0 = 0; c0 < g.chunks_per_block; c0 += WAVE) {
         const uint32_t c = c0 + lane;
-        const uint32_t nr = (c < nch && usable && !(e.word >> 31)) ? ci[c].nrec : 0u;
+        const uint32_t nr = (c < nch && counted) ? ci[c].nrec : 0u;
         uint32_t ts, te;
         const uint32_t ps = wave_excl_scan(nr, ts), pe = wave_excl_scan((nr + IX_STRIDE - 1) / IX_STRIDE, te);
         if (c < g.chunks_per_block) ck[c] = IxChunk{nent + pe, nseq + ps};
@@ -902,63 +879,71 @@
     }
 }
 
-__global__ __launch_bounds__(1024) void k_build_index(EncGeom g, const ChunkInfo* __restrict__ info, const BlockOut* __restrict__ table,
-                                                      const ResultRec* __restrict__ res, void* __restrict__ ix, uint64_t ix_capacity,
-                                                      uint32_t blocks_done = 0)
-{
-    __shared__ uint32_t s_a[1024], s_b[1024];
-    __shared__ uint32_t s_carry_a, s_carry_b;
-    const uint32_t t = threadIdx.x;
-    IxHeader* hd = (IxHeader*)ix;
+__device__ __forceinline__ void index_scan(const EncGeom& g, bool usable, void* __restrict__ ix, uint64_t ix_capacity, uint32_t* s_a, uint32_t* s_b,
+                                           uint32_t& s_carry_a, uint32_t& s_carry_b)
+{
+    const uint32_t t = threadIdx.x, wave = t >> 6;
     IxBlock* blocks = ix_blocks(ix);
-    IxChunk* chunks = ix_chunks(ix, g.n_blocks);
-    const size_t fixed = ix_entries_at(g.n_blocks, g.chunks_per_block);
-    if (ix_capacity < fixed) { if (t == 0 && ix_capacity >= sizeof(IxHeader)) hd->magic = 0; return; }
-    const bool usable = res->status == ST_OK;
-    for (uint32_t b = t; b < g.n_blocks && !blocks_done; b += 1024) {
-        const BlockOut e = table[b];
-        const ChunkInfo* ci = info + (uint64_t)b * g.chunks_per_block;
-        IxChunk* ck = chunks + (uint64_t)b * g.chunks_per_block;
-        const uint32_t nch = (e.dst_size + g.chunk_size - 1) / g.chunk_size;
-        uint32_t nseq = 0, nent = 0, last = 0xFFFFFFFFu;
-        for (uint32_t c0 = 0; c0 < g.chunks_per_block; c0 += 8) {
-            uint32_t nr[8];
-#pragma unroll
-            for (uint32_t k = 0; k < 8; k++) nr[k] = (c0 + k < nch) ? ci[c0 + k].nrec : 0;
-#pragma unroll
-            for (uint32_t k = 0; k < 8; k++) {
-                const uint32_t c = c0 + k;
-                if (c >= g.chunks_per_block) break;
-                ck[c] = IxChunk{nent, nseq};
-                if (usable && !(e.word >> 31) && nr[k]) { nseq += nr[k]; nent += (nr[k] + IX_STRIDE - 1) / IX_STRIDE; last = c; }
-            }
-        }
-        if (last != 0xFFFFFFFFu) { ck[last].ent_off |= 0x80000000u; nseq += 1; }
-        blocks[b].nseq = nseq; blocks[b].nentries = nent;
-    }
-    __syncthreads();
     if (t == 0) { s_carry_a = 0; s_carry_b = 0; }
     __syncthreads();
     for (uint32_t base = 0; base < g.n_blocks; base += 1024) {
         const uint32_t b = base + t;
         const uint32_t va = (b < g.n_blocks) ? blocks[b].nseq : 0, vb = (b < g.n_blocks) ? blocks[b].nentries : 0;
-        s_a[t] = va; s_b[t] = vb;
+        uint32_t ta, tb;
+        const uint32_t pa = wave_excl_scan(va, ta), pb = wave_excl_scan(vb, tb);
+        if (lane_id() == 0) { s_a[wave] = ta; s_b[wave] = tb; }
         __syncthreads();
-        for (uint32_t off = 1; off < 1024; off <<= 1) {
-            const uint32_t aa = (t >= off) ? s_a[t - off] : 0, ab = (t >= off) ? s_b[t - off] : 0;
-            __syncthreads();
-            s_a[t] += aa; s_b[t] += ab;
-            __syncthreads();
-        }
-        if (b < g.n_blocks) { blocks[b].seq_base = s_carry_a + s_a[t] - va; blocks[b].entry_base = s_carry_b + s_b[t] - vb; }
+        uint32_t ba = 0, bb = 0, alla = 0, allb = 0;
+        for (uint32_t k = 0; k < 16; k++) { const uint32_t xa = s_a[k], xb = s_b[k]; alla += xa; allb += xb; if (k < wave) { ba += xa; bb += xb; } }
+        if (b < g.n_blocks) { blocks[b].seq_base = s_carry_a + ba + pa; blocks[b].entry_base = s_carry_b + bb + pb; }
         __syncthreads();
-        if (t == 1023) { s_carry_a += s_a[1023]; s_carry_b += s_b[1023]; }
+        if (t == 0) { s_carry_a += alla; s_carry_b += allb; }
         __syncthreads();
     }
     if (t == 0) {
+        const size_t fixed = ix_entries_at(g.n_blocks, g.chunks_per_block);
         const bool fits = (uint64_t)s_carry_b * sizeof(IxEntry) <= ix_capacity - fixed;
-        *hd = IxHeader{usable && fits ? IX_MAGIC : 0u, g.n_blocks, g.chunks_per_block, s_carry_a, s_carry_b, IX_STRIDE, g.linked ? 1u : 0u, 0u};
-    }
+        *(IxHeader*)ix = IxHeader{usable && fits ? IX_MAGIC : 0u, g.n_blocks, g.chunks_per_block, s_carry_a, s_carry_b, IX_STRIDE, g.linked ? 1u : 0u, 0u};
+    }
+}
+
+constexpr int LI_WAVES = 16;
+__global__ __launch_bounds__(64 * LI_WAVES) void k_layout_index(EncGeom g, ChunkInfo* info, BlockOut* table, uint32_t* blk_bytes,
+                                                               uint8_t* __restrict__ dst, uint64_t dst_cap, ResultRec* res, const uint64_t* recs,
+                                                               void* ix, uint64_t ix_capacity, uint32_t laid_out, uint32_t* ticket)
+{
+    __shared__ uint64_t s_part[16];
+    __shared__ uint64_t s_carry;
+    __shared__ uint32_t s_a[16], s_b[16];
+    __shared__ uint32_t s_carry_a, s_carry_b, s_last;
+    const uint32_t b = uni(blockIdx.x * LI_WAVES + (threadIdx.x >> 6));
+    const bool ix_room = ix && ix_capacity >= ix_entries_at(g.n_blocks, g.chunks_per_block);
+    if (b < g.n_blocks) {
+        uint32_t word, blen;
+        if (laid_out) { word = table[b].word; blen = table[b].dst_size; }
+        else {
+            word = layout_block(g, info, table, blk_bytes, b);
+            const uint64_t bstart = g.first_off + (uint64_t)b * g.block_size;
+            blen = (uint32_t)((bstart + g.block_size < g.src_size) ? g.block_size : g.src_size - bstart);
+        }
+        if (ix_room) index_block(g, info + (uint64_t)b * g.chunks_per_block, ix, b, (blen + g.chunk_size - 1) / g.chunk_size,
+                                 !(word >> 31) && (!laid_out || res->status == ST_OK));
+    }
+    if (!wg_arrives_last(ticket, gridDim.x, &s_last)) return;
+    const uint32_t t = threadIdx.x;
+    bool usable;
+    if (laid_out) usable = res->status == ST_OK;
+    else { usable = layout_scan(g, table, blk_bytes, dst, dst_cap, res, recs, s_part, s_carry); __syncthreads(); }
+    if (!ix) return;
+    if (!ix_room) { if (t == 0 && ix_capacity >= sizeof(IxHeader)) ((IxHeader*)ix)->magic = 0; return; }
+    if (!usable && !laid_out) {
+        IxBlock* blocks = ix_blocks(ix);
+        IxChunk* ck = ix_chunks(ix, g.n_blocks);
+        for (uint32_t i = t; i < g.n_blocks; i += 1024) { blocks[i].nseq = 0; blocks[i].nentries = 0; }
+        for (uint32_t i = t; i < g.n_chunks; i += 1024) ck[i] = IxChunk{0u, 0u};
+        __syncthreads();
+    }
+    index_scan(g, usable, ix, ix_capacity, s_a, s_b, s_carry_a, s_carry_b);
 }
 
 __device__ __forceinline__ void emit_len_ext(uint8_t* p, uint32_t v )
diff --git a/lz4_frame_conduit_amd/csrc/engine.hip b/lz4_frame_conduit_amd/csrc/engine.hip
--- a/lz4_frame_conduit_amd/csrc/engine.hip
+++ b/lz4_frame_conduit_amd/csrc/engine.hip
@@ -168,7 +168,7 @@
     (void)hipSetDevice(device);
     (void)hipStreamSynchronize((hipStream_t)stream);
     desc.release(); seqcnt.release(); spx.release(); selfix.release(); selfcnt.release(); postab.release(); pdbuf.release(); tight.release();
-    info.release(); recs.release(); e1_scratch.release(); walkbuf.release(); density.release(); ixtmp.release(); table.release(); blk_bytes.release(); res.release(); bad.release();
+    info.release(); recs.release(); e1_scratch.release(); walkbuf.release(); density.release(); ixtmp.release(); table.release(); blk_bytes.release(); res.release(); ctl.release();
     d_in.release(); d_out.release(); bframes.release(); btable.release(); mframes.release(); mtable.release(); cframes.release(); cblocks.release(); cchunks.release();
     h_in.release(); h_out.release(); h_small.release();
     for (int i = 0; i < 24; i++) if (ev[i]) (void)hipEventDestroy((hipEvent_t)ev[i]);
@@ -194,6 +194,19 @@
     if (!ev_fork) { if (hipEventCreateWithFlags(&a, hipEventDisableTiming) != hipSuccess) { (void)hipGetLastError(); return false; } ev_fork = a; }
     if (!ev_join) { if (hipEventCreateWithFlags(&b, hipEventDisableTiming) != hipSuccess) { (void)hipGetLastError(); return false; } ev_join = b; }
     return true;
+}
+
+size_t lz4f_mi355x_engine::ctl_words(CtlWords** out)
+{
+    if (!ctl.p) {
+        if (ctl.ensure(sizeof(CtlWords))) return make_err(LZ4F_ERROR_allocation_failed);
+        CtlWords* w = (CtlWords*)ctl.p;
+        if (hipMemsetAsync(w, 0, sizeof(CtlWords), (hipStream_t)stream) != hipSuccess || hipMemsetAsync(&w->first_end, 0xFF, 8, (hipStream_t)stream) != hipSuccess) {
+            ctl.release(); set_last_error("control words: hipMemsetAsync failed"); return make_err(LZ4F_ERROR_GENERIC);
+        }
+    }
+    *out = (CtlWords*)ctl.p;
+    return 0;
 }
 
 size_t lz4f_mi355x_engine::sync()
@@ -302,7 +315,7 @@
     p.ixtmp_bytes = inband ? p.index_cap + 64 : 0;
     p.info_bytes = (size_t)(g.n_chunks + 1) * sizeof(ChunkInfo); p.recs_bytes = (size_t)(rec_pool_at(g.n_chunks) + g.rec_pool) * 8;
     p.blk_bytes = (size_t)(g.n_blocks + 1) * 4; p.table_bytes = (size_t)(g.n_blocks + 1) * sizeof(BlockOut);
-    p.res_bytes = sizeof(ResultRec) + sizeof(TrailerPlan) + 64;
+    p.res_bytes = sizeof(ResultRec) + 64;
     return p;
 }
 
@@ -346,22 +359,17 @@
     return 0;
 }
 
-void lz4f_mi355x_engine::enc_layout(const EncodePlan& p, uint8_t* d_dst, uint64_t dst_cap, ResultRec* rec, BlockOut* tbl, void* d_index)
-{
-    constexpr int W = 4;
+void lz4f_mi355x_engine::enc_layout(const EncodePlan& p, uint8_t* d_dst, uint64_t dst_cap, ResultRec* rec, BlockOut* tbl, void* d_index, CtlWords* cw)
+{
     hipStream_t st = (hipStream_t)stream; const EncGeom& g = p.g;
     if (p.layout_small)
         hipLaunchKernelGGL(k_layout_small, dim3(1), dim3(1024), 0, st, g, (ChunkInfo*)info.p, tbl, (uint32_t*)blk_bytes.p, d_dst, dst_cap, rec, (const uint64_t*)recs.p);
-    else {
-        if (g.n_blocks) hipLaunchKernelGGL((k_layout_blocks<W>), dim3((g.n_blocks + W - 1) / W), dim3(64 * W), 0, st, g, (ChunkInfo*)info.p, tbl, (uint32_t*)blk_bytes.p);
-        hipLaunchKernelGGL(k_layout_scan, dim3(1), dim3(1024), 0, st, g, tbl, (const uint32_t*)blk_bytes.p, d_dst, dst_cap, rec, (const uint64_t*)recs.p);
-        if (g.n_chunks) hipLaunchKernelGGL(k_layout_chunks, dim3((g.n_chunks + 255) / 256), dim3(256), 0, st, g, (ChunkInfo*)info.p, (const BlockOut*)tbl, d_dst, (const ResultRec*)rec);
-    }
+    if (!p.layout_small || d_index)
+        hipLaunchKernelGGL(k_layout_index, dim3(std::max<uint32_t>((g.n_blocks + LI_WAVES - 1) / LI_WAVES, 1u)), dim3(64 * LI_WAVES), 0, st, g, (ChunkInfo*)info.p, tbl,
+                           (uint32_t*)blk_bytes.p, d_dst, dst_cap, rec, (const uint64_t*)recs.p, d_index, (uint64_t)p.index_cap, p.layout_small ? 1u : 0u, &cw->layout_ticket);
+    if (!p.layout_small && g.n_chunks)
+        hipLaunchKernelGGL(k_layout_chunks, dim3((g.n_chunks + 255) / 256), dim3(256), 0, st, g, (ChunkInfo*)info.p, (const BlockOut*)tbl, d_dst, (const ResultRec*)rec);
     if (g.n_chunks) recs_ctl_clean = recs.p;
-    if (d_index) {
-        if (g.n_blocks) hipLaunchKernelGGL((k_index_blocks<W>), dim3((g.n_blocks + W - 1) / W), dim3(64 * W), 0, st, g, (const ChunkInfo*)info.p, (const BlockOut*)tbl, (const ResultRec*)rec, d_index, (uint64_t)p.index_cap);
-        hipLaunchKernelGGL(k_build_index, dim3(1), dim3(1024), 0, st, g, (const ChunkInfo*)info.p, (const BlockOut*)tbl, (const ResultRec*)rec, d_index, (uint64_t)p.index_cap, 1u);
-    }
 }
 
 void lz4f_mi355x_engine::enc_emit(const CompressJob& j, const EncodePlan& p, uint8_t* d_dst, const ResultRec* rec, BlockOut* tbl, void* d_index)
@@ -390,12 +398,9 @@
     hipStream_t st = (hipStream_t)stream; const EncGeom& g = p.g;
     if (j.endmark && j.content_checksum)
         hipLaunchKernelGGL(k_xxh32_content, dim3(1), dim3(64), 0, st, j.d_src + j.first_off, (uint64_t)(j.src_size - j.first_off), d_dst, rec, 0u);
-    if (p.inband && g.n_blocks) {
-        TrailerPlan* plan = (TrailerPlan*)((uint8_t*)res.p + sizeof(ResultRec) + 32);
-        hipLaunchKernelGGL(k_trailer_plan, dim3(1), dim3(64), 0, st, d_dst, dst_cap, rec, g.n_blocks, d_index,
-                           (uint64_t)ix_entries_at(g.n_blocks, g.chunks_per_block), plan);
-        hipLaunchKernelGGL(k_trailer_copy, dim3(256), dim3(256), 0, st, d_dst, (const TrailerPlan*)plan, tbl, g.n_blocks, d_index);
-    }
+    if (p.inband && g.n_blocks)
+        hipLaunchKernelGGL(k_trailer, dim3(256), dim3(256), 0, st, d_dst, dst_cap, rec, tbl, g.n_blocks, g.block_checksum ? 1u : 0u,
+                           g.write_endmark == 2 ? 8u : g.write_endmark ? 4u : 0u, d_index, (uint64_t)ix_entries_at(g.n_blocks, g.chunks_per_block));
 }
 
 lz4f_mi355x_engine::CompressJob lz4f_mi355x_engine::make_compress_job(const uint8_t* d_src, uint64_t src_size, uint64_t first_off, uint32_t block_size,
@@ -417,6 +422,8 @@
     if (inband && ((uintptr_t)d_dst & 15) != 0) { set_last_error("in-band index: the frame buffer must be 16-byte aligned"); return make_err(LZ4F_ERROR_GENERIC); }
     if (p.too_large) { set_last_error("input too large for one call"); return make_err(LZ4F_ERROR_srcSize_tooLarge); }
     if (size_t e = enc_workspaces(p, !d_table)) return e;
+    CtlWords* cw;
+    if (size_t e = ctl_words(&cw)) return e;
     if (inband) d_index = ixtmp.p;
     BlockOut* tbl = (BlockOut*)(d_table ? d_table : table.p);
     ResultRec* r = (ResultRec*)(d_res ? d_res : res.p);
@@ -429,7 +436,7 @@
         tick(0, true);
     }
     tick(1, false);
-    enc_layout(p, d_dst, dst_cap, r, tbl, d_index);
+    enc_layout(p, d_dst, dst_cap, r, tbl, d_index, cw);
     tick(1, true);
     if (p.g.n_chunks) enc_emit(j, p, d_dst, r, tbl, d_index);
     enc_tail(j, p, d_dst, dst_cap, r, tbl, d_index);
@@ -474,17 +481,19 @@
 }
 static bool prof_read(hipStream_t st, void* to, const void* from, size_t n) { return hipStreamSynchronize(st) == hipSuccess && hipMemcpy(to, from, n, hipMemcpyDeviceToHost) == hipSuccess; }
 
-size_t lz4f_mi355x_engine::dec_table(const DecompressJob& j, const DecodePlan& p, ResultRec* res, BlockOut** tbl_out, uint32_t* path)
+size_t lz4f_mi355x_engine::dec_table(const DecompressJob& j, const DecodePlan& p, ResultRec* res, BlockOut** tbl_out, uint32_t* path, const OpenIx& oi)
 {
     hipStream_t st = (hipStream_t)stream; const uint32_t n_max = p.n_max;
     BlockOut* tbl = (BlockOut*)j.table_direct;
     if (!tbl) { if (table.ensure((size_t)(n_max + 1) * sizeof(BlockOut))) return make_err(LZ4F_ERROR_allocation_failed); tbl = (BlockOut*)table.p; }
+    CtlWords* cw = (CtlWords*)ctl.p;
+    bool verdict_set = p.begin_small;
     if (p.given) {
         if (!j.table_in_place && !j.table_direct)
             HIP_TRY(hipMemcpyAsync(tbl, j.d_table, (size_t)n_max * sizeof(BlockOut), hipMemcpyDeviceToDevice, st));
         if (p.begin_small)
             hipLaunchKernelGGL(k_begin_table_small, dim3(1), dim3(256), 0, st, (const BlockOut*)tbl, n_max, (uint64_t)j.frame_cap, (uint64_t)j.dst_cap,
-                               j.block_size, j.block_checksum ? 1u : 0u, j.linked ? 1u : 0u, res, (uint32_t*)bad.p);
+                               j.block_size, j.block_checksum ? 1u : 0u, j.linked ? 1u : 0u, res, cw->verdict);
         else {
             hipLaunchKernelGGL(k_init_result, dim3(1), dim3(64), 0, st, res, n_max, 0u);
             if (n_max) hipLaunchKernelGGL(k_check_table, dim3(std::min<uint32_t>((n_max + 255) / 256, 1024u)), dim3(256), 0, st, (const BlockOut*)tbl, n_max, (uint64_t)j.frame_cap, (uint64_t)j.dst_cap,
@@ -497,11 +506,10 @@
         uint32_t lgrid = std::min<uint32_t>((uint32_t)((list_cap + 255) / 256), 4096u);
         WalkState* ws = nullptr; const uint64_t* list = nullptr;
         if (p.walk == DecodePlan::WALK_TRAILER) {
-            if (walkbuf.ensure(256)) return make_err(LZ4F_ERROR_allocation_failed);
-            ws = (WalkState*)walkbuf.p;
-            hipLaunchKernelGGL(k_walk_head, dim3(1), dim3(64), 0, st, j.d_frame, j.frame_cap, ws, j.hint_n);
-            list = j.hint_list;
             lgrid = std::min<uint32_t>((j.hint_n + 255) / 256, 4096u);
+            hipLaunchKernelGGL(k_open_trailer, dim3(std::max(lgrid, 1u)), dim3(256), 0, st, j.d_frame, (uint64_t)j.frame_cap, (uint64_t)j.dst_cap, cw, j.hint_list, j.hint_n,
+                               tbl, n_max, res, oi);
+            verdict_set = true;
             *path |= LZ4F_MI355X_PATH_TRAILER;
         } else if (p.walk == DecodePlan::WALK_PARALLEL) {
             const uint32_t n_chunks = (uint32_t)((j.frame_cap + WK_CHUNK - 1) / WK_CHUNK);
@@ -540,12 +548,13 @@
             if (sw.prof && p.walk == DecodePlan::WALK_PARALLEL && prof_read(st, &h, ws, sizeof(h))) fprintf(stderr, "parallel walk: done %u overflow %u candidates %u first_end %u first_break %u (header ok %u, hsize %u, block %u)\n", h.done, h.overflow, h.total, h.first_end, h.first_break, h.head_ok, h.hsize, h.bs);
             if (sw.prof && p.walk == DecodePlan::WALK_SEEDED && prof_read(st, &h, ws, sizeof(h))) fprintf(stderr, "seeded walk: done %u overflow %u entries %u first_end %u first_break %u\n", h.done, h.overflow, h.total, h.first_end, h.first_break);
         }
-        hipLaunchKernelGGL(k_walk_frame, dim3(1), dim3(64), 0, st, j.d_frame, j.frame_cap, j.dst_cap, tbl, n_max, res, list ? (const uint32_t*)&ws->done : nullptr);
+        if (p.walk != DecodePlan::WALK_TRAILER)
+            hipLaunchKernelGGL(k_walk_frame, dim3(1), dim3(64), 0, st, j.d_frame, j.frame_cap, j.dst_cap, tbl, n_max, res, list ? (const uint32_t*)&ws->done : nullptr);
         tick(4, true);
     }
-    if (!p.begin_small) {
-        HIP_TRY(hipMemsetAsync(bad.p, 0xFF, 8, st));
-        HIP_TRY(hipMemsetAsync((uint8_t*)bad.p + 8, 0, 24, st));
+    if (!verdict_set) {
+        HIP_TRY(hipMemsetAsync(cw->verdict, 0xFF, 8, st));
+        HIP_TRY(hipMemsetAsync(cw->verdict + 2, 0, 24, st));
     }
     *tbl_out = tbl;
     return 0;
@@ -560,9 +569,9 @@
     if (beside) { HIP_TRY(hipEventRecord((hipEvent_t)ev_fork, st)); HIP_TRY(hipStreamWaitEvent(xs, (hipEvent_t)ev_fork, 0)); }
     tick(5, false, xs);
     if (n_max < XXH_LANE4_BELOW)
-        hipLaunchKernelGGL((k_xxh32_blocks4<1>), dim3(n_max), dim3(64), beside ? (12u << 10) : XXH_SPREAD_LDS, xs, (uint8_t*)j.d_frame, tbl, res, n_max, 1u, (uint32_t*)bad.p);
+        hipLaunchKernelGGL((k_xxh32_blocks4<1>), dim3(n_max), dim3(64), beside ? (12u << 10) : XXH_SPREAD_LDS, xs, (uint8_t*)j.d_frame, tbl, res, n_max, 1u, ((CtlWords*)ctl.p)->verdict);
     else
-        hipLaunchKernelGGL((k_xxh32_blocks<W>), dim3((n_max + W - 1) / W), dim3(64 * W), 0, xs, (uint8_t*)j.d_frame, tbl, res, n_max, 1u, (uint32_t*)bad.p);
+        hipLaunchKernelGGL((k_xxh32_blocks<W>), dim3((n_max + W - 1) / W), dim3(64 * W), 0, xs, (uint8_t*)j.d_frame, tbl, res, n_max, 1u, ((CtlWords*)ctl.p)->verdict);
     tick(5, true, xs);
     if (beside) { HIP_TRY(hipEventRecord((hipEvent_t)ev_join, xs)); aux_pending = true; }
     return 0;
@@ -637,20 +646,31 @@
     return 0;
 }
 
-size_t lz4f_mi355x_engine::dec_indexed(const DecompressJob& j, const DecodePlan& p, ResultRec* res, BlockOut* tbl, const IndexSrc& ix, const uint32_t** ix_flags, uint32_t* path)
-{
+size_t lz4f_mi355x_engine::dec_indexed_ws(const DecodePlan& p, const IndexSrc& ix, bool* runs)
+{
+    *runs = false;
     if (!ix.d) return 0;
-    hipStream_t st = (hipStream_t)stream; void* d_index = ix.d;
-    const uint32_t chunk = pick_chunk_size(j.block_size), cpb = j.block_size / chunk, n_ix = p.n_ix;
     if ((size_t)ix.seqs + 4096 > ix_seq_cap) ix_seq_cap = (size_t)ix.seqs + ix.seqs / 4 + 4096;
     if (!ix.seqs) return 0;
     const size_t dsrc_at = (ix_seq_cap + 64) * sizeof(SeqDesc);
     if (desc.ensure(dsrc_at + (ix_seq_cap + 64) * 4) || seqcnt.ensure(256 + (size_t)p.n_max * (8 + 8 * IXL_PUB))) return make_err(LZ4F_ERROR_allocation_failed);
-    HIP_TRY(hipMemsetAsync(seqcnt.p, 0, 256 + (j.linked ? (size_t)p.n_max * 8 : 0), st));
+    *runs = true;
+    return 0;
+}
+size_t lz4f_mi355x_engine::dec_indexed(const DecompressJob& j, const DecodePlan& p, ResultRec* res, BlockOut* tbl, const IndexSrc& ix, bool opened, const uint32_t** ix_flags, uint32_t* path)
+{
+    bool runs = opened;
+    if (!opened) { if (size_t e = dec_indexed_ws(p, ix, &runs)) return e; }
+    if (!runs) return 0;
+    hipStream_t st = (hipStream_t)stream; void* d_index = ix.d;
+    const uint32_t chunk = pick_chunk_size(j.block_size), cpb = j.block_size / chunk, n_ix = p.n_ix;
+    const size_t dsrc_at = (ix_seq_cap + 64) * sizeof(SeqDesc);
+    if (!opened) HIP_TRY(hipMemsetAsync(seqcnt.p, 0, 256 + (j.linked ? (size_t)p.n_max * 8 : 0), st));
     unsigned long long* iprof = (unsigned long long*)(sw.prof ? prof_buf() : nullptr);
     tick(8, false);
-    hipLaunchKernelGGL(k_check_index, dim3(1), dim3(64), 0, st, (const void*)d_index, (uint64_t)ix.size, n_ix, cpb, chunk,
-                       (uint64_t)ix_seq_cap, (uint32_t*)seqcnt.p, (const ResultRec*)res);
+    if (!opened)
+        hipLaunchKernelGGL(k_check_index, dim3(1), dim3(64), 0, st, (const void*)d_index, (uint64_t)ix.size, n_ix, cpb, chunk,
+                           (uint64_t)ix_seq_cap, (uint32_t*)seqcnt.p, (const ResultRec*)res);
     hipLaunchKernelGGL(k_check_blocks, dim3((n_ix + 255) / 256), dim3(256), 0, st, (const void*)d_index, (const BlockOut*)tbl, (const ResultRec*)res, n_ix,
                        (uint32_t*)seqcnt.p);
     const IxRoute r = ix_route(j, sw, n_ix, ix.seqs);
@@ -797,9 +817,15 @@
                            (const ResultRec*)res, n_max, j.linked ? 1u : 0u, j.block_size, (uint64_t)j.hist0, (uint8_t*)tight.p);
     }
     const bool check_here = n_max <= 64;
-    if (n_max && !check_here) hipLaunchKernelGGL(k_finish_check, dim3((n_max + 255) / 256), dim3(256), 0, st, (const BlockOut*)tbl, (const ResultRec*)res, n_max, j.linked ? 1u : 0u, j.block_size, (uint32_t*)bad.p);
-    hipLaunchKernelGGL(k_finish_decode, dim3(1), dim3(64), 0, st, j.d_dst, tbl, res, n_max, j.linked ? 1u : 0u, j.block_size,
-                       (const uint32_t*)bad.p, j.block_checksum ? 1u : 0u, path, ix_flags, check_here ? 1u : 0u, (uint64_t)j.dst_cap);
+    CtlWords* cw = (CtlWords*)ctl.p;
+    if (p.walk == DecodePlan::WALK_TRAILER && !check_here)
+        hipLaunchKernelGGL(k_finish, dim3((n_max + 255) / 256), dim3(256), 0, st, j.d_dst, tbl, res, n_max, j.linked ? 1u : 0u, j.block_size, cw,
+                           j.block_checksum ? 1u : 0u, path, ix_flags, (uint64_t)j.dst_cap);
+    else {
+        if (n_max && !check_here) hipLaunchKernelGGL(k_finish_check, dim3((n_max + 255) / 256), dim3(256), 0, st, (const BlockOut*)tbl, (const ResultRec*)res, n_max, j.linked ? 1u : 0u, j.block_size, cw->verdict);
+        hipLaunchKernelGGL(k_finish_decode, dim3(1), dim3(64), 0, st, j.d_dst, tbl, res, n_max, j.linked ? 1u : 0u, j.block_size,
+                           (const uint32_t*)cw->verdict, j.block_checksum ? 1u : 0u, path, ix_flags, check_here ? 1u : 0u, (uint64_t)j.dst_cap);
+    }
     if (j.content_checksum && !p.given && !sw.no_content_check)
         hipLaunchKernelGGL(k_xxh32_content, dim3(1), dim3(64), 0, st, (const uint8_t*)j.d_dst, 0ull, (uint8_t*)j.d_frame, res, 1u);
     tick(7, true);
@@ -811,7 +837,8 @@
     HIP_TRY(hipSetDevice(device));
     hipStream_t st = (hipStream_t)stream;
     if (!d_res) { if (res.ensure(sizeof(ResultRec))) return make_err(LZ4F_ERROR_allocation_failed); d_res = (lz4f_mi355x_result*)res.p; }
-    if (bad.ensure(64)) return make_err(LZ4F_ERROR_allocation_failed);
+    CtlWords* cw;
+    if (size_t e = ctl_words(&cw)) return e;
     ResultRec* r = (ResultRec*)d_res;
     const DecodePlan p = decode_plan(j, sw, device_cus(device));
     uint32_t path = 0;
@@ -824,14 +851,22 @@
     } aux_join{this, st};
     tick(11, false);
     BlockOut* tbl;
-    if (size_t e = dec_table(j, p, r, &tbl, &path)) return e;
+    IndexSrc ix; OpenIx oi; memset(&oi, 0, sizeof(oi));
+    const bool ix_early = p.n_max && p.walk == DecodePlan::WALK_TRAILER && p.ix_by_trailer;
+    if (ix_early) {
+        if (size_t e = dec_index(j, p, r, nullptr, &ix, &path)) return e;
+        bool runs = false;
+        if (!j.linked) { if (size_t e = dec_indexed_ws(p, ix, &runs)) return e; }
+        const uint32_t chunk = pick_chunk_size(j.block_size);
+        if (runs) oi = OpenIx{ix.d, (uint64_t)ix.size, p.n_ix, j.block_size / chunk, chunk, (uint64_t)ix_seq_cap, (uint32_t*)seqcnt.p};
+    }
+    if (size_t e = dec_table(j, p, r, &tbl, &path, oi)) return e;
     const uint32_t* ix_flags = nullptr;
     if (p.n_max) {
         if (j.block_checksum) { if (size_t e = dec_checksums(j, p, r, tbl)) return e; }
         tick(6, false);
-        IndexSrc ix;
-        if (size_t e = dec_index(j, p, r, tbl, &ix, &path)) return e;
-        if (size_t e = dec_indexed(j, p, r, tbl, ix, &ix_flags, &path)) return e;
+        if (!ix_early) { if (size_t e = dec_index(j, p, r, tbl, &ix, &path)) return e; }
+        if (size_t e = dec_indexed(j, p, r, tbl, ix, oi.flags != nullptr, &ix_flags, &path)) return e;
         if (size_t e = dec_generic(j, p, r, tbl, ix_flags, &path)) return e;
         tick(6, true);
     }
diff --git a/lz4_frame_conduit_amd/csrc/engine.hpp b/lz4_frame_conduit_amd/csrc/engine.hpp
--- a/lz4_frame_conduit_amd/csrc/engine.hpp
+++ b/lz4_frame_conduit_amd/csrc/engine.hpp
@@ -53,11 +53,15 @@
 
 }
 
+namespace lz4f { struct CtlWords; struct OpenIx; }
+
 struct lz4f_mi355x_engine {
     int   device = 0;
     void* stream = nullptr;
     bool  own_stream = false;
-    lz4f::DevBuf info, recs, table, blk_bytes, res, bad;
+    lz4f::DevBuf info, recs, table, blk_bytes, res;
+    lz4f::DevBuf ctl;
+    size_t ctl_words(lz4f::CtlWords** out);
     lz4f::DevBuf ixtmp;
     lz4f::DevBuf walkbuf;
     lz4f::DevBuf density;
@@ -136,7 +140,7 @@
     static EncodePlan encode_plan(const CompressJob& j, const Switches& sw, uint32_t cus, bool inband, size_t index_cap);
     size_t enc_workspaces(const EncodePlan& p, bool own_table);
     size_t enc_find(const CompressJob& j, const EncodePlan& p);
-    void   enc_layout(const EncodePlan& p, uint8_t* d_dst, uint64_t dst_cap, lz4f::ResultRec* rec, lz4f::BlockOut* tbl, void* d_index);
+    void   enc_layout(const EncodePlan& p, uint8_t* d_dst, uint64_t dst_cap, lz4f::ResultRec* rec, lz4f::BlockOut* tbl, void* d_index, lz4f::CtlWords* cw);
     void   enc_emit(const CompressJob& j, const EncodePlan& p, uint8_t* d_dst, const lz4f::ResultRec* rec, lz4f::BlockOut* tbl, void* d_index);
     void   enc_tail(const CompressJob& j, const EncodePlan& p, uint8_t* d_dst, uint64_t dst_cap, lz4f::ResultRec* rec, const lz4f::BlockOut* tbl, const void* d_index);
 
@@ -159,11 +163,12 @@
     struct IxRoute { bool selffed, doubling; uint32_t gate; };
     static DecodePlan decode_plan(const DecompressJob& j, const Switches& sw, uint32_t cus);
     static IxRoute ix_route(const DecompressJob& j, const Switches& sw, uint32_t n_ix, uint32_t ix_seqs);
-    size_t dec_table(const DecompressJob& j, const DecodePlan& p, lz4f::ResultRec* res, lz4f::BlockOut** tbl, uint32_t* path);
+    size_t dec_table(const DecompressJob& j, const DecodePlan& p, lz4f::ResultRec* res, lz4f::BlockOut** tbl, uint32_t* path, const lz4f::OpenIx& oi);
     size_t dec_checksums(const DecompressJob& j, const DecodePlan& p, lz4f::ResultRec* res, lz4f::BlockOut* tbl);
     size_t dec_index(const DecompressJob& j, const DecodePlan& p, lz4f::ResultRec* res, lz4f::BlockOut* tbl, IndexSrc* ix, uint32_t* path);
     size_t dec_self_index(const DecompressJob& j, const DecodePlan& p, lz4f::ResultRec* res, lz4f::BlockOut* tbl, bool spx_walk, IndexSrc* ix);
-    size_t dec_indexed(const DecompressJob& j, const DecodePlan& p, lz4f::ResultRec* res, lz4f::BlockOut* tbl, const IndexSrc& ix, const uint32_t** ix_flags, uint32_t* path);
+    size_t dec_indexed_ws(const DecodePlan& p, const IndexSrc& ix, bool* runs);
+    size_t dec_indexed(const DecompressJob& j, const DecodePlan& p, lz4f::ResultRec* res, lz4f::BlockOut* tbl, const IndexSrc& ix, bool opened, const uint32_t** ix_flags, uint32_t* path);
     size_t dec_generic(const DecompressJob& j, const DecodePlan& p, lz4f::ResultRec* res, lz4f::BlockOut* tbl, const uint32_t* only_if, uint32_t* path);
     size_t dec_finish(const DecompressJob& j, const DecodePlan& p, lz4f::ResultRec* res, lz4f::BlockOut* tbl, const uint32_t* ix_flags, uint32_t path);
 };
diff --git a/lz4_frame_conduit_amd/csrc/frame_dev.cuh b/lz4_frame_conduit_amd/csrc/frame_dev.cuh
--- a/lz4_frame_conduit_amd/csrc/frame_dev.cuh
+++ b/lz4_frame_conduit_amd/csrc/frame_dev.cuh
@@ -176,14 +176,11 @@
     }
 }
 
-__global__ __launch_bounds__(64) void k_walk_frame(const uint8_t* __restrict__ frame, uint64_t frame_cap, uint64_t dst_cap,
-                             BlockOut* __restrict__ table, uint32_t table_cap, ResultRec* __restrict__ res, const uint32_t* __restrict__ walked = nullptr)
-{
-    if (threadIdx.x >= WAVE || blockIdx.x != 0) return;
-    if (walked && *walked) return;
+__device__ __forceinline__ void walk_frame_wave(const uint8_t* __restrict__ frame, uint64_t frame_cap, uint64_t dst_cap,
+                                                BlockOut* __restrict__ table, uint32_t table_cap, ResultRec* __restrict__ res, uint32_t* ra_sink)
+{
     const uint32_t lane = lane_id();
     ResultRec r; r.size = 0; r.consumed = 0; r.status = ST_OK; r.n_blocks = 0; r.first_bad_block = 0xFFFFFFFFu; r.flags = 0;
-    __shared__ uint32_t ra_sink[WAVE];
     const uint32_t sink0 = uni((uint32_t)(uintptr_t)(lptr_t)ra_sink);
     auto fail = [&](uint32_t st) { asm volatile("s_waitcnt vmcnt(0)" ::: "memory"); r.status = st; *res = r; };
     if (frame_cap < 7) return fail(ST_INCOMPLETE);
@@ -227,6 +224,14 @@
     r.n_blocks = n; r.consumed = pos; r.size = h.content;
     *res = r;
 }
+__global__ __launch_bounds__(64) void k_walk_frame(const uint8_t* __restrict__ frame, uint64_t frame_cap, uint64_t dst_cap,
+                             BlockOut* __restrict__ table, uint32_t table_cap, ResultRec* __restrict__ res, const uint32_t* __restrict__ walked = nullptr)
+{
+    __shared__ uint32_t ra_sink[WAVE];
+    if (threadIdx.x >= WAVE || blockIdx.x != 0) return;
+    if (walked && *walked) return;
+    walk_frame_wave(frame, frame_cap, dst_cap, table, table_cap, res, ra_sink);
+}
 
 constexpr uint32_t WK_CHUNK = 65536, WK_SLOTS = 30, WK_HOPS = 3;
 struct WalkState {
@@ -487,12 +492,9 @@
     if (t == 0) ws->total = s_carry;
 }
 
-__global__ __launch_bounds__(256) void k_walk_link(const uint8_t* __restrict__ frame, uint64_t frame_cap, uint64_t dst_cap, WalkState* __restrict__ ws,
-                                                   const uint64_t* __restrict__ list, BlockOut* __restrict__ table, uint32_t table_cap)
-{
-    if (!ws->head_ok || ws->overflow) return;
-    const uint32_t total = ws->total;
-    const uint32_t bs = ws->bs, bck = ws->bck;
+__device__ __forceinline__ void walk_link(const uint8_t* __restrict__ frame, uint64_t frame_cap, uint64_t dst_cap, uint32_t total, uint32_t bs, uint32_t bck,
+                                          uint32_t* first_end, uint32_t* first_break, const uint64_t* __restrict__ list, BlockOut* __restrict__ table, uint32_t table_cap)
+{
     for (uint32_t i = blockIdx.x * 256 + threadIdx.x; i < total; i += gridDim.x * 256) {
         const uint64_t p = list[i];
         uint64_t nx = 0; bool end = false;
@@ -504,8 +506,8 @@
             last = ok2 && e2;
             ok = last || (i + 1 < total && list[i + 1] == nx);
         }
-        if (!ok) atomicMin(&ws->first_break, i);
-        else if (last) atomicMin(&ws->first_end, i);
+        if (!ok) atomicMin(first_break, i);
+        else if (last) atomicMin(first_end, i);
         if (ok && i < table_cap) {
             const uint64_t out = (uint64_t)i * bs;
             const uint32_t w = *(const u32_ua*)(frame + p);
@@ -514,44 +516,97 @@
         }
     }
 }
-
-__global__ void k_walk_verdict(const uint8_t* __restrict__ frame, uint64_t frame_cap, uint64_t dst_cap, WalkState* __restrict__ ws,
-                               const uint64_t* __restrict__ list, uint32_t table_cap, ResultRec* __restrict__ res)
-{
-    if (threadIdx.x != 0 || blockIdx.x != 0) return;
+__global__ __launch_bounds__(256) void k_walk_link(const uint8_t* __restrict__ frame, uint64_t frame_cap, uint64_t dst_cap, WalkState* __restrict__ ws,
+                                                   const uint64_t* __restrict__ list, BlockOut* __restrict__ table, uint32_t table_cap)
+{
     if (!ws->head_ok || ws->overflow) return;
-    const uint32_t hsize = ws->hsize, bs = ws->bs, bck = ws->bck, flg = ws->flg;
+    walk_link(frame, frame_cap, dst_cap, ws->total, ws->bs, ws->bck, &ws->first_end, &ws->first_break, list, table, table_cap);
+}
+
+__device__ __forceinline__ bool walk_verdict(const uint8_t* __restrict__ frame, uint64_t frame_cap, uint64_t dst_cap, const FrameHead& h, uint32_t total,
+                                             uint32_t first_end, uint32_t first_break, const uint64_t* __restrict__ list, uint32_t table_cap, ResultRec* __restrict__ res)
+{
+    const uint32_t hsize = h.hsize, bs = h.bs, bck = h.bck, flg = h.flg;
     uint32_t n = 0; uint64_t pos = hsize;
-    if (ws->total == 0 || list[0] != hsize) {
-        if (frame_cap - pos < 4 || *(const u32_ua*)(frame + pos) != 0) return;
+    if (total == 0 || list[0] != hsize) {
+        if (frame_cap - pos < 4 || *(const u32_ua*)(frame + pos) != 0) return false;
         pos += 4;
     } else {
-        const uint32_t e = ws->first_end;
-        if (e == 0xFFFFFFFFu || ws->first_break <= e || e >= table_cap) return;
-        if ((uint64_t)e * bs >= dst_cap) return;
+        const uint32_t e = first_end;
+        if (e == 0xFFFFFFFFu || first_break <= e || e >= table_cap) return false;
+        if ((uint64_t)e * bs >= dst_cap) return false;
         n = e + 1;
         const uint64_t p = list[e];
         pos = p + 4 + word_size(*(const u32_ua*)(frame + p)) + 4 * bck + 4;
     }
     uint32_t tail;
-    if (frame_end(flg, frame_cap - pos, tail)) return;
+    if (frame_end(flg, frame_cap - pos, tail)) return false;
     pos += tail;
-    ResultRec r; r.size = ws->content; r.consumed = pos; r.status = ST_OK; r.n_blocks = n; r.first_bad_block = 0xFFFFFFFFu; r.flags = flg;
+    ResultRec r; r.size = h.content; r.consumed = pos; r.status = ST_OK; r.n_blocks = n; r.first_bad_block = 0xFFFFFFFFu; r.flags = flg;
     *res = r;
-    ws->done = 1;
+    return true;
+}
+__global__ void k_walk_verdict(const uint8_t* __restrict__ frame, uint64_t frame_cap, uint64_t dst_cap, WalkState* __restrict__ ws,
+                               const uint64_t* __restrict__ list, uint32_t table_cap, ResultRec* __restrict__ res)
+{
+    if (threadIdx.x != 0 || blockIdx.x != 0) return;
+    if (!ws->head_ok || ws->overflow) return;
+    FrameHead h = {}; h.hsize = ws->hsize; h.bs = ws->bs; h.bck = ws->bck; h.flg = ws->flg; h.content = ws->content;
+    if (walk_verdict(frame, frame_cap, dst_cap, h, ws->total, ws->first_end, ws->first_break, list, table_cap, res)) ws->done = 1;
+}
+
+struct CtlWords {
+    uint32_t layout_ticket, open_ticket, finish_ticket, pad0;
+    uint32_t first_end, first_break;
+    uint32_t pad[2];
+    uint32_t verdict[8];
+};
+__device__ __forceinline__ void verdict_preset(uint32_t* w, uint32_t lane) { if (lane < 8) w[lane] = lane < 2 ? 0xFFFFFFFFu : 0u; }
+
+struct OpenIx { const void* ix; uint64_t ix_size; uint32_t n_ix, chunks_per_block, chunk_size; uint64_t seq_cap; uint32_t* flags; };
+__global__ __launch_bounds__(256) void k_open_trailer(const uint8_t* __restrict__ frame, uint64_t frame_cap, uint64_t dst_cap, CtlWords* ctl,
+                                                      const uint64_t* __restrict__ list, uint32_t total, BlockOut* table, uint32_t table_cap,
+                                                      ResultRec* res, OpenIx oi)
+{
+    __shared__ FrameHead s_h;
+    __shared__ uint32_t s_ok, s_last;
+    __shared__ uint32_t ra_sink[WAVE];
+    if (threadIdx.x == 0) { FrameHead h = {}; s_ok = frame_head_parse(frame, frame_cap, h) == ST_OK ? 1u : 0u; s_h = h; }
+    __syncthreads();
+    if (s_ok) walk_link(frame, frame_cap, dst_cap, total, s_h.bs, s_h.bck, &ctl->first_end, &ctl->first_break, list, table, table_cap);
+    if (!wg_arrives_last(&ctl->open_ticket, gridDim.x, &s_last)) return;
+    if (threadIdx.x >= WAVE) return;
+    const uint32_t lane = lane_id();
+    uint32_t done = 0;
+    if (lane == 0) {
+        const uint32_t fe = ld_agent(&ctl->first_end), fb = ld_agent(&ctl->first_break);
+        __hip_atomic_store(&ctl->first_end, 0xFFFFFFFFu, __ATOMIC_RELAXED, __HIP_MEMORY_SCOPE_AGENT);
+        __hip_atomic_store(&ctl->first_break, 0xFFFFFFFFu, __ATOMIC_RELAXED, __HIP_MEMORY_SCOPE_AGENT);
+        if (s_ok && walk_verdict(frame, frame_cap, dst_cap, s_h, total, fe, fb, list, table_cap, res)) done = 1;
+    }
+    done = uni(done);
+    if (!done) walk_frame_wave(frame, frame_cap, dst_cap, table, table_cap, res, ra_sink);
+    asm volatile("s_waitcnt vmcnt(0)" ::: "memory");
+    verdict_preset(ctl->verdict, lane);
+    if (oi.flags) {
+        oi.flags[lane] = 0u;
+        asm volatile("s_waitcnt vmcnt(0)" ::: "memory");
+        if (lane == 0) check_index(oi.ix, oi.ix_size, oi.n_ix, oi.chunks_per_block, oi.chunk_size, oi.seq_cap, oi.flags, res);
+    }
 }
 
 struct TrailerPlan { uint64_t at, list_at, ix_at, ix_bytes, total; uint32_t n_list, ok; };
 
-__global__ void k_trailer_plan(uint8_t* __restrict__ dst, uint64_t dst_cap, ResultRec* __restrict__ res, uint32_t n_blocks, const void* __restrict__ ix,
-                               uint64_t ix_fixed, TrailerPlan* __restrict__ plan)
-{
-    if (threadIdx.x != 0 || blockIdx.x != 0) return;
+__device__ __forceinline__ TrailerPlan trailer_plan(uint64_t dst_cap, const ResultRec* res, const BlockOut* __restrict__ table, uint32_t n_blocks, uint32_t bck,
+                                                    uint32_t tail_bytes, const void* ix, uint64_t ix_fixed, bool& with_ix)
+{
     TrailerPlan p; memset(&p, 0, sizeof(p));
+    with_ix = false;
     if (res->status == ST_OK && n_blocks) {
-        const uint64_t F = res->size;
+        const BlockOut e = table[n_blocks - 1];
+        const uint64_t F = e.src_off + (e.word & 0x7FFFFFFFu) + 4u * bck + tail_bytes;
         const IxHeader* hd = (const IxHeader*)ix;
-        const bool with_ix = ix && hd->magic == IX_MAGIC;
+        with_ix = ix && hd->magic == IX_MAGIC;
         p.at = F;
         p.list_at = (F + 8 + 15) & ~(uint64_t)15;
         p.n_list = (n_blocks + 1) & ~1u;
@@ -559,28 +614,34 @@
         p.ix_bytes = with_ix ? (ix_fixed + (uint64_t)hd->total_entries * sizeof(IxEntry) + 15) & ~(uint64_t)15 : 0;
         p.total = p.ix_at + p.ix_bytes + sizeof(TrailerFoot) - F;
         p.ok = (F + p.total <= dst_cap && p.total - 8 < 0xFFFFFFFFull) ? 1u : 0u;
-        if (p.ok) {
-            uint8_t* t = dst + F;
-            const uint32_t sz = (uint32_t)(p.total - 8);
-            st32le(t, TR_MAGIC); st32le(t + 4, sz);
-            for (uint64_t q = F + 8; q < p.list_at; q++) dst[q] = 0;
-            TrailerFoot f{with_ix ? hd->total_seqs : 0u, with_ix ? hd->total_entries : 0u, 0u, 0u, TR_FOOT, n_blocks, p.total};
-            memcpy(dst + p.ix_at + p.ix_bytes, &f, sizeof(f));
-            res->size = F + p.total;
-        } else res->status = ST_DSTSMALL;
-    }
-    *plan = p;
-}
-__global__ __launch_bounds__(256) void k_trailer_copy(uint8_t* __restrict__ dst, const TrailerPlan* __restrict__ plan, const BlockOut* __restrict__ table,
-                                                      uint32_t n_blocks, const void* __restrict__ ix)
-{
-    const TrailerPlan p = *plan;
-    if (!p.ok) return;
-    const uint64_t t = (uint64_t)blockIdx.x * 256 + threadIdx.x, step = (uint64_t)gridDim.x * 256;
-    uint64_t* list = (uint64_t*)(dst + p.list_at);
-    for (uint64_t i = t; i < p.n_list; i += step) list[i] = i < n_blocks ? table[i].src_off - 4 : 0;
-    const uint4* s = (const uint4*)ix; uint4* d = (uint4*)(dst + p.ix_at);
-    for (uint64_t i = t; i < p.ix_bytes / 16; i += step) d[i] = s[i];
+    }
+    return p;
+}
+__global__ __launch_bounds__(256) void k_trailer(uint8_t* __restrict__ dst, uint64_t dst_cap, ResultRec* res, const BlockOut* __restrict__ table,
+                                                 uint32_t n_blocks, uint32_t bck, uint32_t tail_bytes, const void* __restrict__ ix, uint64_t ix_fixed)
+{
+    const bool was_ok = res->status == ST_OK && n_blocks;
+    bool with_ix;
+    const TrailerPlan p = trailer_plan(dst_cap, res, table, n_blocks, bck, tail_bytes, ix, ix_fixed, with_ix);
+    if (p.ok) {
+        const uint64_t t = (uint64_t)blockIdx.x * 256 + threadIdx.x, step = (uint64_t)gridDim.x * 256;
+        uint64_t* list = (uint64_t*)(dst + p.list_at);
+        for (uint64_t i = t; i < p.n_list; i += step) list[i] = i < n_blocks ? table[i].src_off - 4 : 0;
+        const uint4* s = (const uint4*)ix; uint4* d = (uint4*)(dst + p.ix_at);
+        for (uint64_t i = t; i < p.ix_bytes / 16; i += step) d[i] = s[i];
+    }
+    if (threadIdx.x != 0 || blockIdx.x != 0 || !was_ok) return;
+    if (p.ok) {
+        const uint64_t F = p.at;
+        const IxHeader* hd = (const IxHeader*)ix;
+        uint8_t* t = dst + F;
+        const uint32_t sz = (uint32_t)(p.total - 8);
+        st32le(t, TR_MAGIC); st32le(t + 4, sz);
+        for (uint64_t q = F + 8; q < p.list_at; q++) dst[q] = 0;
+        TrailerFoot f{with_ix ? hd->total_seqs : 0u, with_ix ? hd->total_entries : 0u, 0u, 0u, TR_FOOT, n_blocks, p.total};
+        memcpy(dst + p.ix_at + p.ix_bytes, &f, sizeof(f));
+        res->size = F + p.total;
+    } else res->status = ST_DSTSMALL;
 }
 
 __global__ void k_init_result(ResultRec* res, uint32_t n_blocks, uint32_t flags)
@@ -725,8 +786,8 @@
     if (lane == 0) table[b].dst_size = got < 0 ? (uint32_t)-3 : (uint64_t)got <= room ? (uint32_t)got : (uint32_t)-2;
 }
 
-__global__ __launch_bounds__(256) void k_finish_check(const BlockOut* __restrict__ table, const ResultRec* __restrict__ res, uint32_t n_max,
-                                                      uint32_t linked, uint32_t block_size, uint32_t* __restrict__ w)
+__device__ __forceinline__ void finish_check(const BlockOut* __restrict__ table, const ResultRec* __restrict__ res, uint32_t n_max,
+                                             uint32_t linked, uint32_t block_size, uint32_t* __restrict__ w)
 {
     if (res->status != ST_OK) return;
     const uint32_t n = res->n_blocks < n_max ? res->n_blocks : n_max;
@@ -746,11 +807,15 @@
         if (sum) atomicAdd((unsigned long long*)(w + 4), (unsigned long long)sum);
     }
 }
-
-__global__ __launch_bounds__(64) void k_finish_decode(uint8_t* dst, BlockOut* __restrict__ table, ResultRec* res, uint32_t n_max,
-                                                      uint32_t linked, uint32_t block_size, const uint32_t* __restrict__ bad_ck, uint32_t with_ck,
-                                                      uint32_t plan = 0, const uint32_t* __restrict__ ix_flags = nullptr, uint32_t check_here = 0,
-                                                      uint64_t dst_cap = ~0ull)
+__global__ __launch_bounds__(256) void k_finish_check(const BlockOut* __restrict__ table, const ResultRec* __restrict__ res, uint32_t n_max,
+                                                      uint32_t linked, uint32_t block_size, uint32_t* __restrict__ w)
+{
+    finish_check(table, res, n_max, linked, block_size, w);
+}
+
+__device__ __forceinline__ void finish_decode(uint8_t* dst, BlockOut* __restrict__ table, ResultRec* res, uint32_t n_max,
+                                              uint32_t linked, uint32_t block_size, const uint32_t* bad_ck, uint32_t with_ck,
+                                              uint32_t plan, const uint32_t* __restrict__ ix_flags, uint32_t check_here, uint64_t dst_cap, bool by_ticket)
 {
     if (lane_id() == 0) res->flags = (res->flags & 0xFFFu) | (plan << 12) | ((ix_flags && *ix_flags) ? (LZ4F_MI355X_PATH_INDEX_DROPPED << 12) : 0u);
     if (res->status != ST_OK) return;
@@ -770,7 +835,8 @@
 #pragma unroll
         for (int sft = 1; sft < 64; sft <<= 1) sum += __shfl_xor(sum, sft);
         w45 = sum;
-    } else { w1 = bad_ck[1]; w2 = bad_ck[2]; w45 = *(const uint64_t*)(bad_ck + 4); }
+    } else if (by_ticket) { w1 = ld_agent(bad_ck + 1); w2 = ld_agent(bad_ck + 2); w45 = (uint64_t)ld_agent(bad_ck + 4) | (uint64_t)ld_agent(bad_ck + 5) << 32; }
+    else { w1 = bad_ck[1]; w2 = bad_ck[2]; w45 = *(const uint64_t*)(bad_ck + 4); }
     const uint32_t first_bad = w1 < n ? w1 : 0xFFFFFFFFu;
     const uint32_t bad_kind = first_bad != 0xFFFFFFFFu ? table[first_bad].dst_size : 0u;
     const uint32_t ck = with_ck ? bad_ck[0] : 0xFFFFFFFFu;
@@ -820,5 +886,21 @@
         if (const uint32_t st = frame_size_status(res->flags, declared, out)) res->status = st;
     }
 }
-
-}
+__global__ __launch_bounds__(64) void k_finish_decode(uint8_t* dst, BlockOut* __restrict__ table, ResultRec* res, uint32_t n_max,
+                                                      uint32_t linked, uint32_t block_size, const uint32_t* __restrict__ bad_ck, uint32_t with_ck,
+                                                      uint32_t plan = 0, const uint32_t* __restrict__ ix_flags = nullptr, uint32_t check_here = 0,
+                                                      uint64_t dst_cap = ~0ull)
+{
+    finish_decode(dst, table, res, n_max, linked, block_size, bad_ck, with_ck, plan, ix_flags, check_here, dst_cap, false);
+}
+__global__ __launch_bounds__(256) void k_finish(uint8_t* dst, BlockOut* table, ResultRec* res, uint32_t n_max, uint32_t linked, uint32_t block_size,
+                                                CtlWords* ctl, uint32_t with_ck, uint32_t plan, const uint32_t* ix_flags, uint64_t dst_cap)
+{
+    __shared__ uint32_t s_last;
+    finish_check(table, res, n_max, linked, block_size, ctl->verdict);
+    if (!wg_arrives_last(&ctl->finish_ticket, gridDim.x, &s_last)) return;
+    if (threadIdx.x >= WAVE) return;
+    finish_decode(dst, table, res, n_max, linked, block_size, ctl->verdict, with_ck, plan, ix_flags, 0u, dst_cap, true);
+}
+
+}
```

Result: no change. 749.7 (-0.0%).
